# cc-ai/climategan

Hardware: AMD Instinct MI355X
Metric: 640x640 images/sec (G+D step): per-domain sample slots per second of the joint Masker+Painter training step (update_G + update_D), global batch 32 per domain (higher is better)
Workload: dtype bf16

## Files before the change

climategan_amd/_lib.py:

```python
import ctypes as C
import os
from pathlib import Path

_HERE = Path(__file__).resolve().parent
LIB_PATH = Path(os.environ["CGAN_LIB"]).resolve() if os.environ.get("CGAN_LIB") else _HERE / "libcgan_hip.so"

CGAN_F16, CGAN_BF16, CGAN_F32 = 0, 1, 2
ACT_NONE, ACT_RELU, ACT_LRELU, ACT_TANH, ACT_SIGMOID = 0, 1, 2, 3, 4
PAD_ZERO, PAD_REFLECT = 0, 1
ABI_VERSION = 1


class ConvDesc(C.Structure):
    _fields_ = [
        ("dtype", C.c_int32), ("n", C.c_int32), ("h_in", C.c_int32), ("w_in", C.c_int32),
        ("c_in", C.c_int32), ("c_out", C.c_int32),
        ("kh", C.c_int32), ("kw", C.c_int32), ("stride", C.c_int32), ("pad", C.c_int32), ("dilation", C.c_int32),
        ("pad_mode", C.c_int32), ("h_out", C.c_int32), ("w_out", C.c_int32), ("in_upsample", C.c_int32),
        ("act", C.c_int32), ("act_slope", C.c_float), ("has_bias", C.c_int32), ("has_residual", C.c_int32),
        ("residual_upsample", C.c_int32),
    ]


class NormStatsDesc(C.Structure):
# ... 2 lines not shown

class SpadeDesc(C.Structure):
    _fields_ = [
        ("dtype", C.c_int32), ("n", C.c_int32), ("h", C.c_int32), ("w", C.c_int32), ("c", C.c_int32),
        ("x_upsample", C.c_int32), ("cond_h", C.c_int32), ("cond_w", C.c_int32), ("cond_c", C.c_int32),
        ("hidden", C.c_int32), ("ksize", C.c_int32), ("act", C.c_int32), ("act_slope", C.c_float),
    ]


class SnItem(C.Structure):
    _fields_ = [("w_bar", C.c_void_p), ("u", C.c_void_p), ("v", C.c_void_p), ("sigma", C.c_void_p),
                ("workspace", C.c_void_p), ("rows", C.c_int32), ("cols", C.c_int32)]


class PackItem(C.Structure):
    _fields_ = [("w_oihw", C.c_void_p), ("bias", C.c_void_p), ("sigma", C.c_void_p), ("packed", C.c_void_p),
                ("bias_out", C.c_void_p), ("c_out", C.c_int32), ("c_in", C.c_int32), ("kh", C.c_int32),
                ("kw", C.c_int32), ("transposed", C.c_int32)]


class AdamItem(C.Structure):
    _fields_ = [("p", C.c_void_p), ("g", C.c_void_p), ("m", C.c_void_p), ("v", C.c_void_p), ("copy", C.c_void_p),
                ("numel", C.c_int64)]


class AmpOptimItem(C.Structure):
    _fields_ = [("p", C.c_void_p), ("g", C.c_void_p), ("m", C.c_void_p), ("v", C.c_void_p), ("step", C.c_void_p),
                ("numel", C.c_int64)]


class DataTfMap(C.Structure):
    _fields_ = [("row_off", C.c_int32), ("col_off", C.c_int32), ("flip", C.c_int32)]


class DataTfStage(C.Structure):
    _fields_ = [("in_h", C.c_int32), ("in_w", C.c_int32), ("out_h", C.c_int32), ("out_w", C.c_int32)]


class DataTfItem(C.Structure):
    _fields_ = [("src", C.c_void_p), ("dst", C.c_void_p), ("src_h", C.c_int32), ("src_w", C.c_int32),
                ("channels", C.c_int32), ("stride_c", C.c_int32), ("stride_h", C.c_int32), ("stride_w", C.c_int32),
                ("out_h", C.c_int32), ("out_w", C.c_int32), ("n_stages", C.c_int32), ("u8_min", C.c_float),
                ("u8_range", C.c_float), ("stage", DataTfStage * 2), ("map", DataTfMap * 3),
                ("stats", C.c_void_p), ("far_plane", C.c_float), ("dec_flags", C.c_int32)]


class DataTfPalette(C.Structure):
    _fields_ = [("n", C.c_int32), ("default_class", C.c_int32), ("colour", C.c_uint32 * 16), ("cls", C.c_int32 * 16)]


class DataMinmaxItem(C.Structure):
    _fields_ = [("src", C.c_void_p), ("out", C.c_void_p), ("pixels", C.c_int64), ("channels", C.c_int32),
                ("far_plane", C.c_float)]


_P = C.c_void_p
_SIGNATURES = {
    "cgan_version": (C.c_int, []),
    "cgan_last_error": (C.c_char_p, []),
    "cgan_conv2d_packed_weight_bytes": (C.c_size_t, [C.POINTER(ConvDesc)]),
    "cgan_conv2d_pack_weight": (C.c_int, [_P, _P, _P, _P, _P, C.POINTER(ConvDesc), _P]),
    "cgan_conv2d_nhwc_fwd": (C.c_int, [_P, _P, _P, _P, _P, C.POINTER(ConvDesc), _P]),
    "cgan_conv2d_pack_weight_batched": (C.c_int, [_P, C.c_int32, C.c_int32, C.c_int32, _P]),
    "cgan_conv2d_dgrad_packed_weight_bytes": (C.c_size_t, [C.POINTER(ConvDesc)]),
    "cgan_conv2d_pack_weight_dgrad": (C.c_int, [_P, _P, _P, C.POINTER(ConvDesc), _P]),
    "cgan_conv2d_nhwc_bwd_data": (C.c_int, [_P, _P, _P, C.POINTER(ConvDesc), _P]),
    "cgan_conv2d_nhwc_fwd_pair": (C.c_int, [_P, _P, _P, _P, _P, C.POINTER(ConvDesc), _P]),
    "cgan_pair_expand_weight": (C.c_int, [_P, _P, _P, C.c_int32, C.c_int32, C.c_int32, C.c_int32, C.c_int32, _P]),
    "cgan_pair_instnorm_stats": (C.c_int, [_P, _P, _P, C.c_int32, C.c_int32, C.c_int32, C.c_int64, C.c_float, _P]),
    "cgan_pair_spade_apply": (C.c_int, [_P, _P, _P, _P, _P, _P, C.c_int32, C.c_int32, C.c_int32, C.c_int32, C.c_int32, C.c_int32,
                                        C.c_int32, C.c_float, _P]),
    "cgan_pair_make_m_cond_workspace_bytes": (C.c_size_t, [C.c_int32]),
    "cgan_pair_make_m_cond": (C.c_int, [_P, _P, _P, _P, C.c_int32, C.c_int32, C.c_int32, C.c_int32, C.c_int32, C.c_int32, C.c_int32,
                                        _P, C.c_size_t, _P]),
    "cgan_pair_from_nchw": (C.c_int, [_P, _P, C.c_int32, C.c_int32, C.c_int32, C.c_int32, C.c_int32, _P]),
    "cgan_pair_to_nchw": (C.c_int, [_P, _P, C.c_int32, C.c_int32, C.c_int32, C.c_int32, C.c_int32, C.c_int32, _P]),
    "cgan_pair_to_nhwc": (C.c_int, [_P, _P, C.c_int32, C.c_int64, C.c_int32, _P]),
    "cgan_pair_maxpool3x3s2": (C.c_int, [_P, _P, C.c_int32, C.c_int32, C.c_int32, C.c_int32, C.c_int32, _P]),
    "cgan_pair_resize_bilinear": (C.c_int, [_P, _P, C.c_int32, C.c_int32, C.c_int32, C.c_int32, C.c_int32, C.c_int32,
                                            C.c_int32, C.c_int32, _P]),
    "cgan_pair_resize_nearest": (C.c_int, [_P, _P, C.c_int32, C.c_int32, C.c_int32, C.c_int32, C.c_int32, C.c_int32, C.c_int32,
                                           _P]),
    "cgan_pair_resize_bicubic": (C.c_int, [_P, _P, C.c_int32, C.c_int32, C.c_int32, C.c_int32, C.c_int32, C.c_int32, C.c_int32, _P]),
    "cgan_pair_mul": (C.c_int, [_P, _P, _P, C.c_int32, C.c_int64, C.c_int32, _P]),
    "cgan_pair_copy_channels": (C.c_int, [_P, _P, C.c_int32, C.c_int64, C.c_int32, C.c_int32, C.c_int32, _P]),
    "cgan_conv2d_nhwc_bwd_data_add": (C.c_int, [_P, _P, _P, _P, C.POINTER(ConvDesc), _P]),
    "cgan_conv2d_nhwc_bwd_data_relu": (C.c_int, [_P, _P, _P, _P, C.POINTER(ConvDesc), _P]),
    "cgan_conv2d_nhwc_bwd_data_add_relu": (C.c_int, [_P, _P, _P, _P, _P, C.POINTER(ConvDesc), _P]),
    "cgan_conv2d_kernel_kind": (C.c_int, [C.POINTER(ConvDesc), C.c_int32]),
    "cgan_conv2d_kernel_kind_on": (C.c_int, [C.POINTER(ConvDesc), C.c_int32, _P]),
    "cgan_conv2d_bind_workspace": (C.c_int, [_P, _P, C.c_size_t]),
    "cgan_rccl_load": (C.c_int, [C.c_char_p]),
    "cgan_rccl_loaded": (C.c_int, []),
    "cgan_comm_unique_id": (C.c_int, [_P]),
    "cgan_comm_init_rank": (C.c_int, [C.POINTER(C.c_void_p), C.c_int32, _P, C.c_int32]),
    "cgan_comm_destroy": (C.c_int, [_P]),
    "cgan_allreduce_bucket": (C.c_int, [_P, C.c_int64, C.c_int32, _P, _P]),
    "cgan_seg_counts": (C.c_int, [_P, C.c_int32, C.c_int32, C.c_int32, C.c_int64, C.c_int32, _P, _P, _P]),
    "cgan_mask_label_encode": (C.c_int, [_P] + [C.c_int32] * 10 + [_P, _P]),
    "cgan_masker_eval_workspace_bytes": (C.c_size_t, [C.c_int32] * 3),
    "cgan_masker_eval": (C.c_int, [_P, C.c_int32, _P, C.c_int32, C.c_int32, C.c_int32, C.c_int32, C.c_double, C.c_double,
                                   _P, _P, _P, _P, _P, _P, C.c_size_t, _P]),
    "cgan_resize_crop_geometry":(C.c_int, [C.c_int32, C.c_int32, C.c_int32, C.POINTER(C.c_int32), C.POINTER(C.c_int32),
                                            C.POINTER(C.c_int32), C.POINTER(C.c_int32)]),
    "cgan_resize_u8": (C.c_int, [_P, C.c_int32, C.c_int32, C.c_int32, C.c_int32, C.c_int32, _P, C.c_int32, _P, C.c_int32, _P,
                                 _P, C.c_size_t, _P]),
# ... 7 lines not shown
    "cgan_norm_act_apply": (C.c_int, [_P, _P, _P, _P, C.POINTER(NormStatsDesc), C.c_int32, C.c_float, _P]),
    "cgan_make_m_cond_bwd_nhwc": (C.c_int, [_P, _P, _P, _P, _P, C.c_int32, C.c_int32, C.c_int32, C.c_int32, C.c_int32,
                                            C.c_int32, _P]),
    "cgan_resize_nearest_bwd_nhwc": (C.c_int, [_P, _P, C.c_int32, C.c_int32, C.c_int32, C.c_int32, C.c_int32, C.c_int32,
                                               C.c_int32, C.c_int32, C.c_int32, _P]),
    "cgan_norm_add_act_apply": (C.c_int, [_P, _P, _P, _P, _P, C.POINTER(NormStatsDesc), C.c_int32, C.c_float, _P]),
    "cgan_spade_packed_weight_bytes": (C.c_size_t, [C.POINTER(SpadeDesc)]),
    "cgan_spade_pack_weights": (C.c_int, [_P, _P, _P, _P, _P, _P, _P, C.POINTER(SpadeDesc), _P]),
    "cgan_spade_fused_fwd": (C.c_int, [_P, _P, _P, _P, _P, _P, C.POINTER(SpadeDesc), _P]),
    "cgan_spade_fused_fwd_train": (C.c_int, [_P, _P, _P, _P, _P, _P, _P, C.POINTER(SpadeDesc), _P]),
    "cgan_spectral_norm_workspace_bytes": (C.c_size_t, [C.c_int32, C.c_int32]),
    "cgan_spectral_norm_power_iter": (C.c_int, [_P, _P, _P, _P, C.c_int32, C.c_int32, _P, C.c_size_t, _P]),
    "cgan_spectral_norm_power_iter_batched": (C.c_int, [_P, C.c_int32, C.c_int32, C.c_int32, _P]),
    "cgan_extra_adam_multi_tensor": (C.c_int, [_P, C.c_int32, C.c_int64, C.c_int32, C.c_int32, C.c_int32, C.c_double,
                                               C.c_double, C.c_double, C.c_double, C.c_double, _P]),
    "cgan_grads_nonfinite_check_multi_tensor": (C.c_int, [_P, C.c_int32, C.c_int64, C.c_double, C.c_int32, _P, _P]),
    "cgan_adam_multi_tensor": (C.c_int, [_P, C.c_int32, C.c_int64] + [C.c_double] * 6 + [_P, _P]),
    "cgan_rmsprop_multi_tensor": (C.c_int, [_P, C.c_int32, C.c_int64] + [C.c_double] * 5 + [_P, _P]),
    "cgan_amp_optim_finish": (C.c_int, [_P, C.c_int32, _P, _P]),
    "cgan_nchw_to_nhwc": (C.c_int, [_P, _P, _P, C.c_int32, C.c_int32, C.c_int32, C.c_int32, C.c_int32, C.c_int32, _P]),
    "cgan_nhwc_to_nchw": (C.c_int, [_P, _P, _P, _P, C.c_int32, C.c_int32, C.c_int32, C.c_int32, C.c_int32, C.c_int32, _P]),
    "cgan_resize_nearest_nhwc": (C.c_int, [_P, _P, C.c_int32, C.c_int32, C.c_int32, C.c_int32, C.c_int32, C.c_int32,
                                           C.c_int32, C.c_int32, C.c_int32, _P]),
    "cgan_avgpool3x3s2_nhwc": (C.c_int, [_P, _P, C.c_int32, C.c_int32, C.c_int32, C.c_int32, C.c_int32, _P]),
    "cgan_maxpool3x3s2_nhwc": (C.c_int, [_P, _P, C.c_int32, C.c_int32, C.c_int32, C.c_int32, C.c_int32, _P]),
    "cgan_resize_bilinear_nhwc": (C.c_int, [_P, _P, C.c_int32, C.c_int32, C.c_int32, C.c_int32, C.c_int32, C.c_int32,
                                            C.c_int32, C.c_int32, _P]),
    "cgan_resize_bicubic_nhwc": (C.c_int, [_P, _P, C.c_int32, C.c_int32, C.c_int32, C.c_int32, C.c_int32, C.c_int32,
                                           C.c_int32, _P]),
    "cgan_sumpool2x2_nhwc": (C.c_int, [_P, _P, C.c_int32, C.c_int32, C.c_int32, C.c_int32, C.c_int32, _P]),
    "cgan_reflect_pad_bwd_nhwc": (C.c_int, [_P, _P, C.c_int32, C.c_int32, C.c_int32, C.c_int32, C.c_int32, C.c_int32, _P]),
    "cgan_copy_channels_nhwc": (C.c_int, [_P, _P, C.c_int64, C.c_int32, C.c_int32, C.c_int32, C.c_int32, _P]),
    "cgan_eltwise_nhwc": (C.c_int, [_P, _P, _P, C.c_int32, C.c_int32, C.c_int64, _P]),
    "cgan_fold_bn": (C.c_int, [_P, _P, _P, _P, _P, _P, C.c_float, _P, _P, C.c_int32, C.c_int64, _P]),
    "cgan_act_bwd": (C.c_int, [_P, _P, _P, C.c_int32, C.c_int32, C.c_float, C.c_int64, _P]),
    "cgan_instnorm_act_bwd_workspace_bytes": (C.c_size_t, [C.POINTER(NormStatsDesc)]),
    "cgan_instnorm_act_bwd": (C.c_int, [_P, _P, _P, _P, C.POINTER(NormStatsDesc), C.c_int32, C.c_float, _P, C.c_size_t,
                                        _P]),
    "cgan_spade_bwd_prepare": (C.c_int, [_P, _P, _P, _P, _P, _P, _P, _P, _P, C.POINTER(SpadeDesc), _P]),
    "cgan_spade_hidden_bwd_workspace_bytes": (C.c_size_t, [C.POINTER(SpadeDesc)]),
    "cgan_spade_hidden_bwd": (C.c_int, [_P, _P, _P, _P, _P, _P, _P, _P, C.c_size_t, C.POINTER(SpadeDesc), _P]),
    "cgan_batchnorm_train_stats": (C.c_int, [_P, _P, _P, C.c_float, _P, _P, _P, _P, _P, _P, _P, C.POINTER(NormStatsDesc), _P,
                                             C.c_size_t, _P]),
    "cgan_batchnorm_train_stats_from_partials": (C.c_int, [_P, C.c_int32, _P, _P, C.c_float, _P, _P, _P, _P, _P, _P, _P,
                                                           C.POINTER(NormStatsDesc), _P]),
    "cgan_conv2d_stats_chunk_pixels": (C.c_int32, [C.POINTER(ConvDesc)]),
    "cgan_conv2d_nhwc_fwd_stats": (C.c_int, [_P, _P, _P, _P, _P, C.c_size_t, C.POINTER(ConvDesc), _P]),
    "cgan_bn_train_prepare": (C.c_int, [_P, _P, _P, _P, C.c_float, C.c_float, C.c_int64, _P, _P, _P, _P, _P, C.c_int32, _P]),
    "cgan_batchnorm_act_bwd_workspace_bytes": (C.c_size_t, [C.c_int32]),
    "cgan_batchnorm_act_bwd": (C.c_int, [_P, _P, _P, _P, _P, _P, _P, _P, _P, _P, _P, _P, C.c_int32, C.c_int64, C.c_int32,
                                         C.c_int32, C.c_float, _P, C.c_size_t, _P]),
    "cgan_batchnorm_act_bwd_grouped": (C.c_int, [_P, _P, _P, _P, _P, _P, _P, _P, _P, _P, _P, _P, C.c_int32, C.c_int64,
                                                 C.c_int32, C.c_int32, C.c_int32, C.c_float, _P, C.c_size_t, _P]),
    "cgan_bce_logits_nhwc": (C.c_int, [_P, C.c_int32, C.c_int64, C.c_int32, C.c_float, C.c_float, _P, _P, _P]),
    "cgan_hinge_nhwc": (C.c_int, [_P, C.c_int32, C.c_int64, C.c_int32, C.c_int32, C.c_int32, C.c_float, _P, _P, _P]),
    "cgan_l1_nhwc": (C.c_int, [_P, _P, C.c_int32, C.c_int64, C.c_float, _P, _P, _P]),
    "cgan_mse_const_nhwc": (C.c_int, [_P, C.c_int32, C.c_int64, C.c_int32, C.c_float, C.c_float, _P, _P, _P]),
    "cgan_painter_aux_losses": (C.c_int, [_P, _P, _P, C.c_int32, C.c_int32, C.c_int32, C.c_int32, C.c_float, C.c_float,
                                          C.c_float, C.c_float, _P, _P, _P]),
    "cgan_resize_bicubic_bwd_nhwc": (C.c_int, [_P, _P, C.c_int32, C.c_int32, C.c_int32, C.c_int32, C.c_int32, C.c_int32,
                                               C.c_int32, _P]),
    "cgan_spectral_norm_bwd": (C.c_int, [_P, _P, _P, _P, _P, C.c_int32, C.c_int32, _P, _P]),
    "cgan_painter_heads_fwd": (C.c_int, [_P, _P, _P, _P, _P, C.c_int32, C.c_int32, C.c_int32, C.c_int32, _P]),
    "cgan_painter_heads_bwd": (C.c_int, [_P, _P, _P, _P, C.c_int32, C.c_int32, C.c_int32, C.c_int32, _P]),
    "cgan_diffaug_fwd": (C.c_int, [_P, _P, _P, _P, C.c_int32, C.c_int32, C.c_int32, C.c_int32, C.c_int32, C.c_int32,
                                   C.c_int32, _P, _P]),
    "cgan_diffaug_bwd": (C.c_int, [_P, _P, _P, _P, C.c_int32, C.c_int32, C.c_int32, C.c_int32, C.c_int32, C.c_int32,
                                   C.c_int32, _P, _P]),
    "cgan_painter_heads_diffaug_fwd": (C.c_int, [_P, _P, _P, _P, _P, _P, _P, C.c_int32, C.c_int32, C.c_int32, C.c_int32,
                                                 C.c_int32, C.c_int32, C.c_int32, _P, _P]),
    "cgan_painter_heads_diffaug_bwd": (C.c_int, [_P, _P, _P, _P, _P, _P, C.c_int32, C.c_int32, C.c_int32, C.c_int32,
                                                 C.c_int32, C.c_int32, C.c_int32, _P, _P]),
    "cgan_data_transform": (C.c_int, [_P, _P, C.c_int32, C.c_int32, C.c_int32, C.c_int32, _P, _P, _P, C.c_int32, _P, _P]),
    "cgan_data_source_minmax": (C.c_int, [_P, _P, C.c_int32, C.c_int32, _P, _P]),
    "cgan_data_jitter": (C.c_int, [_P, _P, _P, C.c_int32, C.c_int32, C.c_int32, C.c_int32, _P, _P, _P, _P]),
    "cgan_avgpool3x3s2_bwd_nhwc": (C.c_int, [_P, _P, C.c_int32, C.c_int32, C.c_int32, C.c_int32, C.c_int32, _P]),
    "cgan_maxpool2x2_nhwc": (C.c_int, [_P, _P, C.c_int32, C.c_int32, C.c_int32, C.c_int32, C.c_int32, _P]),
    "cgan_maxpool2x2_bwd_nhwc": (C.c_int, [_P, _P, _P, C.c_int32, C.c_int32, C.c_int32, C.c_int32, C.c_int32, _P]),
    "cgan_maxpool2x2_relu_bwd_nhwc": (C.c_int, [_P, _P, _P, C.c_int32, C.c_int32, C.c_int32, C.c_int32, C.c_int32, _P]),
    "cgan_softmax_nhwc": (C.c_int, [_P, _P, C.c_int32, C.c_int64, C.c_int32, _P]),
    "cgan_softmax_bwd_nhwc": (C.c_int, [_P, _P, _P, C.c_int32, C.c_int64, C.c_int32, _P]),
    "cgan_sigmoid_pair_nhwc": (C.c_int, [_P, _P, C.c_int32, C.c_int64, _P]),
    "cgan_sigmoid_pair_bwd_nhwc": (C.c_int, [_P, _P, _P, C.c_int32, C.c_int64, _P]),
    "cgan_softmax_ce_nhwc": (C.c_int, [_P, _P, C.c_int32, C.c_int64, C.c_int32, C.c_float, _P, _P, _P]),
    "cgan_tv_nhwc": (C.c_int, [_P, C.c_int32, C.c_int32, C.c_int32, C.c_int32, C.c_int32, C.c_float, C.c_float, _P, _P, _P]),
    "cgan_advent_entropy_pair_nhwc": (C.c_int, [_P, _P, _P, C.c_int32, C.c_int64, C.c_int32, C.c_int32, _P]),
    "cgan_entropy_pair_from_nchw": (C.c_int, [_P, _P, _P, C.c_int32, C.c_int32, C.c_int32, C.c_int32, C.c_int32, _P]),
    "cgan_entropy_pair_from_nchw_bwd": (C.c_int, [_P, _P, _P, _P, C.c_int32, C.c_int32, C.c_int32, C.c_int32, C.c_int32, _P]),
    "cgan_advent_entropy_pair_bwd_nhwc": (C.c_int, [_P, _P, _P, _P, C.c_int32, C.c_int64, C.c_int32, C.c_int32, _P]),
    "cgan_entropy_map_nhwc": (C.c_int, [_P, _P, _P, C.c_int32, C.c_int64, C.c_int32, _P]),
    "cgan_entropy_map_bwd_nhwc": (C.c_int, [_P, _P, _P, _P, C.c_int32, C.c_int64, C.c_int32, _P]),
    "cgan_minent_nhwc": (C.c_int, [_P, C.c_int32, C.c_int64, C.c_int32, C.c_int32, C.c_float, C.c_float, _P, _P, _P, _P]),
    "cgan_bce_logits_map_nhwc": (C.c_int, [_P, _P, C.c_int32, C.c_int64, C.c_float, _P, _P, _P]),
    "cgan_ground_intersection_nhwc": (C.c_int, [_P, _P, C.c_int32, C.c_int64, C.c_float, _P, _P]),
    "cgan_affine_sum_nhwc": (C.c_int, [_P, C.c_int32, C.c_int64, C.c_int32, C.c_float, C.c_float, _P, _P, _P]),
    "cgan_resize_bilinear_bwd_workspace_bytes": (C.c_size_t, [C.c_int32] * 4),
    "cgan_resize_bilinear_bwd_nhwc": (C.c_int, [_P, _P] + [C.c_int32] * 8 + [_P, C.c_size_t, _P]),
    "cgan_maxpool3x3s2_bwd_nhwc": (C.c_int, [_P, _P, _P, C.c_int32, C.c_int32, C.c_int32, C.c_int32, C.c_int32, _P]),
    "cgan_add_act_nhwc": (C.c_int, [_P, _P, _P, C.c_int32, C.c_int32, C.c_float, C.c_int64, _P]),
    "cgan_slice_channels_nhwc": (C.c_int, [_P, _P, C.c_int64, C.c_int32, C.c_int32, C.c_int32, _P]),
    "cgan_sigm_loss_workspace_bytes": (C.c_size_t, [C.c_int32, C.c_int32, C.c_int32]),
    "cgan_sigm_loss_nhwc": (C.c_int, [_P, _P, C.c_int32, C.c_int32, C.c_int32, C.c_int32, C.c_float, C.c_int32, C.c_float,
                                      _P, _P, _P, C.c_size_t, _P]),
    "cgan_normalize_u8_workspace_bytes": (C.c_size_t, [C.c_int32]),
    "cgan_normalize_u8_nhwc": (C.c_int, [_P, C.c_int32, _P, C.c_int32, C.c_int32, C.c_int32, C.c_int32, _P, C.c_size_t,
                                         _P]),
# ... 115 lines not shown
```

climategan_amd/autograd.py:

```python
import ctypes as C

import os

import torch

from . import ops


GRAD_SCALE = 1.0


def set_grad_scale(s: float):
    global GRAD_SCALE
    GRAD_SCALE = float(s)


BN_GROUPS = 1


class bn_groups:

    def __init__(self, groups: int):
        self.groups = int(groups)

# ... 89 lines not shown

    @staticmethod
    def backward(ctx, dy_t):
        c, h, w, cs = ctx.cfg
        return ops.resize_nearest_bwd(ops.NHWC(dy_t.contiguous(), c), (h, w), cs).t, None, None, None


class ConvFn(torch.autograd.Function):

    @staticmethod
    def forward(ctx, x_t, weight, bias, res_t, packed, cfg, sn):
        x = ops.NHWC(x_t, cfg["c_in"])
        res = ops.NHWC(res_t, weight.shape[0]) if res_t is not None else None
        if cfg.get("mask_input") and (cfg.get("in_upsample", False) or cfg.get("pair_in", False)):
            raise NotImplementedError("ConvFn: mask_input with a folded upsample / a pair map")
        if cfg.get("want_stats") and res is None and cfg["act"] == ops.ACT_NONE and not cfg.get("in_upsample", False):
            y, cfg["stats_out"] = ops.conv2d_with_stats(x, packed, stride=cfg["stride"], pad=cfg["pad"],
                                                        dilation=cfg["dilation"], pad_mode=cfg.get("pad_mode", ops.PAD_ZERO),
                                                        groups=BN_GROUPS)
        else:
            y = ops.conv2d(x, packed, stride=cfg["stride"], pad=cfg["pad"], dilation=cfg["dilation"], act=cfg["act"],
                           slope=cfg["slope"], residual=res, in_upsample=cfg.get("in_upsample", False),
                           residual_upsample=cfg.get("residual_upsample", False),
                           pad_mode=cfg.get("pad_mode", ops.PAD_ZERO))
        ctx.cfg = cfg
        ctx.has_bias = bias is not None
        ctx.has_res = res_t is not None
        ctx.premasked = False
        ctx.sn = None if sn is None else (tuple(sn) if cfg.get("sn_owned") else tuple(t.clone() for t in sn))
        ctx.dgrad = None
        if ctx.needs_input_grad[0] and not cfg.get("pair_in", False):
            ctx.dgrad = ops.dgrad_register(weight, ctx.sn[0] if ctx.sn is not None else None, x_t.dtype, cfg["stride"])
        ctx.save_for_backward(x_t, weight, y.t if cfg["act"] != ops.ACT_NONE else None)
        return y.t

    @staticmethod
    def backward(ctx, dy_t):
        cfg = ctx.cfg
        x_t, weight, y_t = ctx.saved_tensors
        c_out = weight.shape[0]
        ups = cfg.get("in_upsample", False)
        dy = ops.NHWC(dy_t.contiguous(), c_out)
        if y_t is not None and not ctx.premasked:
            dy = ops.act_bwd(ops.NHWC(y_t, c_out), dy, cfg["act"], cfg["slope"])
        sigma = ctx.sn[0] if ctx.sn is not None else None
        dx_t = dres_t = None
        pair = cfg.get("pair_in", False)
        w_eff = torch.cat([weight.detach(), weight.detach()], 1) if pair else weight
        if ctx.needs_input_grad[0]:
            h_in, w_in = (x_t.shape[1] * 2, x_t.shape[2] * 2) if ups else (x_t.shape[1], x_t.shape[2])
            relu_out = ops.NHWC(x_t, cfg["c_in"]) if cfg.get("mask_input") else None
            dx = ops.conv2d_bwd_data(dy, w_eff, (x_t.shape[0], h_in, w_in), stride=cfg["stride"], pad=cfg["pad"],
                                     dilation=cfg["dilation"], sigma=sigma, pad_mode=cfg.get("pad_mode", ops.PAD_ZERO),
                                     prepacked=ctx.dgrad, relu_out=relu_out)
            dx_t = (ops.sumpool2x2(dx) if ups else dx).t
        if ctx.has_res and ctx.needs_input_grad[3]:
            dres_t = (ops.sumpool2x2(dy) if cfg.get("residual_upsample", False) else dy).t
        dw = db = None
        if ctx.needs_input_grad[1] or (ctx.has_bias and ctx.needs_input_grad[2]):
            def wgrad():
                dw, db = ops.conv2d_bwd_weight(ops.NHWC(x_t, cfg["c_in"]), dy, tuple(w_eff.shape), stride=cfg["stride"],
                                               pad=cfg["pad"], dilation=cfg["dilation"], want_bias=ctx.has_bias,
                                               in_upsample=ups, pad_mode=cfg.get("pad_mode", ops.PAD_ZERO))
                if pair:
                    dw = dw[:, :weight.shape[1]] + dw[:, weight.shape[1]:]
                if ctx.sn is not None:
                    dw = ops.spectral_norm_bwd(dw, weight.detach(), ctx.sn[1], ctx.sn[2], ctx.sn[0])
                return dw, db
            dw, db = wgrad()
        return dx_t, dw, db, dres_t, None, None, None


class ConvPassFn(torch.autograd.Function):

    @staticmethod
    def forward(ctx, x_t, weight, bias, packed, cfg):
        x = ops.NHWC(x_t, cfg["c_in"])
        if cfg.get("want_stats") and cfg.get("act", ops.ACT_NONE) != ops.ACT_NONE:
            raise NotImplementedError("ConvPassFn: the statistics epilogue belongs to a conv without an activation")
        if cfg.get("want_stats"):
            y, cfg["stats_out"] = ops.conv2d_with_stats(x, packed, stride=cfg["stride"], pad=cfg["pad"],
                                                        dilation=cfg["dilation"], pad_mode=cfg.get("pad_mode", ops.PAD_ZERO),
                                                        groups=BN_GROUPS)
        else:
            y = ops.conv2d(x, packed, stride=cfg["stride"], pad=cfg["pad"], dilation=cfg["dilation"],
                           act=cfg.get("act", ops.ACT_NONE), slope=cfg.get("slope", 0.0),
                           pad_mode=cfg.get("pad_mode", ops.PAD_ZERO))
        ctx.cfg = cfg
        ctx.has_bias = bias is not None
        ctx.premasked = False
        ctx.dgrad = ops.dgrad_register(weight, None, x_t.dtype, cfg["stride"]) if ctx.needs_input_grad[0] else None
        ctx.save_for_backward(x_t, weight, y.t if cfg.get("act", ops.ACT_NONE) != ops.ACT_NONE else None)
        return y.t, x_t

    @staticmethod
    def backward(ctx, dy_t, dpass_t):
        cfg = ctx.cfg
        x_t, weight, y_t = ctx.saved_tensors
        c_out = weight.shape[0]
        dy = ops.NHWC(dy_t.contiguous(), c_out)
        if y_t is not None and not ctx.premasked:
            dy = ops.act_bwd(ops.NHWC(y_t, c_out), dy, cfg["act"], cfg.get("slope", 0.0))
        dx_t = None
        if ctx.needs_input_grad[0]:
            add = ops.NHWC(dpass_t.contiguous(), cfg["c_in"]) if dpass_t is not None else None
            relu_out = ops.NHWC(x_t, cfg["c_in"]) if cfg.get("mask_input") else None
            dx_t = ops.conv2d_bwd_data(dy, weight, (x_t.shape[0], x_t.shape[1], x_t.shape[2]), stride=cfg["stride"],
                                       pad=cfg["pad"], dilation=cfg["dilation"],
                                       pad_mode=cfg.get("pad_mode", ops.PAD_ZERO), add=add, prepacked=ctx.dgrad,
                                       relu_out=relu_out).t
        dw = db = None
        if ctx.needs_input_grad[1] or (ctx.has_bias and ctx.needs_input_grad[2]):
            dw, db = ops.conv2d_bwd_weight(
                ops.NHWC(x_t, cfg["c_in"]), dy, tuple(weight.shape), stride=cfg["stride"], pad=cfg["pad"],
                dilation=cfg["dilation"], want_bias=ctx.has_bias, pad_mode=cfg.get("pad_mode", ops.PAD_ZERO))
        return dx_t, dw, db, None, None


class InstNormActFn(torch.autograd.Function):

    @staticmethod
    def forward(ctx, x_t, c, eps, act, slope):
        x = ops.NHWC(x_t, c)
        mean, rstd = ops.instnorm_stats(x, eps=eps)
        out = ops.norm_act_apply(x, mean, rstd, act=act, slope=slope)
        ctx.c, ctx.act, ctx.slope = c, act, slope
        ctx.save_for_backward(out.t, rstd)
        return out.t

    @staticmethod
    def backward(ctx, dy_t):
        out_t, rstd = ctx.saved_tensors
        dx = ops.instnorm_act_bwd(ops.NHWC(out_t, ctx.c), ops.NHWC(dy_t.contiguous(), ctx.c), rstd, act=ctx.act,
                                  slope=ctx.slope)
        return dx.t, None, None, None, None


_SPADE_REMAT_GAMMA = os.environ.get("CGAN_SPADE_REMAT_GAMMA") == "1"


_SPADE_FUSED_BWD = os.environ.get("CGAN_SPADE_FUSED_BWD", "1") != "0"


class SpadeFn(torch.autograd.Function):

    @staticmethod
    def forward(ctx, x_t, cond_t, mean, rstd, w_sh, b_sh, w_g, b_g, w_b, b_b, packed, cfg):
        x = ops.NHWC(x_t, cfg["c"])
        cond = ops.NHWC(cond_t, cfg["cond_c"])
        gamma_t = None
        if _SPADE_REMAT_GAMMA or not any(ctx.needs_input_grad):
            y = ops.spade_fused(x, mean, rstd, cond, packed, act=cfg["act"], slope=cfg["slope"],
                                x_upsample=cfg["x_upsample"])
        else:
            y, gamma = ops.spade_fused(x, mean, rstd, cond, packed, act=cfg["act"], slope=cfg["slope"],
                                       x_upsample=cfg["x_upsample"], want_gamma=True)
            gamma_t = gamma.t
        ctx.cfg = cfg
        ctx.save_for_backward(x_t, cond_t, mean, rstd, y.t, w_sh, b_sh, w_g, b_g, w_b, b_b, gamma_t)
        return y.t

    @staticmethod
    def backward(ctx, dy_t):
# ... 121 lines not shown
        ctx.c, ctx.hw = c, (x_t.shape[1], x_t.shape[2])
        return ops.avgpool3x3s2(ops.NHWC(x_t, c)).t

    @staticmethod
    def backward(ctx, dy_t):
        return ops.avgpool3x3s2_bwd(ops.NHWC(dy_t.contiguous(), ctx.c), ctx.hw).t, None


class MaxPool2x2Fn(torch.autograd.Function):

    @staticmethod
    def forward(ctx, x_t, c, mask_input=False):
        ctx.c = c
        ctx.mask_input = bool(mask_input)
        ctx.save_for_backward(x_t)
        return ops.maxpool2x2(ops.NHWC(x_t, c)).t

    @staticmethod
    def backward(ctx, dy_t):
        (x_t,) = ctx.saved_tensors
        return ops.maxpool2x2_bwd(ops.NHWC(x_t, ctx.c), ops.NHWC(dy_t.contiguous(), ctx.c), relu_input=ctx.mask_input).t, None, None


_BN_BWD_READS_OUT = os.environ.get("CGAN_BN_BWD_OUT") == "1"


class BatchNormActFn(torch.autograd.Function):

    @staticmethod
    def forward(ctx, x_t, gamma, beta, running_mean, running_var, c, eps, momentum, act, slope, nbt=None, res_t=None,
                conv_stats=None):
        n, h, w, cs = x_t.shape
        G = BN_GROUPS
        if n % G:
            raise ValueError("BatchNormActFn: batch %d does not divide into %d groups" % (n, G))
        npix = n * h * w // G
        x_t = x_t.contiguous()
        flat = ops.NHWC(x_t.view(G, npix, 1, cs), c)
        if conv_stats is not None and npix % conv_stats.chunk_pixels == 0:
            mean, rstd, mean_f, rstd_f = ops.batchnorm_train_stats_from_partials(
                conv_stats, G, npix, c, gamma, beta, running_mean, running_var, nbt, eps, momentum)
        else:
            mean, rstd, mean_f, rstd_f = ops.batchnorm_train_stats(flat, gamma, beta, running_mean, running_var, nbt, eps,
                                                                   momentum)
        res = None
        if res_t is not None:
            if res_t.shape != x_t.shape:
                raise ValueError("BatchNormActFn: residual %s does not match %s" % (tuple(res_t.shape), tuple(x_t.shape)))
            res = ops.NHWC(res_t.contiguous().view(G, npix, 1, cs), c)
        out = ops.norm_act_apply(flat, mean_f, rstd_f, act=act, slope=slope, residual=res).t.view(n, h, w, cs)
        ctx.cfg = (c, act, slope, G)
        ctx.has_res = res_t is not None
        ctx.premasked = False
        keep_out = res_t is not None or _BN_BWD_READS_OUT
        ctx.save_for_backward(x_t, out if keep_out else None, mean, rstd, gamma,
                              None if keep_out else mean_f, None if keep_out else rstd_f)
        return out

    @staticmethod
    def backward(ctx, dy_t):
        from . import _lib
        lib = _lib.load()
        x_t, out, mean, rstd, gamma, mean_f, rstd_f = ctx.saved_tensors
        c, act, slope, G = ctx.cfg
        if ctx.premasked:
            act = ops.ACT_NONE
        n, h, w, cs = x_t.shape
        nbytes = G * lib.cgan_batchnorm_act_bwd_workspace_bytes(c)
        ws = torch.empty(nbytes, dtype=torch.uint8, device=x_t.device)
        dx = torch.empty_like(x_t)
        want_res = ctx.has_res and ctx.needs_input_grad[11]
        dy_t = dy_t.contiguous()
        if want_res and act == ops.ACT_NONE:
            dres = dy_t
        else:
            dres = torch.empty_like(x_t) if want_res else None
        dg = db = None
        if gamma is not None:
            dg, db = torch.empty((2, c), dtype=torch.float32, device=x_t.device).unbind(0)
        _lib.check(lib.cgan_batchnorm_act_bwd_grouped(
            ops._ptr(x_t), ops._ptr(out), ops._ptr(dy_t), ops._ptr(mean), ops._ptr(rstd), ops._ptr(gamma),
            ops._ptr(mean_f), ops._ptr(rstd_f), ops._ptr(dx), ops._ptr(dg), ops._ptr(db), ops._ptr(dres) if dres is not None and dres is not dy_t else None,
            ops._DT[x_t.dtype], n * h * w, c, G, act, slope, ops._ptr(ws), nbytes, ops._stream()),
            "cgan_batchnorm_act_bwd_grouped")
        return dx, dg, db, None, None, None, None, None, None, None, None, dres, None


def claim_relu_mask(out_t: torch.Tensor) -> bool:
    fn = out_t.grad_fn
    if fn is None:
        return False
    if isinstance(fn, BatchNormActFn._backward_cls):
        if not fn.has_res or fn.cfg[1] != ops.ACT_RELU:
            return False
    elif isinstance(fn, (ConvFn._backward_cls, ConvPassFn._backward_cls)):
        if fn.cfg.get("act", ops.ACT_NONE) != ops.ACT_RELU:
            return False
    else:
        return False
    fn.premasked = True
    return True


def _scaled(dx, c, g):
    return None if dx is None else ops.scale_by_scalar(ops.NHWC(dx, c), g.reshape(1).float().contiguous()).t


class PainterAuxFn(torch.autograd.Function):

    @staticmethod
    def forward(ctx, fake_t, x, m, lam_tv, lam_ctx, lam_rec):
        from . import _lib
        n, h, w = fake_t.shape[0], fake_t.shape[1], fake_t.shape[2]
        x = x.contiguous().float()
        m = m.contiguous().float()
        cnt = float(n * 3 * h * w)
        wh = GRAD_SCALE * lam_tv * 2.0 / (3 * (h - 1) * w) / n
        ww = GRAD_SCALE * lam_tv * 2.0 / (3 * h * (w - 1)) / n
        acc = torch.zeros(3, dtype=torch.float32, device=fake_t.device)
        dfake = torch.empty_like(fake_t) if ctx.needs_input_grad[0] else None
        _lib.check(_lib.load().cgan_painter_aux_losses(ops._ptr(fake_t), ops._ptr(x), ops._ptr(m), ops._DT[fake_t.dtype], n, h, w,
                                                       wh, ww, GRAD_SCALE * lam_ctx / cnt, GRAD_SCALE * lam_rec / cnt,
                                                       ops._ptr(acc), ops._ptr(dfake), ops._stream()), "cgan_painter_aux_losses")
        ctx.save_for_backward(dfake)
        if GRAD_SCALE != 1.0:
            acc = acc / GRAD_SCALE
        ctx.mark_non_differentiable(acc)
        return acc.sum(), acc

    @staticmethod
    def backward(ctx, g, _g_parts):
        (dfake,) = ctx.saved_tensors
        return _scaled(dfake, 3, g), None, None, None, None, None


class ResizeBicubicFn(torch.autograd.Function):

    @staticmethod
    def forward(ctx, x_t, c, size):
        ctx.cfg = (c, x_t.shape[1], x_t.shape[2], int(size[0]), int(size[1]))
        return ops.resize_bicubic(ops.NHWC(x_t, c), size).t

    @staticmethod
    def backward(ctx, dy):
        from . import _lib
        c, h_in, w_in, h_out, w_out = ctx.cfg
        dy = dy.contiguous()
        dx = torch.empty((dy.shape[0], h_in, w_in, dy.shape[3]), dtype=dy.dtype, device=dy.device)
        _lib.check(_lib.load().cgan_resize_bicubic_bwd_nhwc(ops._ptr(dy), ops._ptr(dx), ops._DT[dy.dtype], dy.shape[0], c, h_in,
                                                            w_in, h_out, w_out, ops._stream()), "cgan_resize_bicubic_bwd_nhwc")
        return dx, None, None


def _call(name, *args):
# ... 347 lines not shown
```

climategan_amd/csrc/conv_gemm.h:

```cpp
#pragma once
#include "cgan_common.h"

struct ConvGemmArgs {
  const uint16_t* x;
  const u32x4* w;
  const float* bias;
  const uint16_t* res;
  const uint16_t* res2;
  uint16_t* y;
  int n, h_in, w_in, cin_s;
  int cout, cout_s, ctiles, ksteps;
  int kh, kw, stride, pad, dil, pad_mode;
  int h_out, w_out, npix;
  int act, has_res, res_ups;
  float slope;
  float* stats;
};

struct ConvGemmCls {
  int koff;
  int kh, kw;
  int offy, offx;
};
struct ConvGemmExtArgs {
  ConvGemmArgs a;
  int cls_s;
  int ksplit;
  int ks_per;
  float* ws;
  int pair;
  ConvGemmCls cls[4];
};
bool conv_gemm_ext_shape_ok(const ConvGemmArgs& a);
int conv_gemm_splitk_plan(const ConvGemmArgs& a);
size_t conv_gemm_splitk_workspace_bytes(const ConvGemmArgs& a, int ksplit);
int conv_gemm_splitk_launch(const ConvGemmArgs& a, int ksplit, float* ws, int dtype, hipStream_t s);
int conv_gemm_cls_launch(const ConvGemmArgs& a, int cls_s, const ConvGemmCls* cls, int dtype, hipStream_t s);
int conv_gemm_pair_launch(const ConvGemmArgs& a, int dtype, hipStream_t s);

bool conv_gemm_applicable(const CganConvDesc* d);
int conv_gemm_launch(const ConvGemmArgs& a, int dtype, hipStream_t s);
bool conv_gemm_res2_ok(const ConvGemmArgs& a, int dtype);
int conv_gemm_stats_chunk_pixels(const ConvGemmArgs& a, int dtype);
bool conv_gemm_big_ok(const ConvGemmArgs& a);
bool conv1x1_allc_ok(const ConvGemmArgs& a);
int conv1x1_allc_launch(const ConvGemmArgs& a, int dtype, hipStream_t s);
int conv_gemm_big_launch(const ConvGemmArgs& a, int dtype, hipStream_t s);
bool conv_gemm_big_pair_ok(const ConvGemmArgs& a, int dtype);
int conv_gemm_big_pair_launch(const ConvGemmArgs& a, int dtype, hipStream_t s);
bool conv1x1_xres_ok(const ConvGemmArgs& a);
int conv1x1_xres_launch(const ConvGemmArgs& a, int dtype, hipStream_t s);

#ifdef __HIPCC__
typedef float f32x2 __attribute__((ext_vector_type(2)));

__device__ __forceinline__ float row16_sum(float v) {
  v += __builtin_bit_cast(float, __builtin_amdgcn_update_dpp(0, __builtin_bit_cast(int, v), 0x128, 0xf, 0xf, false));
  v += __builtin_bit_cast(float, __builtin_amdgcn_update_dpp(0, __builtin_bit_cast(int, v), 0x124, 0xf, 0xf, false));
  v += __builtin_bit_cast(float, __builtin_amdgcn_update_dpp(0, __builtin_bit_cast(int, v), 0x122, 0xf, 0xf, false));
  v += __builtin_bit_cast(float, __builtin_amdgcn_update_dpp(0, __builtin_bit_cast(int, v), 0x121, 0xf, 0xf, false));
  return v;
}

template <typename T, int WC, int WP>
__device__ __forceinline__ void conv_gemm_stats_epilogue(f32x4 (&acc)[WC][WP], const ConvGemmArgs& p, int cout_base,
                                                         int chunk, int j, int g) {
  if (p.bias) {
#pragma unroll
    for (int c = 0; c < WC; ++c) {
      const int chb = cout_base + c * 16 + 4 * g;
      const f32x4 b = chb < p.cout_s ? *reinterpret_cast<const f32x4*>(p.bias + chb) : (f32x4){0.f, 0.f, 0.f, 0.f};
#pragma unroll
      for (int t = 0; t < WP; ++t) acc[c][t] += b;
    }
  }
  constexpr float inv_cnt = 1.f / (float)(WP * 16);
#pragma unroll
  for (int c = 0; c < WC; ++c) {
    f32x2 vr[WP][2];
#pragma unroll
    for (int t = 0; t < WP; ++t) {
#pragma unroll
      for (int hh = 0; hh < 2; ++hh) {
        float r0, r1;
        unpack2<T>(pack2<T>(acc[c][t][2 * hh], acc[c][t][2 * hh + 1]), r0, r1);
        vr[t][hh] = (f32x2){r0, r1};
      }
    }
    f32x2 s0[2] = {vr[0][0], vr[0][1]};
#pragma unroll
    for (int t = 1; t < WP; ++t) {
      s0[0] += vr[t][0];
      s0[1] += vr[t][1];
    }
    float sm[4], sq[4];
#pragma unroll
    for (int r = 0; r < 4; ++r) sm[r] = row16_sum(s0[r >> 1][r & 1]) * inv_cnt;
    const f32x2 m2[2] = {(f32x2){sm[0], sm[1]}, (f32x2){sm[2], sm[3]}};
    f32x2 s1[2];
#pragma unroll
    for (int hh = 0; hh < 2; ++hh) {
      const f32x2 dv = vr[0][hh] - m2[hh];
      s1[hh] = dv * dv;
    }
#pragma unroll
    for (int t = 1; t < WP; ++t)
#pragma unroll
      for (int hh = 0; hh < 2; ++hh) {
        const f32x2 dv = vr[t][hh] - m2[hh];
        s1[hh] += dv * dv;
      }
#pragma unroll
    for (int r = 0; r < 4; ++r) sq[r] = row16_sum(s1[r >> 1][r & 1]);
    const int ch = cout_base + c * 16 + 4 * g;
    if (j == 0 && ch < p.cout_s) {
      float o[8];
#pragma unroll
      for (int r = 0; r < 4; ++r) {
        o[2 * r] = sm[r];
        o[2 * r + 1] = sq[r];
      }
      float* dst = p.stats + ((size_t)chunk * p.cout_s + ch) * 2;
      *reinterpret_cast<f32x4*>(dst) = (f32x4){o[0], o[1], o[2], o[3]};
      *reinterpret_cast<f32x4*>(dst + 4) = (f32x4){o[4], o[5], o[6], o[7]};
    }
  }
}

template <typename T, int WC, int WP, int PP, bool RES2 = false>
__device__ __forceinline__ void conv_gemm_staged_store(const f32x4 (&acc)[WC][WP], const ConvGemmArgs& p,
                                                       unsigned char* stg, int pix0, int cout_base, const float* bias_ep,
                                                       int lane, int j, int g) {
  constexpr int ROWB = WC * 64 + 16;
  constexpr int CH = WC * 2;
  constexpr int NIT = PP * 16 * CH / 64;
  constexpr int NPASS = WP / PP;
  constexpr int PSTEP = 64 / CH;
  static_assert(64 % CH == 0 && WP % PP == 0, "a lane keeps its channel chunk over the iterations");
  const int qc = lane % CH, pl0 = lane / CH;
  const int ch = cout_base + qc * 8;
  const bool ch_ok = ch < p.cout_s;
  const bool plain = !bias_ep && !p.has_res && p.act == CGAN_ACT_NONE && p.cout == p.cout_s;
  f32x4 bb0 = (f32x4){0.f, 0.f, 0.f, 0.f}, bb1 = bb0;
  if (bias_ep && ch_ok) {
    bb0 = *reinterpret_cast<const f32x4*>(bias_ep + ch);
    bb1 = *reinterpret_cast<const f32x4*>(bias_ep + ch + 4);
  }
  u32x4 rv[NPASS][NIT];
  u32x4 rm[RES2 ? (NPASS > 1 ? 2 : 1) : 1][RES2 ? NIT : 1];
  auto load_rm = [&](int pass, u32x4 (&dst)[RES2 ? NIT : 1]) {
#pragma unroll
    for (int it = 0; it < (RES2 ? NIT : 0); ++it) {
      const int pix = pix0 + pass * PP * 16 + it * PSTEP + pl0;
      dst[it] = (u32x4){0u, 0u, 0u, 0u};
      if (pix < p.npix && ch_ok) dst[it] = CGAN_LD_STREAM(reinterpret_cast<const u32x4*>(p.res2 + (size_t)pix * p.cout_s + ch));
    }
  };
  if (p.has_res) {
#pragma unroll
    for (int pass = 0; pass < NPASS; ++pass)
#pragma unroll
      for (int it = 0; it < NIT; ++it) {
        const int pix = pix0 + pass * PP * 16 + it * PSTEP + pl0;
        rv[pass][it] = (u32x4){0u, 0u, 0u, 0u};
        if (pix < p.npix && ch_ok) {
          size_t rbase;
          if (p.res_ups) {
            const int ox = pix % p.w_out;
            const int r = pix / p.w_out;
            const int oy = r % p.h_out;
            const int nn = r / p.h_out;
            rbase = (((size_t)nn * (p.h_out >> 1) + (oy >> 1)) * (p.w_out >> 1) + (ox >> 1)) * p.cout_s;
          } else {
            rbase = (size_t)pix * p.cout_s;
          }
          rv[pass][it] = CGAN_LD_STREAM(reinterpret_cast<const u32x4*>(p.res + rbase + ch));
        }
      }
    if (RES2 && p.has_res == 3) load_rm(0, rm[0]);
    __builtin_amdgcn_sched_barrier(0);
  }
#pragma unroll
  for (int pass = 0; pass < NPASS; ++pass) {
#pragma unroll
    for (int tt = 0; tt < PP; ++tt)
#pragma unroll
      for (int c = 0; c < WC; ++c)
        *reinterpret_cast<f32x4*>(stg + (tt * 16 + j) * ROWB + c * 64 + g * 16) = acc[c][pass * PP + tt];
    asm volatile("s_waitcnt lgkmcnt(0)" ::: "memory");
    if (RES2 && NPASS > 1 && p.has_res == 3 && pass + 1 < NPASS) {
      __builtin_amdgcn_sched_barrier(0);
      load_rm(pass + 1, rm[(pass + 1) & 1]);
      __builtin_amdgcn_sched_barrier(0);
    }
    if (pass == 0 || (RES2 && p.has_res == 3 && pass >= 2)) __builtin_amdgcn_s_waitcnt(0x0F70);
#pragma unroll
    for (int it = 0; it < NIT; ++it) {
      const int pl = it * PSTEP + pl0;
      const int pix = pix0 + pass * PP * 16 + pl;
      const f32x4 v0 = *reinterpret_cast<const f32x4*>(stg + pl * ROWB + qc * 32);
      const f32x4 v1 = *reinterpret_cast<const f32x4*>(stg + pl * ROWB + qc * 32 + 16);
      float v[8] = {v0[0], v0[1], v0[2], v0[3], v1[0], v1[1], v1[2], v1[3]};
      if (!plain) {
        if (bias_ep) {
#pragma unroll
          for (int r = 0; r < 4; ++r) {
            v[r] += bb0[r];
            v[4 + r] += bb1[r];
          }
        }
        if (RES2 && p.has_res == 3) {
#pragma unroll
          for (int e = 0; e < 4; ++e) {
            float r0, r1, m0, m1;
            unpack2<T>(rv[pass][it][e], r0, r1);
            unpack2<T>(rm[RES2 && NPASS > 1 ? (pass & 1) : 0][RES2 ? it : 0][e], m0, m1);
            v[2 * e] = cgan_res_apply3(v[2 * e], r0, m0);
            v[2 * e + 1] = cgan_res_apply3(v[2 * e + 1], r1, m1);
          }
        } else if (p.has_res) {
#pragma unroll
          for (int e = 0; e < 4; ++e) {
            float r0, r1;
            unpack2<T>(rv[pass][it][e], r0, r1);
            v[2 * e] = cgan_res_apply(v[2 * e], r0, p.has_res);
            v[2 * e + 1] = cgan_res_apply(v[2 * e + 1], r1, p.has_res);
          }
        }
        act_apply_n(v, p.act, p.slope);
        if (p.cout < p.cout_s) {
#pragma unroll
          for (int r = 0; r < 8; ++r)
            if (ch + r >= p.cout) v[r] = 0.f;
        }
      }
      u32x4 o;
#pragma unroll
      for (int e = 0; e < 4; ++e) o[e] = pack2<T>(v[2 * e], v[2 * e + 1]);
      if (pix < p.npix && ch_ok) CGAN_ST_STREAM(o, reinterpret_cast<u32x4*>(p.y + (size_t)pix * p.cout_s + ch));
    }
    asm volatile("s_waitcnt lgkmcnt(0)" ::: "memory");
  }
}
#endif
```

climategan_amd/csrc/conv_gemm.hip:

```cpp
#include "conv_gemm.h"
#include <type_traits>

namespace {

__device__ __attribute__((aligned(16))) unsigned int g_gemm_zeros[4];

constexpr int NSTAGE = 3;
CGAN_KNOB(int, g_gemm_ws, 0);

__device__ __forceinline__ int reflect_i(int i, int n) {
  if (i < 0) i = -i;
  if (i >= n) i = 2 * n - 2 - i;
  return i;
}

template <typename T, int WAVES_C, int WC, int WP, bool REFLECT, int NS = NSTAGE, bool RES2 = false>
__global__ __launch_bounds__(256, 2) void conv_gemm_kernel(ConvGemmArgs p, int npb, int ncb) {
  constexpr int WAVES_P = 4 / WAVES_C;
  constexpr int CT_BLK = WAVES_C * WC;
  constexpr int PT_BLK = WAVES_P * WP;
  constexpr int STAGE_BYTES = (CT_BLK + PT_BLK) * 1024;
  constexpr int W_PER_WAVE = CT_BLK / 4;
  constexpr int P_PER_WAVE = PT_BLK / 4;
  constexpr int DMA_PER_WAVE = W_PER_WAVE + P_PER_WAVE;
  static_assert(CT_BLK % 4 == 0 && PT_BLK % 4 == 0, "tiles must split evenly over the 4 waves");
  extern __shared__ __attribute__((aligned(1024))) unsigned char smem[];

  const int lane = threadIdx.x & 63;
  const int wave = __builtin_amdgcn_readfirstlane(threadIdx.x >> 6);
  const int j = lane & 15;
  const int g = lane >> 4;
  const int wc = wave % WAVES_C, wp = wave / WAVES_C;

  const int xcd = blockIdx.x & 7, slot = blockIdx.x >> 3;
  const int cblk = slot % ncb;
  const int pblk = xcd * ((npb + 7) >> 3) + slot / ncb;
  if (pblk >= npb) return;

  int pbase[P_PER_WAVE], py0[P_PER_WAVE], px0[P_PER_WAVE];
#pragma unroll
  for (int m = 0; m < P_PER_WAVE; ++m) {
    int pix = (pblk * PT_BLK + wave + 4 * m) * 16 + j;
    bool v = pix < p.npix;
    int pc = v ? pix : 0;
    int ox = pc % p.w_out;
    int r = pc / p.w_out;
    int oy = r % p.h_out;
    int nn = r / p.h_out;
    pbase[m] = nn * p.h_in * p.w_in * p.cin_s + g * 8;
    py0[m] = v ? oy * p.stride - p.pad : -(1 << 28);
    px0[m] = ox * p.stride - p.pad;
  }
  const int ccn = p.cin_s >> 5;
  const long zero_off = reinterpret_cast<const unsigned char*>(g_gemm_zeros) - reinterpret_cast<const unsigned char*>(p.x);

  int i_ky = 0, i_kx = 0, i_cc = 0, i_buf = 0;
  auto issue_piece = [&](int piece) {
    unsigned char* buf = smem + i_buf * STAGE_BYTES;
    if (piece < W_PER_WAVE) {
      const int i = wave + 4 * piece;
      const int ct = min(cblk * CT_BLK + i, p.ctiles - 1);
      const u32x4* src = p.w + ((size_t)ct * p.ksteps + (i_ky * p.kw + i_kx) * ccn + i_cc) * 64 + lane;
      __builtin_amdgcn_global_load_lds((const __attribute__((address_space(1))) void*)src,
                                       (__attribute__((address_space(3))) void*)(buf + i * 1024), 16, 0, 0);
    } else {
      const int m = piece - W_PER_WAVE;
      const int i = wave + 4 * m;
      int iy = py0[m] + i_ky * p.dil, ix = px0[m] + i_kx * p.dil;
      bool ok;
      if (REFLECT) {
// ... 25 lines not shown
    for (int q = 0; q < DMA_PER_WAVE; ++q) issue_piece(q);
    issue_advance();
  };

  f32x4 acc[WC][WP];
#pragma unroll
  for (int c = 0; c < WC; ++c)
#pragma unroll
    for (int t = 0; t < WP; ++t) acc[c][t] = (f32x4){0.f, 0.f, 0.f, 0.f};

  issue();
  if (NS > 2) issue();
  int r_buf = 0;
  for (int ks = 0; ks < p.ksteps; ++ks) {
    asm volatile("s_waitcnt vmcnt(%0) lgkmcnt(0)" ::"n"((NS - 2) * DMA_PER_WAVE) : "memory");
    __builtin_amdgcn_s_barrier();
    const unsigned char* buf = smem + r_buf * STAGE_BYTES;
    u32x4 a[WC], b[WP];
#pragma unroll
    for (int t = 0; t < WP; ++t)
      b[t] = *reinterpret_cast<const u32x4*>(buf + (CT_BLK + wp * WP + t) * 1024 + lane * 16);
#pragma unroll
    for (int c = 0; c < WC; ++c) a[c] = *reinterpret_cast<const u32x4*>(buf + (wc * WC + c) * 1024 + lane * 16);
    constexpr int NM = WC * WP;
    constexpr int GAP = NM / (DMA_PER_WAVE + 1);
    __builtin_amdgcn_sched_barrier(0);
#pragma unroll
    for (int i = 0; i < NM; ++i) {
      const int c = i / WP, t = i % WP;
      acc[c][t] = mfma16(as_vec8<T>(a[c]), as_vec8<T>(b[t]), acc[c][t]);
      if ((i + 1) % GAP == 0 && (i + 1) / GAP <= DMA_PER_WAVE) {
        issue_piece((i + 1) / GAP - 1);
        __builtin_amdgcn_sched_barrier(0);
      }
    }
    issue_advance();
    r_buf = (r_buf + 1 == NS) ? 0 : r_buf + 1;
  }

  constexpr int ROWB = WC * 64 + 16;
  constexpr int PP = (4 * 4 * 16 * ROWB <= NS * STAGE_BYTES && WP % 4 == 0) ? 4
                     : (4 * 2 * 16 * ROWB <= NS * STAGE_BYTES ? 2 : 1);
  static_assert(4 * PP * 16 * ROWB <= NS * STAGE_BYTES, "epilogue staging does not fit");
  static_assert(WP % PP == 0, "WP must be a multiple of PP");
  asm volatile("s_waitcnt vmcnt(0) lgkmcnt(0)" ::: "memory");
  __builtin_amdgcn_s_barrier();
  unsigned char* stg = smem + wave * (PP * 16 * ROWB);
  const int cout_base = (cblk * CT_BLK + wc * WC) * 16;
  const float* bias_ep = p.bias;
  if (p.stats && (pblk * PT_BLK + wp * WP) * 16 < p.npix) {
    conv_gemm_stats_epilogue<T, WC, WP>(acc, p, cout_base, pblk * WAVES_P + wp, j, g);
    if (p.bias) bias_ep = nullptr;
  }
  conv_gemm_staged_store<T, WC, WP, PP, RES2>(acc, p, stg, (pblk * PT_BLK + wp * WP) * 16, cout_base, bias_ep, lane, j, g);
}

template <typename T, int WC, int WP>
__global__ __launch_bounds__(512, 2) void conv_gemm_k64_kernel(ConvGemmArgs p, int npb, int ncb, int tiles_total) {
  constexpr int CT_BLK = 2 * WC, PT_BLK = 2 * WP;
  constexpr int W_BYTES = CT_BLK * 2048, STAGE_BYTES = (CT_BLK + PT_BLK) * 2048;
  constexpr int NS = 3;
  constexpr int W_PER = CT_BLK / 2, P_PER = PT_BLK / 2, PIECES = W_PER + P_PER;
  static_assert(PIECES <= 63, "vmcnt range");
  extern __shared__ __attribute__((aligned(1024))) unsigned char smem[];

  const int lane = threadIdx.x & 63;
  const int wave = __builtin_amdgcn_readfirstlane(threadIdx.x >> 6);
  const int xcd = blockIdx.x & 7, slot = blockIdx.x >> 3, nslot = gridDim.x >> 3;
  const int per = (tiles_total + 7) >> 3;
  const int t0 = xcd * per;
  const int t1 = min(t0 + per, tiles_total);
  const int my_n = (t1 - t0 > slot) ? (t1 - t0 - slot + nslot - 1) / nslot : 0;
  if (my_n <= 0) return;
  const int first = t0 + slot;
  const int cc2n = p.cin_s >> 6;
  const int n_st = p.kh * p.kw * cc2n;
  const int n_it = my_n * n_st;

  if (wave >= 4) {
    const int pw = wave - 4;
    const int half = pw & 1;
    const int ccn = p.cin_s >> 5;
    const long zero_off = reinterpret_cast<const unsigned char*>(g_gemm_zeros) - reinterpret_cast<const unsigned char*>(p.x);
    const int q = lane >> 3;
    const int kchunk = (lane & 7) ^ (4 * half + ((q >> 1) & 3));
    int poff[P_PER];
    unsigned vmask[P_PER];
    const u32x4* wtile[W_PER];
    auto set_tile = [&](int ti) {
      const int gt = first + ti * nslot;
      const int pblk = gt / ncb;
      const int cblk = gt - pblk * ncb;
#pragma unroll
      for (int m = 0; m < W_PER; ++m)
        wtile[m] = p.w + (size_t)min(cblk * CT_BLK + (pw >> 1) + 2 * m, p.ctiles - 1) * p.ksteps * 64 + half * 64 + lane;
#pragma unroll
      for (int m = 0; m < P_PER; ++m) {
        const int pix = (pblk * PT_BLK + (pw >> 1) + 2 * m) * 16 + 8 * half + q;
        const bool v = pix < p.npix;
        const int pc = v ? pix : 0;
        const int ox = pc % p.w_out;
        const int r = pc / p.w_out;
        const int oy = r % p.h_out;
        const int nn = r / p.h_out;
        const int py0 = oy * p.stride - p.pad, px0 = ox * p.stride - p.pad;
        poff[m] = ((nn * p.h_in * p.w_in + py0 * p.w_in + px0) * p.cin_s + kchunk * 8) * 2;
        unsigned mk = 0;
// ... 156 lines not shown
#pragma unroll
        for (int r = 0; r < 4; ++r) {
          v[r] = act_apply(v[r], p.act, p.slope);
          if (ch + r >= p.cout) v[r] = 0.f;
        }
        u32x2 o;
        o.x = pack2<T>(v[0], v[1]);
        o.y = pack2<T>(v[2], v[3]);
        CGAN_ST_STREAM(o, reinterpret_cast<u32x2*>(p.y + (size_t)pix * p.cout_s + ch));
      }
    }
  };

  for (int ti = 0; ti < my_n; ++ti) {
    first_read(ti > 0);
    for (int st = 0; st + 1 < n_st; ++st) {
      step(a0, b0, a1, b1, 1);
      step(a1, b1, a0, b0, 0);
    }
    step(a0, b0, a1, b1, 1);
    step(a1, b1, a0, b0, -1);
    epilogue(ti);
  }
}

template <typename T, int WC, int WP>
int launch_k64(const ConvGemmArgs& a, hipStream_t s) {
  constexpr int CT_BLK = 2 * WC, PT_BLK = 2 * WP;
  constexpr size_t smem = (size_t)3 * (CT_BLK + PT_BLK) * 2048;
  static bool attr_set = false;
  if (!attr_set) {
    hipError_t e = hipFuncSetAttribute(reinterpret_cast<const void*>(&conv_gemm_k64_kernel<T, WC, WP>),
                                       hipFuncAttributeMaxDynamicSharedMemorySize, 160 * 1024);
    if (e != hipSuccess) {
      cgan_set_error("conv_gemm_k64: hipFuncSetAttribute failed: %s", hipGetErrorString(e));
      return CGAN_ERR_HIP;
    }
    attr_set = true;
  }
  const int npb = ceil_div(ceil_div(a.npix, 16), PT_BLK);
  const int ncb = ceil_div(a.ctiles, CT_BLK);
  const int tiles = npb * ncb;
  const int per = ceil_div(tiles, 8);
  const int nslot = per < 32 ? per : 32;
  hipLaunchKernelGGL((conv_gemm_k64_kernel<T, WC, WP>), dim3(8 * nslot), dim3(512), smem, s, a, npb, ncb, tiles);
  return CGAN_OK;
}
bool k64_ok(const ConvGemmArgs& a) {
  return (a.cin_s & 63) == 0 && a.pad_mode != CGAN_PAD_REFLECT && a.kh * a.kw <= 32 &&
         (long)a.n * a.h_in * a.w_in * a.cin_s < (1L << 30) - (1L << 20);
}


template <typename T, int WAVES_C, int WC, int WP, bool REFLECT, int NS = NSTAGE, bool RES2 = false>
int launch_cfg2(const ConvGemmArgs& a, hipStream_t s) {
  constexpr int WAVES_P = 4 / WAVES_C;
  constexpr int CT_BLK = WAVES_C * WC, PT_BLK = WAVES_P * WP;
  constexpr size_t smem = (size_t)NS * (CT_BLK + PT_BLK) * 1024;
  static bool attr_set = false;
  if (!attr_set) {
    hipError_t e = hipFuncSetAttribute(reinterpret_cast<const void*>(&conv_gemm_kernel<T, WAVES_C, WC, WP, REFLECT, NS, RES2>),
                                       hipFuncAttributeMaxDynamicSharedMemorySize, 160 * 1024);
    if (e != hipSuccess) {
      cgan_set_error("conv_gemm: hipFuncSetAttribute failed: %s", hipGetErrorString(e));
      return CGAN_ERR_HIP;
    }
    attr_set = true;
  }
  const int npb = ceil_div(ceil_div(a.npix, 16), PT_BLK);
  const int ncb = ceil_div(a.ctiles, CT_BLK);
  const int grid = ceil_div(npb, 8) * 8 * ncb;
  hipLaunchKernelGGL((conv_gemm_kernel<T, WAVES_C, WC, WP, REFLECT, NS, RES2>), dim3(grid), dim3(256), smem, s, a, npb, ncb);
  return CGAN_OK;
}

template <typename T, int WAVES_C, int WC, int WP, int NS = NSTAGE>
int launch_cfg(const ConvGemmArgs& a, hipStream_t s) {
  return a.pad_mode == CGAN_PAD_REFLECT ? launch_cfg2<T, WAVES_C, WC, WP, true, NS>(a, s)
                                        : launch_cfg2<T, WAVES_C, WC, WP, false, NS>(a, s);
}

CGAN_KNOB(int, g_gemm_cfg, 0);

enum { KIND_PLAIN = 0, KIND_K64_256x128, KIND_K64_128x256, KIND_BIG, KIND_DIRECT, KIND_XRES };
struct Choice {
  int kind;
  int cfg;
};

Choice choose(const ConvGemmArgs& a, bool bf16) {
  const int ptiles = ceil_div(a.npix, 16);
  const bool no_big = g_gemm_ws == 9;
  const bool no_xres = g_gemm_ws == 9 || g_gemm_ws == 12;
  const int ws = (no_big || no_xres || g_gemm_ws == 13 || g_gemm_ws == 14) ? 0 : g_gemm_ws;
  switch (ws) {
    case 5: if (k64_ok(a)) return {KIND_K64_256x128, 0}; break;
    case 6: if (k64_ok(a)) return {KIND_K64_128x256, 0}; break;
    case 8: if (conv_gemm_big_ok(a)) return {KIND_BIG, 0}; break;
    case 10: if (conv1x1_allc_ok(a)) return {KIND_DIRECT, 0}; break;
    case 11: if (conv1x1_xres_ok(a)) return {KIND_XRES, 0}; break;
    default: break;
  }
  const bool automatic = ws == 0 && g_gemm_cfg == 0;
  (void)bf16;
  if (automatic && !no_big && conv1x1_allc_ok(a) && a.ctiles <= 4 && a.npix >= 16384) return {KIND_DIRECT, 0};
  if (automatic && !no_xres && conv1x1_xres_ok(a) && a.ctiles >= 16 && a.npix >= 16384) return {KIND_XRES, 0};
  const bool long_1x1 = a.kh * a.kw == 1 && g_gemm_ws != 13 &&
                        (g_gemm_ws == 14 ? (a.cin_s >= 2048 || (a.cin_s >= 512 && a.ctiles >= 128))
                                         : (a.cin_s >= 1024 || (a.cin_s >= 512 && a.ctiles >= 128)));
  if (automatic && !no_big && conv_gemm_big_ok(a) && a.npix >= 16384 &&
      ((a.cin_s * a.kh * a.kw >= 4096 && a.cin_s >= 512 && !(a.kh * a.kw >= 9 && a.cin_s >= 2048)) || long_1x1))
    return {KIND_BIG, 0};
  if (automatic && k64_ok(a) && a.kh * a.kw >= 9 && a.cin_s >= 512 && a.npix >= 16384) return {KIND_K64_256x128, 0};
  switch (g_gemm_cfg) {
    case 1: return {KIND_PLAIN, 1};
    case 2: if (a.ctiles <= 16) return {KIND_PLAIN, 2}; break;
    case 3: return {KIND_PLAIN, 3};
    case 4: return {KIND_PLAIN, 4};
    case 5: return {KIND_PLAIN, 5};
    default: break;
  }
  if (a.ctiles <= 4) return {KIND_PLAIN, 1};
  if (a.kh * a.kw == 1 && a.ksteps <= 16) return {KIND_PLAIN, 5};
  if (a.ctiles > 8 && a.ctiles <= 16 && ceil_div(ptiles, 8) >= 384) return {KIND_PLAIN, 2};
  if ((long)ceil_div(ptiles, 16) * ceil_div(a.ctiles, 8) >= 384) return {KIND_PLAIN, 3};
  return {KIND_PLAIN, 4};
}

template <typename T>
int launch(const ConvGemmArgs& a, hipStream_t s) {
  const Choice ch = choose(a, std::is_same<T, BF16>::value);
  switch (ch.kind) {
    case KIND_K64_256x128: return launch_k64<T, 8, 4>(a, s);
    case KIND_K64_128x256: return launch_k64<T, 4, 8>(a, s);
    case KIND_BIG: return conv_gemm_big_launch(a, T::id, s);
    case KIND_DIRECT: return conv1x1_allc_launch(a, T::id, s);
    case KIND_XRES: return conv1x1_xres_launch(a, T::id, s);
    default: break;
  }
  switch (ch.cfg) {
    case 1: return launch_cfg<T, 1, 4, 4>(a, s);
    case 2: return launch_cfg<T, 2, 8, 4>(a, s);
    case 3: return launch_cfg<T, 2, 4, 8>(a, s);
    case 5:
      if (a.has_res == 3) return launch_cfg2<T, 2, 4, 4, false, 2, true>(a, s);
      return launch_cfg<T, 2, 4, 4, 2>(a, s);
    default: return launch_cfg<T, 2, 4, 4>(a, s);
  }
}

}

bool conv_gemm_applicable(const CganConvDesc* d) {
  const int cin_s = cgan_cs(d->c_in), cout_s = cgan_cs(d->c_out);
  const long npix = (long)d->n * d->h_out * d->w_out;
  const long in_elems = (long)d->n * d->h_in * d->w_in * cin_s;
  return (cin_s % 32) == 0 && cout_s >= 64 && !d->in_upsample && npix >= 2048 && in_elems < (1L << 31) - (1L << 20) &&
         (long)ceil_div((int)ceil_div((int)npix, 16), 8) * ceil_div(ceil_div(cout_s, 16), 8) >= 128;
}

CGAN_DEV_ONLY(extern "C" void cgan_debug_set_gemm_cfg(int v) { g_gemm_cfg = v; })
CGAN_DEV_ONLY(extern "C" void cgan_debug_set_gemm_ws(int v) { g_gemm_ws = v; })

int conv_gemm_launch(const ConvGemmArgs& a, int dtype, hipStream_t s) {
  return dtype == CGAN_F16 ? launch<F16>(a, s) : launch<BF16>(a, s);
}

bool conv_gemm_res2_ok(const ConvGemmArgs& a, int dtype) {
  const Choice ch = choose(a, dtype == CGAN_BF16);
  return (ch.kind == KIND_PLAIN && ch.cfg == 5 && a.pad_mode != CGAN_PAD_REFLECT) || ch.kind == KIND_BIG;
}

int conv_gemm_stats_chunk_pixels(const ConvGemmArgs& a, int dtype) {
  const Choice ch = choose(a, dtype == CGAN_BF16);
  if (ch.kind == KIND_XRES) return a.npix % 128 == 0 ? 128 : 0;
  if (ch.kind == KIND_BIG) return a.npix % 64 == 0 ? 64 : 0;
  if (ch.kind != KIND_PLAIN) return 0;
  const int ppb = ch.cfg == 3 ? 128 : 64;
  return a.npix % ppb == 0 ? ppb : 0;
}
```

climategan_amd/csrc/conv_gemm_big.hip:

```cpp
#include "conv_gemm.h"
#include <type_traits>

namespace {

__device__ __attribute__((aligned(16))) unsigned int g_big_zeros[4];

template <typename T, int NW, bool PAIR = false, bool RES2 = false>
__global__ __launch_bounds__(NW * 64, NW / 4) void conv_gemm_big_kernel(ConvGemmArgs p, int npb, int ncb) {
  constexpr int WC = NW == 16 ? 4 : 8;
  constexpr int WP = NW == 4 ? 8 : 4;
  constexpr bool DOUBLE = NW == 4;
  constexpr int CT_BLK = 16, PT_BLK = 16;
  constexpr int STAGE = 32 * 1024;
  constexpr int NSW = 2, NSX = 3;
  constexpr int X_BASE = NSW * STAGE;
  constexpr int NPC = 32 / NW;
  constexpr int NM = WC * WP, NR = WC + WP;
  static_assert(NSW * STAGE + NSX * STAGE == 160 * 1024, "the rings take all of the CU's LDS");
  extern __shared__ __attribute__((aligned(1024))) unsigned char smem[];

  const int lane = threadIdx.x & 63;
  const int wave = __builtin_amdgcn_readfirstlane(threadIdx.x >> 6);
  const int xcd = blockIdx.x & 7, slot = blockIdx.x >> 3;
  const int cblk = slot % ncb;
  const int pblk = xcd * ((npb + 7) >> 3) + slot / ncb;
  if (pblk >= npb) return;

  const int half = wave & 1;
  const int ccn = p.cin_s >> 5;
  const int cc2n = p.cin_s >> 6;
  const int n_st = p.kh * p.kw * cc2n;
  const long zero_off = reinterpret_cast<const unsigned char*>(g_big_zeros) - reinterpret_cast<const unsigned char*>(p.x);
  const u32x4* wsrc[NPC];
  int poff[NPC];
  unsigned vmask[NPC];
  const int csb = PAIR ? p.cin_s / Split<T>::NB : p.cin_s;
  const int xs = PAIR ? Split<T>::NS * csb : p.cin_s;
  const float inv_csb = 1.0f / (float)csb;
  const int kchunk = (lane & 7) ^ (4 * half + (((lane >> 3) >> 1) & 3));
  {
    const int q = lane >> 3;
#pragma unroll
    for (int m = 0; m < NPC; ++m) {
      const int t = (wave >> 1) + (NW / 2) * m;
      wsrc[m] = p.w + (size_t)min(cblk * CT_BLK + t, p.ctiles - 1) * p.ksteps * 64 + half * 64 + lane;
      const int pix = (pblk * PT_BLK + t) * 16 + 8 * half + q;
      const bool v = pix < p.npix;
      const int pc = v ? pix : 0;
      const int ox = pc % p.w_out;
      const int r = pc / p.w_out;
      const int oy = r % p.h_out;
      const int nn = r / p.h_out;
      const int py0 = oy * p.stride - p.pad, px0 = ox * p.stride - p.pad;
      poff[m] = ((nn * p.h_in * p.w_in + py0 * p.w_in + px0) * xs + (PAIR ? 0 : kchunk * 8)) * 2;
      unsigned mk = 0;
      for (int ky = 0; ky < p.kh; ++ky)
        for (int kx = 0; kx < p.kw; ++kx) {
          const bool ok = v && (unsigned)(py0 + ky * p.dil) < (unsigned)p.h_in && (unsigned)(px0 + kx * p.dil) < (unsigned)p.w_in;
          mk |= (ok ? 1u : 0u) << (ky * p.kw + kx);
        }
      vmask[m] = mk;
// ... 106 lines not shown
  };
  auto next_slots = [&]() {
    rw = (rw + 1 == NSW) ? 0 : rw + 1;
    rx = (rx + 1 == NSX) ? 0 : rx + 1;
  };

  issue_w_stage();
  issue_x_stage();
  if (n_st > 1) {
    issue_x_stage();
    issue_w_stage();
    asm volatile("s_waitcnt vmcnt(%0)" ::"n"(2 * NPC) : "memory");
  } else {
    asm volatile("s_waitcnt vmcnt(0)" ::: "memory");
  }
  __builtin_amdgcn_s_barrier();
  fetch_half(0, 0, 0, a0, b0);

  for (int s = 0; s < n_st; ++s) {
    const bool more = s + 2 < n_st;
    if (DOUBLE) {
      half_step(a0, b0, a1, b1, true, rw, rx, 1, P1{}, more);
    } else {
      half_step(a0, b0, a0, b0, false, 0, 0, 0, P1{}, more);
      fetch_half(rw, rx, 1, a0, b0);
    }
    if (more) asm volatile("s_waitcnt vmcnt(%0) lgkmcnt(0)" ::"n"(NPC) : "memory");
    else asm volatile("s_waitcnt vmcnt(0) lgkmcnt(0)" ::: "memory");
    __builtin_amdgcn_s_barrier();
    next_slots();
    if (DOUBLE) {
      half_step(a1, b1, a0, b0, true, rw, rx, 0, P2{}, more);
    } else {
      half_step(a0, b0, a0, b0, false, 0, 0, 0, P2{}, more);
      fetch_half(rw, rx, 0, a0, b0);
    }
  }

  constexpr int ROWB = WC * 64 + 16;
  constexpr int PP = NW == 4 ? 4 : 2;
  constexpr int CH = WC * 2;
  static_assert(NW * PP * 16 * ROWB <= 160 * 1024, "epilogue staging does not fit");
  static_assert(WP % PP == 0, "WP must be a multiple of PP");
  asm volatile("s_waitcnt vmcnt(0) lgkmcnt(0)" ::: "memory");
  __builtin_amdgcn_s_barrier();
  unsigned char* stg = smem + wave * (PP * 16 * ROWB);
  const int cout_base = (cblk * CT_BLK + wc * WC) * 16;
  const float* bias_ep = p.bias;
  if (p.stats && (pblk * PT_BLK + wp * WP) * 16 < p.npix) {
    conv_gemm_stats_epilogue<T, WC, WP>(acc, p, cout_base, pblk * (PT_BLK / WP) + wp, j16, g);
    if (p.bias) bias_ep = nullptr;
  }
  if constexpr (!PAIR) {
    conv_gemm_staged_store<T, WC, WP, PP, RES2>(acc, p, stg, (pblk * PT_BLK + wp * WP) * 16, cout_base, bias_ep, lane, j16, g);
    return;
  }
  constexpr int NIT = PP * 16 * CH / 64;
  constexpr int NSB = Split<T>::NS, NCC = Split<T>::NC;
  const int qc = lane % CH, pl0 = lane / CH;
  const int ch = cout_base + qc * 8;
  const bool ch_ok = ch < p.cout_s;
  f32x4 bb0 = (f32x4){0.f, 0.f, 0.f, 0.f}, bb1 = bb0;
  if (bias_ep && ch_ok) {
    bb0 = *reinterpret_cast<const f32x4*>(bias_ep + ch);
    bb1 = *reinterpret_cast<const f32x4*>(bias_ep + ch + 4);
  }
  auto epilogue_pass = [&](auto pass_tag) {
    constexpr int pass = decltype(pass_tag)::value;
#pragma unroll
    for (int tt = 0; tt < PP; ++tt)
#pragma unroll
      for (int c = 0; c < WC; ++c)
        *reinterpret_cast<f32x4*>(stg + (tt * 16 + j16) * ROWB + c * 64 + g * 16) = acc[c][pass * PP + tt];
    asm volatile("s_waitcnt lgkmcnt(0)" ::: "memory");
    const int pix_base = (pblk * PT_BLK + wp * WP + pass * PP) * 16;
    u32x4 rs[NIT][NCC];
    if (p.has_res) {
      __builtin_amdgcn_sched_barrier(0);
#pragma unroll
      for (int it = 0; it < NIT; ++it) {
        const int pix = pix_base + it * (64 / CH) + pl0;
        size_t rpix = (size_t)(pix < p.npix ? pix : 0);
        if (p.res_ups && pix < p.npix) {
          const int ox = pix % p.w_out;
          const int r = pix / p.w_out;
          const int oy = r % p.h_out;
          const int nn = r / p.h_out;
          rpix = ((size_t)nn * (p.h_out >> 1) + (oy >> 1)) * (p.w_out >> 1) + (ox >> 1);
        }
        const uint16_t* rp = p.res + rpix * p.cout_s * NSB + ch;
#pragma unroll
        for (int k = 0; k < NCC; ++k) {
          rs[it][k] = (u32x4){0u, 0u, 0u, 0u};
          if (pix < p.npix && ch_ok) rs[it][k] = *reinterpret_cast<const u32x4*>(rp + k * p.cout_s);
        }
      }
      __builtin_amdgcn_sched_barrier(0);
    }
    __builtin_amdgcn_s_waitcnt(0x0F70);
#pragma unroll
    for (int it = 0; it < NIT; ++it) {
      const int pl = it * (64 / CH) + pl0;
      const int pix = pix_base + pl;
      const f32x4 v0 = *reinterpret_cast<const f32x4*>(stg + pl * ROWB + qc * 32);
      const f32x4 v1 = *reinterpret_cast<const f32x4*>(stg + pl * ROWB + qc * 32 + 16);
      float v[8] = {v0[0], v0[1], v0[2], v0[3], v1[0], v1[1], v1[2], v1[3]};
      if (bias_ep) {
#pragma unroll
        for (int r = 0; r < 4; ++r) {
          v[r] += bb0[r];
          v[4 + r] += bb1[r];
        }
      }
      if (p.has_res) {
        float rsum[8] = {0.f, 0.f, 0.f, 0.f, 0.f, 0.f, 0.f, 0.f};
#pragma unroll
        for (int k = NCC - 1; k >= 0; --k) {
#pragma unroll
          for (int e = 0; e < 4; ++e) {
            float r0, r1;
            unpack2<T>(rs[it][k][e], r0, r1);
            rsum[2 * e] += r0;
            rsum[2 * e + 1] += r1;
          }
        }
#pragma unroll
        for (int r = 0; r < 8; ++r) v[r] += rsum[r];
      }
      act_apply_n(v, p.act, p.slope);
      if (p.cout < p.cout_s) {
#pragma unroll
        for (int r = 0; r < 8; ++r)
          if (ch + r >= p.cout) v[r] = 0.f;
      }
      uint16_t* yp = p.y + (size_t)pix * p.cout_s * NSB + ch;
#pragma unroll
      for (int k = 0; k < NCC; ++k) {
        u32x4 comp;
#pragma unroll
        for (int e = 0; e < 4; ++e) {
          comp[e] = pack2<T>(v[2 * e], v[2 * e + 1]);
          float q0, q1;
          unpack2<T>(comp[e], q0, q1);
          v[2 * e] -= q0;
          v[2 * e + 1] -= q1;
        }
        if (pix < p.npix && ch_ok) *reinterpret_cast<u32x4*>(yp + k * p.cout_s) = comp;
      }
    }
    asm volatile("s_waitcnt lgkmcnt(0)" ::: "memory");
  };
  static_assert(WP / PP == 2, "two staging passes");
  epilogue_pass(std::integral_constant<int, 0>{});
  epilogue_pass(std::integral_constant<int, 1>{});
}

template <typename T, int NW, bool PAIR = false, bool RES2 = false>
int launch_big(const ConvGemmArgs& a, hipStream_t s) {
  constexpr size_t smem = 160 * 1024;
  static bool attr_set = false;
  if (!attr_set) {
    hipError_t e = hipFuncSetAttribute(reinterpret_cast<const void*>(&conv_gemm_big_kernel<T, NW, PAIR, RES2>),
                                       hipFuncAttributeMaxDynamicSharedMemorySize, 160 * 1024);
    if (e != hipSuccess) {
      cgan_set_error("conv_gemm_big: hipFuncSetAttribute failed: %s", hipGetErrorString(e));
      return CGAN_ERR_HIP;
    }
    attr_set = true;
  }
  const int npb = ceil_div(ceil_div(a.npix, 16), 16);
  const int ncb = ceil_div(a.ctiles, 16);
  const int grid = ceil_div(npb, 8) * 8 * ncb;
  hipLaunchKernelGGL((conv_gemm_big_kernel<T, NW, PAIR, RES2>), dim3(grid), dim3(NW * 64), smem, s, a, npb, ncb);
  return CGAN_OK;
}

}

bool conv_gemm_big_ok(const ConvGemmArgs& a) {
  return (a.cin_s & 63) == 0 && a.pad_mode != CGAN_PAD_REFLECT && a.kh * a.kw <= 32 && a.ctiles >= 12 &&
         (long)a.n * a.h_in * a.w_in * a.cin_s < (1L << 30) - (1L << 20);
}

CGAN_KNOB(int, g_big_waves, 8);
CGAN_DEV_ONLY(extern "C" void cgan_debug_set_big_waves(int v) { g_big_waves = v; })

int conv_gemm_big_launch(const ConvGemmArgs& a, int dtype, hipStream_t s) {
  if (g_big_waves == 16 && a.has_res != 3)
    return dtype == CGAN_F16 ? launch_big<F16, 16>(a, s) : launch_big<BF16, 16>(a, s);
  if (a.has_res == 3)
    return dtype == CGAN_F16 ? launch_big<F16, 8, false, true>(a, s) : launch_big<BF16, 8, false, true>(a, s);
  return dtype == CGAN_F16 ? launch_big<F16, 8>(a, s) : launch_big<BF16, 8>(a, s);
}

bool conv_gemm_big_pair_ok(const ConvGemmArgs& a, int dtype) {
  const int nb = cgan_split_blocks(dtype), ns = cgan_split_store_blocks(dtype);
  return (a.cin_s & 63) == 0 && (a.cin_s % nb) == 0 && a.pad_mode != CGAN_PAD_REFLECT && a.kh * a.kw <= 32 && a.ctiles >= 12 &&
         a.npix >= 16384 && a.stats == nullptr &&
         (long)a.n * a.h_in * a.w_in * (a.cin_s / nb) * ns < (1L << 30) - (1L << 20) &&
         (long)a.npix * a.cout_s * ns < (1L << 31);
}
int conv_gemm_big_pair_launch(const ConvGemmArgs& a, int dtype, hipStream_t s) {
  return dtype == CGAN_F16 ? launch_big<F16, 8, true>(a, s) : launch_big<BF16, 8, true>(a, s);
}
```

climategan_amd/csrc/conv_mfma.hip:

```cpp
#include "cgan_common.h"
#include "conv3x3_lds.h"
#include "conv_gemm.h"

namespace {

struct ConvParams {
  const uint16_t* x;
  const u32x4* w;
  const float* bias;
  const uint16_t* res;
  const uint16_t* res2;
  uint16_t* y;
  int n, h_in, w_in, hx, wx, cin_s, cin_p, cg;
  int cout, cout_s, ctiles;
  int kh, kw, stride, pad, dil, pad_mode;
  int h_out, w_out, npix;
  int kgroups, ksteps;
  int in_ups, act, has_res, res_ups;
  int in_zs;
  int cls_s;
  int cls_pad;
  float slope;
  float* stats;
  int pair;
// ... 596 lines not shown
extern "C" int cgan_conv2d_pack_weight(const float* w_oihw, const float* bias, const float* sigma, void* packed,
                                       float* bias_out, const CganConvDesc* d, void* stream) {
  ConvParams p;
  int rc = fill_params(p, d);
  if (rc != CGAN_OK) return rc;
  CGAN_REQUIRE(w_oihw && packed, "conv2d_pack_weight: null pointer");
  const int total = p.ctiles * p.ksteps * 64;
  const int blocks = ceil_div(total, 256) < 2048 ? ceil_div(total, 256) : 2048;
  hipStream_t s = (hipStream_t)stream;
  if (d->dtype == CGAN_F16)
    hipLaunchKernelGGL(pack_conv_weight_kernel<F16>, dim3(blocks), dim3(256), 0, s, w_oihw, bias, sigma,
                       (uint16_t*)packed, bias_out, d->c_out, d->c_in, p.cin_p, d->kh, d->kw, p.ctiles, p.ksteps, 0);
  else
    hipLaunchKernelGGL(pack_conv_weight_kernel<BF16>, dim3(blocks), dim3(256), 0, s, w_oihw, bias, sigma,
                       (uint16_t*)packed, bias_out, d->c_out, d->c_in, p.cin_p, d->kh, d->kw, p.ctiles, p.ksteps, 0);
  CGAN_CHECK_LAUNCH("conv2d_pack_weight");
  return CGAN_OK;
}

extern "C" int cgan_conv2d_pack_weight_batched(const CganPackItem* items_device, int32_t count, int32_t dtype,
                                               int32_t max_fragments, void* stream) {
  CGAN_REQUIRE(items_device && count > 0 && max_fragments > 0, "conv2d_pack_weight_batched: bad arguments");
  CGAN_REQUIRE(dtype == CGAN_F16 || dtype == CGAN_BF16, "conv2d_pack_weight_batched: bad dtype %d", dtype);
  const int blocks = ceil_div(max_fragments, 256) < 512 ? ceil_div(max_fragments, 256) : 512;
  hipStream_t s = (hipStream_t)stream;
  if (dtype == CGAN_F16)
    hipLaunchKernelGGL(pack_conv_weight_batched_kernel<F16>, dim3(blocks, count), dim3(256), 0, s, items_device);
  else
    hipLaunchKernelGGL(pack_conv_weight_batched_kernel<BF16>, dim3(blocks, count), dim3(256), 0, s, items_device);
  CGAN_CHECK_LAUNCH("conv2d_pack_weight_batched");
  return CGAN_OK;
}

#include <mutex>
namespace {
struct WsSlot { int device; void* stream; void* ws; size_t bytes; };
constexpr int WS_SLOTS = 64;
WsSlot g_ws[WS_SLOTS];
int g_ws_n = 0;
int g_ws_next = 0;
std::mutex g_ws_mu;
int ws_device() {
  int dev = 0;
  if (hipGetDevice(&dev) != hipSuccess) dev = 0;
  return dev;
}
WsSlot ws_lookup(void* stream) {
  const int dev = ws_device();
  std::lock_guard<std::mutex> lk(g_ws_mu);
  for (int i = 0; i < g_ws_n; ++i)
    if (g_ws[i].stream == stream && g_ws[i].device == dev) return g_ws[i];
  return WsSlot{dev, stream, nullptr, 0};
}
size_t ws_max_bytes() {
  const int dev = ws_device();
  std::lock_guard<std::mutex> lk(g_ws_mu);
  size_t m = 0;
  for (int i = 0; i < g_ws_n; ++i)
    if (g_ws[i].device == dev && g_ws[i].bytes > m) m = g_ws[i].bytes;
  return m;
}
}

extern "C" int cgan_conv2d_bind_workspace(void* stream, void* workspace, size_t bytes) {
  CGAN_REQUIRE((workspace != nullptr) == (bytes > 0), "conv2d_bind_workspace: workspace and bytes must both be set or both be zero");
  CGAN_REQUIRE((reinterpret_cast<size_t>(workspace) & 15) == 0, "conv2d_bind_workspace: workspace must be 16-byte aligned");
  const int dev = ws_device();
  std::lock_guard<std::mutex> lk(g_ws_mu);
  for (int i = 0; i < g_ws_n; ++i)
    if (g_ws[i].stream == stream && g_ws[i].device == dev) {
      if (workspace == nullptr) {
        g_ws[i] = g_ws[g_ws_n - 1];
        --g_ws_n;
        if (g_ws_next >= g_ws_n) g_ws_next = 0;
      } else {
        g_ws[i].ws = workspace; g_ws[i].bytes = bytes;
      }
      return CGAN_OK;
    }
  if (workspace == nullptr) return CGAN_OK;
  if (g_ws_n < WS_SLOTS) {
    g_ws[g_ws_n++] = WsSlot{dev, stream, workspace, bytes};
  } else {
    g_ws[g_ws_next] = WsSlot{dev, stream, workspace, bytes};
    g_ws_next = (g_ws_next + 1) % WS_SLOTS;
  }
  return CGAN_OK;
}

static int dgrad_desc(const CganConvDesc* f, CganConvDesc* t) {
  CGAN_REQUIRE(f != nullptr, "conv2d bwd_data: null descriptor");
  CGAN_REQUIRE(f->pad_mode == CGAN_PAD_ZERO, "conv2d bwd_data: only zero padding has a backward path");
  CGAN_REQUIRE(f->stride >= 1 && f->dilation >= 1 && f->kh > 0 && f->kw > 0, "conv2d bwd_data: bad kernel params");
  *t = *f;
  t->c_in = f->c_out; t->c_out = f->c_in;
  t->h_in = (f->h_out - 1) * f->stride + 1;
  t->w_in = (f->w_out - 1) * f->stride + 1;
  t->stride = 1;
  t->pad = f->dilation * (f->kh - 1) - f->pad;
  CGAN_REQUIRE(f->kh == f->kw, "conv2d bwd_data: square kernels only");
  t->h_out = t->h_in + 2 * t->pad - f->dilation * (f->kh - 1);
  t->w_out = t->w_in + 2 * t->pad - f->dilation * (f->kw - 1);
  CGAN_REQUIRE(t->h_out <= f->h_in && t->w_out <= f->w_in && t->h_out > 0 && t->w_out > 0,
               "conv2d bwd_data: inconsistent forward descriptor");
  t->in_upsample = 0; t->act = CGAN_ACT_NONE; t->has_bias = 0; t->has_residual = 0; t->residual_upsample = 0;
  return CGAN_OK;
// ... 1 lines not shown

static bool dgrad_subpixel(const CganConvDesc* f) {
  return g_conv_force == 0 && f->kh == 4 && f->kw == 4 && f->stride == 2 && f->pad == 1 && f->dilation == 1 &&
         f->pad_mode == CGAN_PAD_ZERO && f->c_in <= 4 && !f->in_upsample && (cgan_cs(f->c_out) % 32) == 0 &&
         (f->h_in % 2) == 0 && (f->w_in % 2) == 0 && (long)f->h_out * f->w_out >= 1024;
}

template <typename T>
__global__ void pack_dgrad_subpixel_kernel(const float* __restrict__ w, const float* __restrict__ sigma,
                                           uint16_t* __restrict__ packed, int c_out, int c_in, int cin_p) {
  const int nq = cin_p / 32, total = 9 * nq * 64;
  const float sig = sigma ? sigma[0] : 1.f;
  for (int idx = blockIdx.x * blockDim.x + threadIdx.x; idx < total; idx += gridDim.x * blockDim.x) {
    const int lane = idx & 63, ks = idx >> 6;
    const int tap = ks / nq, q = ks - tap * nq;
    const int ty = tap / 3, tx = tap - ty * 3;
    const int row = lane & 15, a = row >> 3, b = (row >> 2) & 1, c = row & 3;
    const int ky = a + 3 - 2 * ty, kx = b + 3 - 2 * tx;
    const int k0 = q * 32 + (lane >> 4) * 8;
    uint16_t o[8];
#pragma unroll
    for (int e = 0; e < 8; ++e) {
      const int co = k0 + e;
      float v = 0.f;
      if (co < c_out && c < c_in && ky >= 0 && ky < 4 && kx >= 0 && kx < 4)
        v = __fdiv_rn(w[(((size_t)co * c_in + c) * 4 + ky) * 4 + kx], sig);
      o[e] = bits_of<T>(v);
    }
    u32x4 pk;
    pk[0] = o[0] | ((uint32_t)o[1] << 16);
    pk[1] = o[2] | ((uint32_t)o[3] << 16);
    pk[2] = o[4] | ((uint32_t)o[5] << 16);
    pk[3] = o[6] | ((uint32_t)o[7] << 16);
    reinterpret_cast<u32x4*>(packed)[idx] = pk;
  }
}

namespace {
enum ConvRoute {
  ROUTE_GEMM,
  ROUTE_SPLITK,
  ROUTE_LDS3X3,
  ROUTE_SMALLCIN,
  ROUTE_SUBPIXEL,
  ROUTE_CLS_GEMM,
  ROUTE_PAIR_BIG,
  ROUTE_PAIR_GEMM,
  ROUTE_GENERAL,
};
enum { FWD_PLAIN, FWD_STATS, FWD_PAIR };
enum { RES_NONE = 0, RES_ADD = 1, RES_RELU = 2, RES_ADD_RELU = 3 };

struct ConvPlan {
  ConvRoute route;
  ConvParams p;
  CganConvDesc d;
  int ksplit;
  float* ws;
};

ConvGemmArgs gemm_args(const ConvParams& p) {
  ConvGemmArgs a;
  a.x = p.x; a.w = p.w; a.bias = p.bias; a.res = p.res; a.res2 = p.res2; a.y = p.y;
  a.n = p.n; a.h_in = p.h_in; a.w_in = p.w_in; a.cin_s = p.cin_s;
  a.cout = p.cout; a.cout_s = p.cout_s; a.ctiles = p.ctiles; a.ksteps = p.ksteps;
  a.kh = p.kh; a.kw = p.kw; a.stride = p.stride; a.pad = p.pad; a.dil = p.dil; a.pad_mode = p.pad_mode;
  a.h_out = p.h_out; a.w_out = p.w_out; a.npix = p.npix;
  a.act = p.act; a.has_res = p.has_res; a.res_ups = p.res_ups; a.slope = p.slope;
  a.stats = p.stats;
  return a;
}

Conv3x3LdsArgs lds_args(const ConvPlan& pl) {
  const ConvParams& p = pl.p;
  Conv3x3LdsArgs a;
  a.x = p.x; a.w = p.w; a.bias = p.bias; a.res = p.res; a.y = p.y;
  a.n = p.n; a.h = p.h_out; a.w_ = p.w_out; a.hi = p.h_in; a.wi = p.w_in; a.pad = p.pad;
  a.reflect = p.pad_mode == CGAN_PAD_REFLECT;
  a.hx = p.hx; a.wx = p.wx; a.cin = pl.d.c_in; a.cin_s = p.cin_s; a.cin_p = p.cin_p;
  a.cout = p.cout; a.cout_s = p.cout_s; a.ctiles = p.ctiles; a.ksteps = p.ksteps;
  a.in_ups = p.in_ups; a.act = p.act; a.has_res = p.has_res; a.res_ups = p.res_ups; a.slope = p.slope;
  a.shuffle = 0; a.shuffle_w = 0; a.k = 0; a.stride = 0;
  if (pl.route == ROUTE_SMALLCIN) {
    a.k = p.kh; a.stride = p.stride; a.res_ups = 0;
  } else if (pl.route == ROUTE_SUBPIXEL) {
    a.h = a.hi = p.hx; a.w_ = a.wi = p.wx; a.pad = 1; a.slope = 0.f;
    a.cout = 16; a.cout_s = 16; a.ctiles = 1; a.ksteps = 9 * (a.cin_p / 32);
    a.shuffle = p.h_out; a.shuffle_w = p.w_out;
  }
  return a;
}

void cls_table(const ConvParams& p, ConvGemmCls (&cls)[4]) {
  int koff = 0;
  for (int c = 0; c < p.cls_s * p.cls_s; ++c) {
    const int ca = c / p.cls_s, cb = c % p.cls_s;
    int ry, rx, nty, ntx;
    cls_axis(p.cls_s, p.kh, p.cls_pad, ca, ry, nty);
    cls_axis(p.cls_s, p.kw, p.cls_pad, cb, rx, ntx);
    cls[c] = ConvGemmCls{koff, nty, ntx, (ca - p.cls_pad + ry) / p.cls_s, (cb - p.cls_pad + rx) / p.cls_s};
    if (nty * ntx == 0) cls[c].kh = cls[c].kw = 0;
    koff += cls_ksteps(p.cls_s, p.kh, p.kw, p.cls_pad, p.cg, c);
  }
}

ConvRoute route_stride1(ConvPlan& pl, bool stats, const WsSlot& ws) {
  const ConvParams& p = pl.p;
  const CganConvDesc* d = &pl.d;
  const bool lds = conv3x3_lds_applicable(d);
  const bool prefer_3x3 = lds && p.cin_s < 256 && g_conv_force != 3;
  if ((g_conv_force == 0 || g_conv_force == 3) && !prefer_3x3 && conv_gemm_applicable(d)) return ROUTE_GEMM;
  ConvRoute r = ROUTE_GENERAL;
  if (g_conv_force != 1 && lds) r = ROUTE_LDS3X3;
  else if (g_conv_force == 0 && conv_smallcin_applicable(d)) r = ROUTE_SMALLCIN;
  if ((r == ROUTE_GENERAL || (r == ROUTE_LDS3X3 && p.cin_s >= 256)) && g_conv_force == 0 && !stats && !p.in_ups &&
      p.cin_p == p.cin_s) {
    const ConvGemmArgs a = gemm_args(p);
    const int ks = conv_gemm_splitk_plan(a);
    if (ks > 1 && conv_gemm_splitk_workspace_bytes(a, ks) <= ws.bytes) {
      pl.ksplit = ks;
      pl.ws = (float*)ws.ws;
      return ROUTE_SPLITK;
    }
  }
  return r;
}

int plan_fwd(ConvPlan& pl, const CganConvDesc* d, int mode, const WsSlot& ws) {
  ConvParams& p = pl.p;
  int rc = fill_params(p, d);
  if (rc != CGAN_OK) return rc;
  pl.d = *d; pl.ksplit = 1; pl.ws = nullptr;
  if (mode != FWD_PAIR) {
    pl.route = route_stride1(pl, mode == FWD_STATS, ws);
    return CGAN_OK;
  }
  const int nb = cgan_split_blocks(d->dtype), ns = cgan_split_store_blocks(d->dtype);
  CGAN_REQUIRE((d->c_in % (8 * nb)) == 0, "conv2d_nhwc_fwd_pair: c_in must be the %d * round_up(C, 8) storage channels of a split map", nb);
  CGAN_REQUIRE((double)p.npix * p.cout_s * ns * 2.0 < 4294967295.0, "conv2d_nhwc_fwd_pair: output map of 4 GiB or more");
  p.pair = 1;
  p.csb = p.cin_s / nb;
  p.xs = ns * p.csb;
  pl.route = ROUTE_GENERAL;
  if (g_conv_force == 0 && !p.in_ups && p.cin_p == p.cin_s && p.npix >= 1024 && p.ksteps >= 4) {
    const ConvGemmArgs a = gemm_args(p);
    if (g_pair_big && conv_gemm_big_pair_ok(a, d->dtype)) pl.route = ROUTE_PAIR_BIG;
    else if (conv_gemm_ext_shape_ok(a) && (double)p.npix * p.cout_s * ns < 2147483647.0) pl.route = ROUTE_PAIR_GEMM;
  }
  return CGAN_OK;
}

int plan_dgrad(ConvPlan& pl, const CganConvDesc* f, int res_mode, const WsSlot& ws) {
  ConvParams& p = pl.p;
  CganConvDesc& t = pl.d;
  int rc = dgrad_desc(f, &t);
  if (rc != CGAN_OK) return rc;
  const int pad_t = t.pad;
  if (pad_t < 0) {
    t.pad = 0;
    t.h_out = t.h_in; t.w_out = t.w_in;
  }
  rc = fill_params(p, &t);
  if (rc != CGAN_OK) return rc;
  pl.ksplit = 1; pl.ws = nullptr;
  t.pad = p.pad = pad_t;
  t.h_out = p.h_out = f->h_in; t.w_out = p.w_out = f->w_in;
  p.npix = f->n * f->h_in * f->w_in;
  p.hx = f->h_out; p.wx = f->w_out;
  p.in_zs = f->stride;
  if (f->stride > 1 && f->dilation == 1 && pad_t >= 0 && g_dgrad_zero_insert == 0) {
    p.cls_s = f->stride; p.cls_pad = pad_t; p.in_zs = 1;
    p.h_in = p.hx; p.w_in = p.wx;
  }
  const bool plain = f->stride == 1 && pad_t >= 0 && t.h_in + 2 * pad_t - t.dilation * (t.kh - 1) == t.h_out &&
                     t.w_in + 2 * pad_t - t.dilation * (t.kw - 1) == t.w_out;
  if (res_mode != RES_NONE) {
    CGAN_REQUIRE(plain, "conv2d_nhwc_bwd_data_add / _relu: only for stride-1 'same' convolutions");
    p.has_res = res_mode == RES_ADD_RELU ? RES_ADD : res_mode;
    p.res_ups = 0;
    t.has_residual = 1;
  }
  if (plain) {
    pl.route = route_stride1(pl, false, ws);
    if (res_mode == RES_ADD_RELU && pl.route == ROUTE_GEMM && conv_gemm_res2_ok(gemm_args(p), t.dtype)) p.has_res = 3;
  } else if (dgrad_subpixel(f)) {
    pl.route = ROUTE_SUBPIXEL;
  } else if (p.cls_s && p.cls_s <= 2 && g_conv_force == 0 && p.cin_p == p.cin_s && conv_gemm_ext_shape_ok(gemm_args(p)) &&
             p.cout_s >= 64) {
    pl.route = ROUTE_CLS_GEMM;
  } else {
    pl.route = ROUTE_GENERAL;
  }
  return CGAN_OK;
}

int route_family(ConvRoute r) {
  switch (r) {
    case ROUTE_GENERAL: return CGAN_CONV_KERNEL_GENERAL;
    case ROUTE_LDS3X3: case ROUTE_SMALLCIN: case ROUTE_SUBPIXEL: return CGAN_CONV_KERNEL_LDS3X3;
    default: return CGAN_CONV_KERNEL_GEMM;
  }
}

int stats_chunk_pixels(const ConvPlan& pl) {
  const CganConvDesc& d = pl.d;
  if (pl.route != ROUTE_GEMM || d.has_residual || d.act != CGAN_ACT_NONE || d.in_upsample) return 0;
  static const float bias_present = 0.f;
  ConvGemmArgs a = gemm_args(pl.p);
  a.bias = d.has_bias ? &bias_present : nullptr;
  return conv_gemm_stats_chunk_pixels(a, d.dtype);
}

int launch_plan(const ConvPlan& pl, hipStream_t s, const char* what) {
  const ConvParams& p = pl.p;
  const int dt = pl.d.dtype;
  int rc = CGAN_OK;
  switch (pl.route) {
    case ROUTE_GEMM: rc = conv_gemm_launch(gemm_args(p), dt, s); break;
    case ROUTE_SPLITK: rc = conv_gemm_splitk_launch(gemm_args(p), pl.ksplit, pl.ws, dt, s); break;
    case ROUTE_LDS3X3: case ROUTE_SUBPIXEL: rc = conv3x3_lds_launch(lds_args(pl), dt, s); break;
    case ROUTE_SMALLCIN: rc = conv_smallcin_launch(lds_args(pl), dt, s); break;
    case ROUTE_CLS_GEMM: {
      ConvGemmCls cls[4];
      cls_table(p, cls);
      rc = conv_gemm_cls_launch(gemm_args(p), p.cls_s, cls, dt, s);
      break;
    }
    case ROUTE_PAIR_BIG: rc = conv_gemm_big_pair_launch(gemm_args(p), dt, s); break;
    case ROUTE_PAIR_GEMM: rc = conv_gemm_pair_launch(gemm_args(p), dt, s); break;
    case ROUTE_GENERAL:
      if (dt == CGAN_F16) launch<F16>(p, s);
      else launch<BF16>(p, s);
      break;
  }
  if (rc != CGAN_OK) return rc;
  CGAN_CHECK_LAUNCH(what);
  return CGAN_OK;
}

void bind(ConvParams& p, const void* x, const void* w, const float* bias, const void* res, void* y) {
  p.x = (const uint16_t*)x; p.w = (const u32x4*)w; p.bias = bias; p.res = (const uint16_t*)res; p.y = (uint16_t*)y;
}
}

extern "C" int cgan_conv2d_nhwc_fwd(const void* x, const void* packed_w, const float* bias_padded, const void* residual,
                                    void* y, const CganConvDesc* d, void* stream) {
  CGAN_REQUIRE(x && packed_w && y, "conv2d_nhwc_fwd: null pointer");
  ConvPlan pl;
  int rc = plan_fwd(pl, d, FWD_PLAIN, ws_lookup(stream));
  if (rc != CGAN_OK) return rc;
  CGAN_REQUIRE(!d->has_bias || bias_padded, "conv2d_nhwc_fwd: has_bias but bias is null");
  CGAN_REQUIRE(!d->has_residual || residual, "conv2d_nhwc_fwd: has_residual but residual is null");
  bind(pl.p, x, packed_w, d->has_bias ? bias_padded : nullptr, residual, y);
  return launch_plan(pl, (hipStream_t)stream, "conv2d_nhwc_fwd");
}

extern "C" int cgan_conv2d_nhwc_fwd_pair(const void* x3, const void* packed_w3, const float* bias_padded,
                                         const void* residual3, void* y3, const CganConvDesc* d, void* stream) {
  CGAN_REQUIRE(x3 && packed_w3 && y3, "conv2d_nhwc_fwd_pair: null pointer");
  ConvPlan pl;
  int rc = plan_fwd(pl, d, FWD_PAIR, WsSlot{});
  if (rc != CGAN_OK) return rc;
  CGAN_REQUIRE(!d->has_bias || bias_padded, "conv2d_nhwc_fwd_pair: has_bias but bias is null");
  CGAN_REQUIRE(!d->has_residual || residual3, "conv2d_nhwc_fwd_pair: has_residual but residual is null");
  bind(pl.p, x3, packed_w3, d->has_bias ? bias_padded : nullptr, residual3, y3);
  return launch_plan(pl, (hipStream_t)stream, "conv2d_nhwc_fwd_pair");
}

extern "C" int32_t cgan_conv2d_stats_chunk_pixels(const CganConvDesc* d) {
  ConvPlan pl;
  if (plan_fwd(pl, d, FWD_STATS, WsSlot{}) != CGAN_OK) return 0;
// ... 47 lines not shown
  const ConvParams& p = pl.p;
  const CganConvDesc& t = pl.d;
  hipStream_t s = (hipStream_t)stream;
  if (pl.route == ROUTE_SUBPIXEL) {
    const int cin_p = lds_args(pl).cin_p;
    const int tot = 9 * (cin_p / 32) * 64;
    if (fwd->dtype == CGAN_F16)
      hipLaunchKernelGGL(pack_dgrad_subpixel_kernel<F16>, dim3(ceil_div(tot, 256)), dim3(256), 0, s, w_oihw, sigma,
                         (uint16_t*)packed, fwd->c_out, fwd->c_in, cin_p);
    else
      hipLaunchKernelGGL(pack_dgrad_subpixel_kernel<BF16>, dim3(ceil_div(tot, 256)), dim3(256), 0, s, w_oihw, sigma,
                         (uint16_t*)packed, fwd->c_out, fwd->c_in, cin_p);
  } else if (p.cls_s) {
    int max_ks = 1;
    for (int c = 0; c < p.cls_s * p.cls_s; ++c) {
      const int k = cls_ksteps(p.cls_s, p.kh, p.kw, p.cls_pad, p.cg, c);
      max_ks = k > max_ks ? k : max_ks;
    }
    const int tot = p.ctiles * max_ks * 64;
    const dim3 grid(ceil_div(tot, 256) < 1024 ? ceil_div(tot, 256) : 1024, p.cls_s * p.cls_s);
    if (fwd->dtype == CGAN_F16)
      hipLaunchKernelGGL(pack_dgrad_classes_kernel<F16>, grid, dim3(256), 0, s, w_oihw, sigma, (uint16_t*)packed, t.c_out,
                         t.c_in, p.cin_p, t.kh, t.kw, p.ctiles, p.cls_s, p.cls_pad);
    else
      hipLaunchKernelGGL(pack_dgrad_classes_kernel<BF16>, grid, dim3(256), 0, s, w_oihw, sigma, (uint16_t*)packed, t.c_out,
                         t.c_in, p.cin_p, t.kh, t.kw, p.ctiles, p.cls_s, p.cls_pad);
  } else {
    const int total = p.ctiles * p.ksteps * 64;
    const int blocks = ceil_div(total, 256) < 2048 ? ceil_div(total, 256) : 2048;
    if (fwd->dtype == CGAN_F16)
      hipLaunchKernelGGL(pack_conv_weight_kernel<F16>, dim3(blocks), dim3(256), 0, s, w_oihw, (const float*)nullptr, sigma,
                         (uint16_t*)packed, (float*)nullptr, t.c_out, t.c_in, p.cin_p, t.kh, t.kw, p.ctiles, p.ksteps, 1);
    else
      hipLaunchKernelGGL(pack_conv_weight_kernel<BF16>, dim3(blocks), dim3(256), 0, s, w_oihw, (const float*)nullptr, sigma,
                         (uint16_t*)packed, (float*)nullptr, t.c_out, t.c_in, p.cin_p, t.kh, t.kw, p.ctiles, p.ksteps, 1);
  }
  CGAN_CHECK_LAUNCH("conv2d_pack_weight_dgrad");
  return CGAN_OK;
}

static int kernel_kind_impl(const CganConvDesc* d, int32_t bwd_data, const WsSlot& ws) {
  ConvPlan pl;
  const int rc = bwd_data ? plan_dgrad(pl, d, RES_NONE, ws) : plan_fwd(pl, d, FWD_PLAIN, ws);
  return rc != CGAN_OK ? rc : route_family(pl.route);
}

extern "C" int cgan_conv2d_kernel_kind_on(const CganConvDesc* d, int32_t bwd_data, void* stream) {
  return kernel_kind_impl(d, bwd_data, ws_lookup(stream));
}
extern "C" int cgan_conv2d_kernel_kind(const CganConvDesc* d, int32_t bwd_data) {
  return kernel_kind_impl(d, bwd_data, WsSlot{0, nullptr, nullptr, ws_max_bytes()});
}

static int bwd_data_impl(const void* dy, const void* packed_w_dgrad, const void* res, const void* relu_out, void* dx,
                         const CganConvDesc* fwd, void* stream, int res_mode) {
  CGAN_REQUIRE(dy && packed_w_dgrad && dx, "conv2d_nhwc_bwd_data: null pointer");
  ConvPlan pl;
  int rc = plan_dgrad(pl, fwd, res_mode, ws_lookup(stream));
  if (rc != CGAN_OK) return rc;
  bind(pl.p, dy, packed_w_dgrad, nullptr, res, dx);
  if (pl.p.has_res == 3) pl.p.res2 = (const uint16_t*)relu_out;
  rc = launch_plan(pl, (hipStream_t)stream, "conv2d_nhwc_bwd_data");
  if (rc != CGAN_OK || res_mode != RES_ADD_RELU || pl.p.has_res == 3) return rc;
  return cgan_act_bwd(relu_out, dx, dx, fwd->dtype, CGAN_ACT_RELU, 0.f,
                      (int64_t)fwd->n * fwd->h_in * fwd->w_in * cgan_cs(fwd->c_in), stream);
}

extern "C" int cgan_conv2d_nhwc_bwd_data(const void* dy, const void* packed_w_dgrad, void* dx, const CganConvDesc* fwd,
                                         void* stream) {
  return bwd_data_impl(dy, packed_w_dgrad, nullptr, nullptr, dx, fwd, stream, RES_NONE);
}

extern "C" int cgan_conv2d_nhwc_bwd_data_relu(const void* dy, const void* packed_w_dgrad, const void* relu_out, void* dx,
                                              const CganConvDesc* fwd, void* stream) {
  CGAN_REQUIRE(relu_out != nullptr, "conv2d_nhwc_bwd_data_relu: null pointer");
  return bwd_data_impl(dy, packed_w_dgrad, relu_out, nullptr, dx, fwd, stream, RES_RELU);
}

extern "C" int cgan_conv2d_nhwc_bwd_data_add_relu(const void* dy, const void* packed_w_dgrad, const void* dx_add,
                                                  const void* relu_out, void* dx, const CganConvDesc* fwd, void* stream) {
  CGAN_REQUIRE(dx_add != nullptr && relu_out != nullptr, "conv2d_nhwc_bwd_data_add_relu: null pointer");
  return bwd_data_impl(dy, packed_w_dgrad, dx_add, relu_out, dx, fwd, stream, RES_ADD_RELU);
}

extern "C" int cgan_conv2d_nhwc_bwd_data_add(const void* dy, const void* packed_w_dgrad, const void* dx_add, void* dx,
                                             const CganConvDesc* fwd, void* stream) {
  CGAN_REQUIRE(dx_add != nullptr, "conv2d_nhwc_bwd_data_add: null pointer");
  return bwd_data_impl(dy, packed_w_dgrad, dx_add, nullptr, dx, fwd, stream, RES_ADD);
}
```

climategan_amd/csrc/train_ops.hip:

```cpp
#include "cgan_common.h"

namespace {

__host__ __device__ inline int grid_for_n(long total) {
  long g = (total + 255) / 256;
  return (int)(g < 1 ? 1 : (g > 8192 ? 8192 : g));
}

__device__ __forceinline__ float act_grad_from_out(float out, int act, float slope) {
  switch (act) {
    case CGAN_ACT_RELU: return out > 0.f ? 1.f : 0.f;
    case CGAN_ACT_LRELU: return out > 0.f ? 1.f : slope;
    case CGAN_ACT_TANH: return 1.f - out * out;
    case CGAN_ACT_SIGMOID: return out * (1.f - out);
    default: return 1.f;
  }
}

template <typename T>
__global__ void act_bwd_kernel(const uint16_t* __restrict__ out, const uint16_t* dy, uint16_t* dx, int act, float slope,
                               long groups) {
  for (long i = (long)blockIdx.x * blockDim.x + threadIdx.x; i < groups; i += (long)gridDim.x * blockDim.x) {
    const u32x4 o = CGAN_LD_STREAM(reinterpret_cast<const u32x4*>(out) + i);
    const u32x4 g = CGAN_LD_STREAM(reinterpret_cast<const u32x4*>(dy) + i);
// ... 373 lines not shown
    float a = 0.f, b = 0.f;
    for (int k0 = kl; k0 < chunks; k0 += 256) {
      float2 v[8];
#pragma unroll
      for (int j = 0; j < 8; ++j) {
        const int k = k0 + 32 * j;
        v[j] = k < chunks ? *reinterpret_cast<const float2*>(rows + (size_t)k * cs * 2) : make_float2(0.f, 0.f);
      }
#pragma unroll
      for (int j = 0; j < 8; ++j) {
        a += v[j].x;
        b += v[j].y;
      }
    }
#pragma unroll
    for (int off = 32; off >= 8; off >>= 1) {
      a += __shfl_down(a, off, 64);
      b += __shfl_down(b, off, 64);
    }
    if (lane < 8) {
      red[grp][wave][chl][0] = a;
      red[grp][wave][chl][1] = b;
    }
  }
  __syncthreads();
  if (threadIdx.x >= 8) return;
  float dg_sum = 0.f, db_sum = 0.f;
  for (int grp = 0; grp < groups; ++grp) {
    float s1 = 0.f, s2 = 0.f;
#pragma unroll
    for (int w = 0; w < 4; ++w) {
      s1 += red[grp][w][chl][0];
      s2 += red[grp][w][chl][1];
    }
    float A = 0.f, B = 0.f, C = 0.f;
    if (ch < c) {
      dg_sum += s2;
      db_sum += s1;
      const float rs = rstd[ch], mu = mean[ch];
      A = rs * (gamma ? gamma[ch] : 1.f);
      const float m1 = s1 * inv_count, m2 = s2 * inv_count;
      B = -A * rs * m2;
      C = A * (mu * rs * m2 - m1);
    }
    coef[ch] = A;
    coef[cs + ch] = B;
    coef[2 * cs + ch] = C;
    mean += cs; rstd += cs; coef += 3 * (size_t)cs;
  }
  if (ch < c) {
    if (dgamma) dgamma[ch] = dg_sum;
    if (dbeta) dbeta[ch] = db_sum;
  }
}

template <typename T, int MASK>
__global__ __launch_bounds__(256) void bn_bwd_apply_kernel(const uint16_t* __restrict__ x, const uint16_t* __restrict__ out,
                                                           const uint16_t* __restrict__ dy, const float* __restrict__ coef,
                                                           const float* __restrict__ fmean, const float* __restrict__ frstd,
                                                           uint16_t* __restrict__ dx, uint16_t* __restrict__ dz_out,
                                                           long npix, int cs, float gneg) {
  const int cg_total = cs / 8;
  const int tpp = cg_total < 256 ? cg_total : 256;
  const int rows = 256 / tpp;
  const int cgl = threadIdx.x % tpp, prow = threadIdx.x / tpp;
  if (prow >= rows) return;
  {
    const size_t gofs = (size_t)blockIdx.y * npix * cs;
    x += gofs; dy += gofs; dx += gofs;
    if (MASK == 1) out += gofs;
    if (dz_out) dz_out += gofs;
    coef += (size_t)blockIdx.y * 3 * cs;
    if (MASK == 2) { fmean += (size_t)blockIdx.y * cs; frstd += (size_t)blockIdx.y * cs; }
  }
  for (int cg = cgl; cg < cg_total; cg += tpp) {
    float A[8], B[8], Cc[8], fm[8], fr[8];
#pragma unroll
    for (int e = 0; e < 8; ++e) {
      A[e] = coef[cg * 8 + e];
      B[e] = coef[cs + cg * 8 + e];
      Cc[e] = coef[2 * cs + cg * 8 + e];
      fm[e] = MASK == 2 ? fmean[cg * 8 + e] : 0.f;
      fr[e] = MASK == 2 ? frstd[cg * 8 + e] : 0.f;
    }
#pragma unroll 2
    for (long p = (long)blockIdx.x * rows + prow; p < npix; p += (long)gridDim.x * rows) {
      const size_t off = (size_t)p * cs + cg * 8;
      const u32x4 vx = CGAN_LD_STREAM(reinterpret_cast<const u32x4*>(x + off));
      u32x4 vo = {0, 0, 0, 0};
      if (MASK == 1) vo = CGAN_LD_STREAM(reinterpret_cast<const u32x4*>(out + off));
      const u32x4 vg = CGAN_LD_STREAM(reinterpret_cast<const u32x4*>(dy + off));
      u32x4 r, z;
#pragma unroll
      for (int e = 0; e < 4; ++e) {
        float xv[2], ov[2], gv[2], res[2], dzv[2];
        unpack2<T>(vx[e], xv[0], xv[1]);
        unpack2<T>(vo[e], ov[0], ov[1]);
        unpack2<T>(vg[e], gv[0], gv[1]);
#pragma unroll
        for (int hh = 0; hh < 2; ++hh) {
          const int k = 2 * e + hh;
          dzv[hh] = gv[hh] * bn_bwd_act_grad<MASK>(ov[hh], xv[hh], fm[k], fr[k], gneg);
          res[hh] = A[k] * dzv[hh] + B[k] * xv[hh] + Cc[k];
        }
        r[e] = pack2<T>(res[0], res[1]);
        z[e] = pack2<T>(dzv[0], dzv[1]);
// ... 177 lines not shown
  CGAN_REQUIRE(out || act == CGAN_ACT_NONE || (fold_mean && fold_rstd),
               "batchnorm_act_bwd: without out the activation mask needs fold_mean / fold_rstd");
  CGAN_REQUIRE(dtype == CGAN_F16 || dtype == CGAN_BF16, "batchnorm_act_bwd: bad dtype %d", dtype);
  CGAN_REQUIRE(groups >= 1 && groups <= 16 && npix_total > 0 && c > 0 && npix_total % groups == 0,
               "batchnorm_act_bwd: bad shape (the pixel count must divide into the groups)");
  CGAN_REQUIRE(act == CGAN_ACT_NONE || act == CGAN_ACT_RELU || act == CGAN_ACT_LRELU,
               "batchnorm_act_bwd: Unsupported activation: %d", act);
  CGAN_REQUIRE(workspace_bytes >= (size_t)groups * cgan_batchnorm_act_bwd_workspace_bytes(c),
               "batchnorm_act_bwd: workspace too small");
  const long npix = npix_total / groups;
  const int cs = cgan_cs(c);
  hipStream_t s = (hipStream_t)stream;
  float* coef = (float*)workspace;
  float* partial = coef + (size_t)groups * 3 * cs;
  const int cg_total = cs / 8;
  const int cgb = cg_total < 256 ? cg_total : 256;
  const int PL = 256 / cgb;
  const int cgblocks = ceil_div(cg_total, cgb);
  long chunks = BN_BWD_MAX_CHUNKS / cgblocks;
  if (chunks < 1) chunks = 1;
  long ppb = (npix + chunks - 1) / chunks;
  if (ppb < 8 * PL) ppb = 8 * PL;
  chunks = (npix + ppb - 1) / ppb;
  const size_t smem = (size_t)PL * cgb * 8 * 2 * sizeof(float);
  const int mask = act == CGAN_ACT_NONE ? 0 : (out ? 1 : 2);
  const float gneg = act == CGAN_ACT_RELU ? 0.f : act_slope;
  uint16_t* dz_early = (mask == 1 && dz_out && act == CGAN_ACT_RELU) ? (uint16_t*)dz_out : nullptr;
#define BN_BWD_REDUCE(M)                                                                                              \
  DISPATCH_T2(dtype, bn_bwd_reduce_kernel, M, dim3((unsigned)chunks, cgblocks, groups), dim3(256), smem, s,           \
              (const uint16_t*)x, (const uint16_t*)out, (const uint16_t*)dy, batch_mean, batch_rstd, fold_mean,       \
              fold_rstd, partial, dz_early, (long)npix, cs, (int)ppb, gneg)
  if (mask == 0) { BN_BWD_REDUCE(0); } else if (mask == 1) { BN_BWD_REDUCE(1); } else { BN_BWD_REDUCE(2); }
#undef BN_BWD_REDUCE
  hipLaunchKernelGGL(bn_bwd_finalize_kernel, dim3(cs / 8), dim3(256), 0, s, (const float*)partial, (int)chunks,
                     batch_mean, batch_rstd, gamma, 1.f / (float)npix, coef, dgamma, dbeta, (int)c, cs, (int)groups);
  const int tpp = cg_total < 256 ? cg_total : 256;
  const int rows = 256 / tpp;
  long blocks = (npix + (long)rows * 4 - 1) / ((long)rows * 4);
  blocks = blocks < 1 ? 1 : (blocks > 4096 / groups ? 4096 / groups : blocks);
#define BN_BWD_APPLY(M)                                                                                               \
  DISPATCH_T2(dtype, bn_bwd_apply_kernel, M, dim3((unsigned)blocks, groups), dim3(256), 0, s, (const uint16_t*)x,     \
              (const uint16_t*)out, (const uint16_t*)dy, (const float*)coef, fold_mean, fold_rstd, (uint16_t*)dx,     \
              (uint16_t*)dz_out, (long)npix, cs, gneg)
  if (dz_early) {
    DISPATCH_T2(dtype, bn_bwd_apply_kernel, 0, dim3((unsigned)blocks, groups), dim3(256), 0, s, (const uint16_t*)x,
                (const uint16_t*)nullptr, (const uint16_t*)dz_early, (const float*)coef, fold_mean, fold_rstd,
                (uint16_t*)dx, (uint16_t*)nullptr, (long)npix, cs, gneg);
  } else if (mask == 0) { BN_BWD_APPLY(0); } else if (mask == 1) { BN_BWD_APPLY(1); } else { BN_BWD_APPLY(2); }
#undef BN_BWD_APPLY
  CGAN_CHECK_LAUNCH("batchnorm_act_bwd");
  return CGAN_OK;
}

extern "C" int cgan_spectral_norm_bwd(float* grad_w, const float* w_bar, const float* u, const float* v,
                                      const float* sigma, int32_t rows, int32_t cols, float* workspace,
                                      void* stream) {
  CGAN_REQUIRE(grad_w && w_bar && u && v && sigma && workspace, "spectral_norm_bwd: null pointer");
  CGAN_REQUIRE(rows > 0 && cols > 0, "spectral_norm_bwd: bad shape");
  hipStream_t s = (hipStream_t)stream;
  const long numel = (long)rows * cols;
  int g = grid_for_n(numel);
  if (g > SN_BWD_ROWS) g = SN_BWD_ROWS;
  hipLaunchKernelGGL(sn_bwd_dot_kernel, dim3(g), dim3(256), 0, s, (const float*)grad_w, w_bar, workspace, numel);
  hipLaunchKernelGGL(sn_bwd_apply_kernel, dim3(grid_for_n(numel)), dim3(256), 0, s, grad_w, u, v, sigma,
                     (const float*)workspace, g, cols, numel);
  CGAN_CHECK_LAUNCH("spectral_norm_bwd");
  return CGAN_OK;
}
```

climategan_amd/deeplab/resnet101_v3.py:

```python
import torch.nn as nn

from .. import functional as Fn
from .. import ops
from ..norms import DEFAULT_COMPUTE_DTYPE, _PackCache, conv_bn_forward, needs_grad


FUSE_RESIDUAL_GRADIENT = True


class Bottleneck(nn.Module):
    expansion = 4

    def __init__(self, inplanes, planes, stride=1, dilation=1, downsample=None, BatchNorm=None):
        super().__init__()
        self.conv1 = nn.Conv2d(inplanes, planes, kernel_size=1, bias=False)
        self.bn1 = BatchNorm(planes)
        self.conv2 = nn.Conv2d(planes, planes, kernel_size=3, stride=stride, dilation=dilation, padding=dilation,
                               bias=False)
        self.bn2 = BatchNorm(planes)
        self.conv3 = nn.Conv2d(planes, planes * 4, kernel_size=1, bias=False)
        self.bn3 = BatchNorm(planes * 4)
        self.relu = nn.ReLU(inplace=True)
        self.downsample = downsample
        self.stride = stride
        self.dilation = dilation
        self._c = [_PackCache() for _ in range(4)]

    def forward_nhwc(self, x, sole_consumer=False):
        residual = x
        if FUSE_RESIDUAL_GRADIENT and self.bn1.training and needs_grad(self, x.t):
            out, residual = conv_bn_forward(self.conv1, self.bn1, self._c[0], x, act=ops.ACT_RELU, passthrough=True,
                                            sole_consumer=sole_consumer)
            x = residual
        else:
            out = conv_bn_forward(self.conv1, self.bn1, self._c[0], x, act=ops.ACT_RELU)
        out = conv_bn_forward(self.conv2, self.bn2, self._c[1], out, act=ops.ACT_RELU)
        if self.downsample is not None:
            residual = conv_bn_forward(self.downsample[0], self.downsample[1], self._c[3], x)
        return conv_bn_forward(self.conv3, self.bn3, self._c[2], out, act=ops.ACT_RELU, residual=residual)


class ResNet(nn.Module):

    def __init__(self, block, layers, output_stride, BatchNorm, verbose=0, no_init=False):
        self.inplanes = 64
        self.verbose = verbose
        super().__init__()
        blocks = [1, 2, 4]
        if output_stride == 16:
            strides, dilations = [1, 2, 2, 1], [1, 1, 1, 2]
        elif output_stride == 8:
            strides, dilations = [1, 2, 1, 1], [1, 1, 2, 4]
        else:
            raise NotImplementedError
        self.conv1 = nn.Conv2d(3, 64, kernel_size=7, stride=2, padding=3, bias=False)
        self.bn1 = BatchNorm(64)
        self.relu = nn.ReLU(inplace=True)
        self.maxpool = nn.MaxPool2d(kernel_size=3, stride=2, padding=1)
        self.layer1 = self._make_layer(block, 64, layers[0], strides[0], dilations[0], BatchNorm)
        self.layer2 = self._make_layer(block, 128, layers[1], strides[1], dilations[1], BatchNorm)
        self.layer3 = self._make_layer(block, 256, layers[2], strides[2], dilations[2], BatchNorm)
        self.layer4 = self._make_MG_unit(block, 512, blocks, strides[3], dilations[3], BatchNorm)
        self.compute_dtype = DEFAULT_COMPUTE_DTYPE
        self.pair_precision = False
        self._stem = _PackCache()

    def _downsample(self, block, planes, stride, BatchNorm):
        if stride != 1 or self.inplanes != planes * block.expansion:
            return nn.Sequential(nn.Conv2d(self.inplanes, planes * block.expansion, kernel_size=1, stride=stride, bias=False),
                                 BatchNorm(planes * block.expansion))
        return None

    def _make_layer(self, block, planes, blocks, stride=1, dilation=1, BatchNorm=None):
        layers = [block(self.inplanes, planes, stride, dilation, self._downsample(block, planes, stride, BatchNorm), BatchNorm)]
        self.inplanes = planes * block.expansion
        for _ in range(1, blocks):
            layers.append(block(self.inplanes, planes, dilation=dilation, BatchNorm=BatchNorm))
        return nn.Sequential(*layers)

    def _make_MG_unit(self, block, planes, blocks, stride=1, dilation=1, BatchNorm=None):
        layers = [block(self.inplanes, planes, stride, dilation=blocks[0] * dilation,
                        downsample=self._downsample(block, planes, stride, BatchNorm), BatchNorm=BatchNorm)]
        self.inplanes = planes * block.expansion
        for i in range(1, len(blocks)):
            layers.append(block(self.inplanes, planes, stride=1, dilation=blocks[i] * dilation, BatchNorm=BatchNorm))
        return nn.Sequential(*layers)

    def forward_nhwc(self, x: ops.NHWC):
        x = conv_bn_forward(self.conv1, self.bn1, self._stem, x, act=ops.ACT_RELU)
        x = Fn.maxpool3x3s2(x)
        sole = False
        for b in self.layer1:
# ... 23 lines not shown
```

climategan_amd/norms.py:

```python
import torch
import torch.nn as nn

from . import ops

DEFAULT_COMPUTE_DTYPE = torch.float16


def _grad_guard(module: nn.Module):
    if torch.is_grad_enabled() and any(p.requires_grad for p in module.parameters()):
        raise NotImplementedError(
            "climategan_amd: only the forward (inference) path is implemented in HIP so far; call under "
            "torch.no_grad() (the reference's infer_all does, trainer.py:217) or set requires_grad=False")


def needs_grad(module: nn.Module, *tensors) -> bool:
    if not torch.is_grad_enabled():
        return False
    return any(t is not None and t.requires_grad for t in tensors) or any(p.requires_grad for p in module.parameters())


def _conv_train(x: ops.NHWC, weight, bias, packed, sn, stride, pad, dilation, kw) -> ops.NHWC:
    from .autograd import ConvFn

    pad_mode = kw.get("pad_mode", ops.PAD_ZERO)
    if pad_mode == ops.PAD_REFLECT and kw.get("in_upsample"):
        raise NotImplementedError("climategan_amd: reflect padding on a folded upsample has no backward kernel")
    res = kw.get("residual")
    cfg = dict(c_in=x.c, stride=stride, pad=pad, dilation=dilation, act=kw.get("act", ops.ACT_NONE),
               slope=kw.get("slope", 0.2), in_upsample=bool(kw.get("in_upsample", False)),
               residual_upsample=bool(kw.get("residual_upsample", False)), pad_mode=pad_mode,
               sn_owned=bool(kw.get("sn_owned", False)), pair_in=bool(kw.get("pair_in", False)),
               want_stats=bool(kw.get("want_stats", False)))
    y_t = ConvFn.apply(x.t, weight, bias, res.t if res is not None else None, packed, cfg, sn)
    if kw.get("want_stats"):
        return ops.NHWC(y_t, weight.shape[0]), cfg.get("stats_out")
    return ops.NHWC(y_t, weight.shape[0])


class _PackCache:

    _plain = {}

    def __init__(self):
        self.key = None
        self.value = None
        self._plain_src = None

    @staticmethod
    def _key_of(params, dtype):
        return tuple((p.data_ptr(), p._version, p.dtype, str(p.device)) if torch.is_tensor(p) else p
                     for p in params if p is not None) + (dtype,)

    def get(self, params, dtype, build):
        key = self._key_of(params, dtype)
        if key != self.key:
            self.value = build()
            self.key = key
        return self.value

    def get_plain(self, weight, bias, dtype):
        import weakref

        key = self._key_of((weight, bias, "plain"), dtype)
        if key == self.key:
            return self.value
        self._plain_src = (weakref.ref(weight), weakref.ref(bias) if bias is not None else None, dtype)
        _PackCache._plain[id(self)] = weakref.ref(self)
        _PackCache.repack_stale(dtype, weight.device)
        return self.value

    @staticmethod
    def repack_stale(dtype, device) -> int:
        self = _PackCache
        stale = []
        for cid, ref in list(_PackCache._plain.items()):
            c = ref()
            src = c._plain_src if c is not None else None
            w = src[0]() if src is not None else None
            if c is None or w is None:
                del _PackCache._plain[cid]
                continue
            b = src[1]() if src[1] is not None else None
            if src[2] != dtype or w.device != device:
                continue
            k = self._key_of((w, b, "plain"), dtype)
# ... 92 lines not shown
        pw = self.packed(x.t.dtype)
        pad = conv_kwargs.pop("pad", m.padding[0])
        if self.trainable and needs_grad(self, x.t):
            snap, self._sn_snapshot = self._sn_snapshot, None
            if self._pre_used and snap is not None:
                sn = snap
                conv_kwargs = dict(conv_kwargs, sn_owned=True)
            else:
                sn = (self._sigma, getattr(m, self.name + "_u").data, getattr(m, self.name + "_v").data)
            return _conv_train(x, getattr(m, self.name + "_bar"), m.bias, pw, sn, m.stride[0], pad, m.dilation[0],
                               conv_kwargs)
        return ops.conv2d(x, pw, stride=m.stride[0], pad=pad, dilation=m.dilation[0], **conv_kwargs)


class PlainConv(nn.Module):

    def __init__(self, conv: nn.Conv2d):
        super().__init__()
        self.conv = conv
        self._cache = _PackCache()

    def packed(self, dtype):
        c = self.conv
        return self._cache.get((c.weight, c.bias), dtype,
                               lambda: ops.pack_conv_weight(c.weight.data, c.bias.data if c.bias is not None else None,
                                                            dtype))


def conv_forward(conv: nn.Module, cache: _PackCache, x: ops.NHWC, **kw) -> ops.NHWC:
    if isinstance(conv, SpectralNorm):
        return conv(x, **kw)
    trainable = kw.pop("trainable", False)
    if not trainable:
        _grad_guard(conv)
    if trainable and needs_grad(conv, x.t):
        pw = cache.get_plain(conv.weight, conv.bias, x.t.dtype)
        return _conv_train(x, conv.weight, conv.bias, pw, None, conv.stride[0], conv.padding[0], conv.dilation[0], kw)
    pair = isinstance(x, ops.PairMap)
    pw = cache.get((conv.weight, conv.bias) + (("pair",) if pair else ()), x.t.dtype,
                   lambda: ops.pack_conv_weight(conv.weight.data, conv.bias.data if conv.bias is not None else None,
                                                x.t.dtype, pair=pair))
    if trainable and needs_grad(conv, x.t):
        return _conv_train(x, conv.weight, conv.bias, pw, None, conv.stride[0], conv.padding[0], conv.dilation[0], kw)
    return ops.conv2d(x, pw, stride=conv.stride[0], pad=conv.padding[0], dilation=conv.dilation[0], **kw)


FUSE_BN_RESIDUAL = True
import os as _os
FUSE_BN_STATS = _os.environ.get("CGAN_FUSE_BN_STATS", "1") != "0"
FUSE_RELU_MASK = _os.environ.get("CGAN_FUSE_RELU_MASK", "1") != "0"


def conv_bn_forward(conv: nn.Conv2d, bn, cache: _PackCache, x: ops.NHWC, pad_mode=ops.PAD_ZERO, pad=None, **kw) -> ops.NHWC:
    train_bn = bn is not None and bn.training
    grad = needs_grad(conv, x.t) or (bn is not None and needs_grad(bn))
    p = conv.padding[0] if pad is None else pad
    if not train_bn and not grad:
        pair = isinstance(x, ops.PairMap)

        def build():
            if bn is None:
                return ops.pack_conv_weight(conv.weight.data, conv.bias.data if conv.bias is not None else None, x.t.dtype,
                                            pair=pair)
            w, b = ops.fold_bn(conv.weight.data, conv.bias.data if conv.bias is not None else None,
                               bn.weight.data if bn.affine else None, bn.bias.data if bn.affine else None,
                               bn.running_mean, bn.running_var, bn.eps)
            return ops.pack_conv_weight(w, b, x.t.dtype, pair=pair)

        params = [conv.weight, conv.bias]
        if bn is not None:
            params += [bn.weight, bn.bias, bn.running_mean, bn.running_var]
        if pair:
            params = params + ["pair"]
        pw = cache.get(params, x.t.dtype, build)
        return ops.conv2d(x, pw, stride=conv.stride[0], pad=p, dilation=conv.dilation[0], pad_mode=pad_mode, **kw)

    if bn is not None and not bn.training:
        raise NotImplementedError("climategan_amd: an eval-mode BatchNorm under autograd has no HIP backward (the "
                                  "reference trains with BatchNorm in training mode)")
    from .autograd import BatchNormActFn

    act, slope, residual = kw.pop("act", ops.ACT_NONE), kw.pop("slope", 0.2), kw.pop("residual", None)
    sole_consumer = kw.pop("sole_consumer", False)
    if kw.get("in_upsample") or kw.get("residual_upsample"):
        raise NotImplementedError("conv_bn_forward: folded upsamples are not used on the training path")
    pw = cache.get_plain(conv.weight, conv.bias, x.t.dtype)
    passthrough = None
    if kw.pop("passthrough", False):
        from .autograd import ConvPassFn

        assert bn is not None and residual is None
        pcfg = dict(c_in=x.c, stride=conv.stride[0], pad=p, dilation=conv.dilation[0], pad_mode=pad_mode, want_stats=FUSE_BN_STATS)
        if sole_consumer and FUSE_RELU_MASK:
            from .autograd import claim_relu_mask
            pcfg["mask_input"] = claim_relu_mask(x.t)
        y_t, pass_t = ConvPassFn.apply(x.t, conv.weight, conv.bias, pw, pcfg)
        y, passthrough = ops.NHWC(y_t, conv.weight.shape[0]), ops.NHWC(pass_t, x.c)
        conv_stats = pcfg.get("stats_out")
    if bn is None:
        return _conv_train(x, conv.weight, conv.bias, pw, None, conv.stride[0], p, conv.dilation[0],
                           dict(act=act, slope=slope, residual=residual, pad_mode=pad_mode))
    if passthrough is None:
        conv_stats = None
        if FUSE_BN_STATS:
            y, conv_stats = _conv_train(x, conv.weight, conv.bias, pw, None, conv.stride[0], p, conv.dilation[0],
                                        dict(pad_mode=pad_mode, want_stats=True))
        else:
            y = _conv_train(x, conv.weight, conv.bias, pw, None, conv.stride[0], p, conv.dilation[0], dict(pad_mode=pad_mode))
    if residual is not None and not FUSE_BN_RESIDUAL:
        from . import functional as Fn
        out_t = BatchNormActFn.apply(y.t, bn.weight if bn.affine else None, bn.bias if bn.affine else None,
                                     bn.running_mean, bn.running_var, y.c, bn.eps,
                                     bn.momentum if bn.momentum is not None else 0.1, ops.ACT_NONE, slope,
                                     bn.num_batches_tracked if bn.track_running_stats else None)
        return Fn.add_act(ops.NHWC(out_t, y.c), residual, act, slope)
    if residual is not None and (residual.c != y.c or residual.t.shape != y.t.shape):
        raise ValueError("conv_bn_forward: residual %s does not match the conv output %s"
                         % (tuple(residual.t.shape), tuple(y.t.shape)))
    out_t = BatchNormActFn.apply(y.t, bn.weight if bn.affine else None, bn.bias if bn.affine else None, bn.running_mean,
                                 bn.running_var, y.c, bn.eps, bn.momentum if bn.momentum is not None else 0.1, act,
                                 slope, bn.num_batches_tracked if bn.track_running_stats else None,
                                 residual.t if residual is not None else None, conv_stats)
    return ops.NHWC(out_t, y.c) if passthrough is None else (ops.NHWC(out_t, y.c), passthrough)


class SPADE(nn.Module):

    def __init__(self, param_free_norm_type, kernel_size, norm_nc, cond_nc):
        super().__init__()
        if param_free_norm_type == "instance":
            self.param_free_norm = nn.InstanceNorm2d(norm_nc, affine=False)
        elif param_free_norm_type == "batch":
            self.param_free_norm = nn.BatchNorm2d(norm_nc, affine=False)
        else:
            raise ValueError("%s is not a recognized param-free norm type in SPADE" % param_free_norm_type)
        self.param_free_norm_type = param_free_norm_type
        nhidden = 128
        pw = kernel_size // 2
        self.mlp_shared = nn.Sequential(nn.Conv2d(cond_nc, nhidden, kernel_size=kernel_size, padding=pw), nn.ReLU())
        self.mlp_gamma = nn.Conv2d(nhidden, norm_nc, kernel_size=kernel_size, padding=pw)
        self.mlp_beta = nn.Conv2d(nhidden, norm_nc, kernel_size=kernel_size, padding=pw)
        self.kernel_size = kernel_size
        self._cache = _PackCache()

    def packed(self, dtype) -> ops.PackedSpade:
        ps = (self.mlp_shared[0].weight, self.mlp_shared[0].bias, self.mlp_gamma.weight, self.mlp_gamma.bias,
              self.mlp_beta.weight, self.mlp_beta.bias)
        return self._cache.get(ps, dtype, lambda: ops.pack_spade_weights(*[p.data for p in ps], dtype))

    def forward_nhwc(self, x: ops.NHWC, cond: ops.NHWC, stats=None, act=ops.ACT_NONE, x_upsample=False) -> ops.NHWC:
        if self.kernel_size != 3:
            raise NotImplementedError("SPADE: only kernel_size 3 is supported")
        if isinstance(x, ops.PairMap):
            return self._forward_pair(x, cond, stats, act, x_upsample)
        batch_stats = False
        if self.param_free_norm_type == "batch":
            bn = self.param_free_norm
            if bn.training:
                from . import autograd as _ag
                if _ag.BN_GROUPS != 1:
                    raise NotImplementedError("SPADE with a batch param-free norm inside autograd.bn_groups(%d): run the "
# ... 90 lines not shown
```

climategan_amd/ops.py:

```python
import collections
import ctypes as C
import functools
import inspect
import os
from dataclasses import dataclass
from typing import Optional, Tuple

import torch

from . import _lib
from ._lib import (ACT_LRELU, ACT_NONE, ACT_RELU, ACT_SIGMOID, ACT_TANH, CGAN_BF16, CGAN_F16, PAD_REFLECT,
                   PAD_ZERO, ConvDesc, NormStatsDesc, PackItem, SnItem, SpadeDesc)

_DT = {torch.float16: CGAN_F16, torch.bfloat16: CGAN_BF16}


def touch(*tensors) -> None:
    ts = [t for t in tensors if t is not None]
    if ts:
        torch.autograd.graph.increment_version(ts)


MAX_MAP_BYTES = 2 ** 31
ABI_MAX_BYTES = 2 ** 31
# ... 981 lines not shown

@dataclass
class ConvStats:
    partial: torch.Tensor
    chunk_pixels: int


def conv2d_with_stats(x: NHWC, pw: PackedConv, stride=1, pad=0, dilation=1, pad_mode=PAD_ZERO, groups: int = 1):
    _need_cuda(x.t)
    _need_cs8("conv2d", x)
    if x.c != pw.c_in:
        raise RuntimeError("conv2d: input has %d channels, weight expects %d" % (x.c, pw.c_in))
    if x.t.dtype != pw.dtype:
        raise RuntimeError("conv2d: activation dtype %s != packed weight dtype %s" % (x.t.dtype, pw.dtype))
    d = _conv_desc(x.dtype_id, x.n, x.h, x.w, pw.c_in, pw.c_out, pw.kh, pw.kw, stride, pad, dilation, pad_mode,
                   has_bias=pw.has_bias)
    lib = _lib.load()
    ppb = lib.cgan_conv2d_stats_chunk_pixels(C.byref(d))
    npix = x.n * d.h_out * d.w_out
    if ppb <= 0 or x.n % groups or (npix // groups) % ppb:
        return conv2d(x, pw, stride=stride, pad=pad, dilation=dilation, pad_mode=pad_mode), None
    y = _empty((x.n, d.h_out, d.w_out, cs8(pw.c_out)), dtype=x.t.dtype, device=x.t.device)
    partial = _empty((npix // ppb, cs8(pw.c_out), 2), dtype=torch.float32, device=x.t.device)
    _lib.check(lib.cgan_conv2d_nhwc_fwd_stats(_ptr(x.t), _ptr(pw.w), _ptr(pw.bias), _ptr(y), _ptr(partial),
                                              partial.numel() * 4, C.byref(d), _stream()), "cgan_conv2d_nhwc_fwd_stats")
    return NHWC(y, pw.c_out), ConvStats(partial, ppb)


def batchnorm_train_stats_from_partials(st: ConvStats, groups: int, pix_per_group: int, c: int, gamma, beta, running_mean,
                                        running_var, num_batches_tracked, eps, momentum):
    lib = _lib.load()
    cs = st.partial.shape[1]
    d = NormStatsDesc(CGAN_BF16, groups, pix_per_group, c, float(eps))
    stats = _empty((4, groups, cs), dtype=torch.float32, device=st.partial.device)
    _lib.check(lib.cgan_batchnorm_train_stats_from_partials(
        _ptr(st.partial), int(st.chunk_pixels), _ptr(gamma), _ptr(beta), float(momentum), _ptr(running_mean),
        _ptr(running_var), _ptr(num_batches_tracked), _ptr(stats[0]), _ptr(stats[1]), _ptr(stats[2]), _ptr(stats[3]),
        C.byref(d), _stream()), "cgan_batchnorm_train_stats_from_partials")
    touch(running_mean, running_var, num_batches_tracked)
    return stats[0], stats[1], stats[2], stats[3]


@_batch_chunked("dxp")
def reflect_pad_bwd(dxp: NHWC, pad: int) -> NHWC:
    _need_cuda(dxp.t)
    h, w = dxp.h - 2 * pad, dxp.w - 2 * pad
    dx = _empty((dxp.n, h, w, dxp.cs), dtype=dxp.t.dtype, device=dxp.t.device)
    lib = _lib.load()
    _lib.check(lib.cgan_reflect_pad_bwd_nhwc(_ptr(dxp.t), _ptr(dx), dxp.dtype_id, dxp.n, dxp.c, h, w, int(pad), _stream()),
               "cgan_reflect_pad_bwd_nhwc")
    return NHWC(dx, dxp.c)


def conv2d_bwd_data(dy: NHWC, w: torch.Tensor, x_shape, stride=1, pad=0, dilation=1,
                    sigma: Optional[torch.Tensor] = None, pad_mode=PAD_ZERO, add: Optional[NHWC] = None,
                    prepacked: Optional[DgradPack] = None, relu_out: Optional[NHWC] = None) -> NHWC:
    same = stride == 1 and pad_mode == PAD_ZERO and 2 * pad == dilation * (w.shape[2] - 1) and w.shape[2] == w.shape[3]
    if relu_out is not None:
        if not same:
            dx = conv2d_bwd_data(dy, w, x_shape, stride, pad, dilation, sigma, pad_mode, add=add, prepacked=prepacked)
            return act_bwd(relu_out, dx, ACT_RELU)
    per_sample = max(dy.t.nbytes // max(dy.n, 1), (x_shape[1] + 2 * pad) * (x_shape[2] + 2 * pad) * cs8(w.shape[1]) * 2)
    if x_shape[0] * per_sample >= MAX_MAP_BYTES:
        k = (MAX_MAP_BYTES - 1) // per_sample
        if k < 1:
            raise RuntimeError("conv2d_bwd_data: ONE sample's map exceeds the 2 GiB a C-ABI call covers")
        return _run_chunks(x_shape[0], k, lambda lo, cnt: conv2d_bwd_data(
            NHWC(dy.t[lo:lo + cnt], dy.c), w, (cnt, x_shape[1], x_shape[2]), stride, pad, dilation, sigma, pad_mode,
            NHWC(add.t[lo:lo + cnt], add.c) if add is not None else None, prepacked,
            NHWC(relu_out.t[lo:lo + cnt], relu_out.c) if relu_out is not None else None))
    if add is not None and not same:
        dx = conv2d_bwd_data(dy, w, x_shape, stride, pad, dilation, sigma, pad_mode, prepacked=prepacked)
        return NHWC(dx.t + add.t, dx.c)
    if pad_mode == PAD_REFLECT and pad > 0:
        n, h_in, w_in = x_shape
        dxp = conv2d_bwd_data(dy, w, (n, h_in + 2 * pad, w_in + 2 * pad), stride=stride, pad=0, dilation=dilation,
                              sigma=sigma, prepacked=prepacked)
        return reflect_pad_bwd(dxp, pad)
    _need_cuda(dy.t, w, sigma)
    _need_cs8("conv2d_bwd_data", dy)
    w = w.detach().contiguous().float()
    c_out, c_in, kh, kw = w.shape
    n, h_in, w_in = x_shape
    d = _conv_desc(dy.dtype_id, n, h_in, w_in, c_in, c_out, kh, kw, stride, pad, dilation, PAD_ZERO, has_bias=False)
    if (d.h_out, d.w_out) != (dy.h, dy.w) or dy.c != c_out or dy.n != n:
        raise RuntimeError("conv2d_bwd_data: dy shape %s does not match the forward conv" % (tuple(dy.t.shape),))
    lib = _lib.load()
    nbytes = lib.cgan_conv2d_dgrad_packed_weight_bytes(C.byref(d))
    if nbytes == 0:
        _lib.check(-1, "cgan_conv2d_dgrad_packed_weight_bytes")
    if (prepacked is not None and prepacked.packed is not None and stride == 1 and prepacked.dtype == dy.t.dtype
            and prepacked.packed.numel() == nbytes and tuple(prepacked.w.shape) == tuple(w.shape)):
        packed = prepacked.packed
    else:
        packed = _empty(nbytes, dtype=torch.uint8, device=w.device)
        _lib.check(lib.cgan_conv2d_pack_weight_dgrad(_ptr(w), _ptr(sigma), _ptr(packed), C.byref(d), _stream()),
                   "cgan_conv2d_pack_weight_dgrad")
    dx = _empty((n, h_in, w_in, cs8(c_in)), dtype=dy.t.dtype, device=dy.t.device)
    _conv_ws()
    if relu_out is not None:
        if relu_out.t.shape != dx.shape or relu_out.t.dtype != dx.dtype or not relu_out.t.is_contiguous():
            raise RuntimeError("conv2d_bwd_data: ``relu_out`` %s does not match dx %s" % (tuple(relu_out.t.shape), tuple(dx.shape)))
        if add is not None:
            if add.t.shape != dx.shape or add.t.dtype != dx.dtype or not add.t.is_contiguous():
                raise RuntimeError("conv2d_bwd_data: ``add`` %s does not match dx %s" % (tuple(add.t.shape), tuple(dx.shape)))
            _lib.check(lib.cgan_conv2d_nhwc_bwd_data_add_relu(_ptr(dy.t), _ptr(packed), _ptr(add.t), _ptr(relu_out.t), _ptr(dx),
                                                              C.byref(d), _stream()), "cgan_conv2d_nhwc_bwd_data_add_relu")
            return NHWC(dx, c_in)
        _lib.check(lib.cgan_conv2d_nhwc_bwd_data_relu(_ptr(dy.t), _ptr(packed), _ptr(relu_out.t), _ptr(dx), C.byref(d), _stream()),
                   "cgan_conv2d_nhwc_bwd_data_relu")
        return NHWC(dx, c_in)
    if add is not None:
        if add.t.shape != dx.shape or add.t.dtype != dx.dtype or not add.t.is_contiguous():
            raise RuntimeError("conv2d_bwd_data: ``add`` %s does not match dx %s" % (tuple(add.t.shape), tuple(dx.shape)))
        _lib.check(lib.cgan_conv2d_nhwc_bwd_data_add(_ptr(dy.t), _ptr(packed), _ptr(add.t), _ptr(dx), C.byref(d), _stream()),
                   "cgan_conv2d_nhwc_bwd_data_add")
        return NHWC(dx, c_in)
    _lib.check(lib.cgan_conv2d_nhwc_bwd_data(_ptr(dy.t), _ptr(packed), _ptr(dx), C.byref(d), _stream()),
               "cgan_conv2d_nhwc_bwd_data")
    return NHWC(dx, c_in)


@_batch_chunked("x")
def sumpool2x2(x: NHWC) -> NHWC:
    _need_cuda(x.t)
    if x.h % 2 or x.w % 2 or x.cs != cs8(x.c):
        raise RuntimeError("sumpool2x2: even extent and round_up(c, 8) storage expected")
    y = _empty((x.n, x.h // 2, x.w // 2, x.cs), dtype=x.t.dtype, device=x.t.device)
    lib = _lib.load()
    _lib.check(lib.cgan_sumpool2x2_nhwc(_ptr(x.t), _ptr(y), x.dtype_id, x.n, x.c, x.h // 2, x.w // 2, _stream()),
               "cgan_sumpool2x2_nhwc")
    return NHWC(y, x.c)


class ZeroArena:

    def __init__(self, numel: int, device):
        self.buf = torch.zeros(int(numel), dtype=torch.float32, device=device)
        self.off = 0

    def take(self, n: int):
        n_al = (n + 63) // 64 * 64
        if self.off + n_al > self.buf.numel():
            return None
        t = self.buf[self.off:self.off + n]
        self.off += n_al
        return t


_ZERO_ARENA = None


# ... 782 lines not shown
```

include/climategan_hip.h:

```cpp
#ifndef CLIMATEGAN_HIP_H
#define CLIMATEGAN_HIP_H

#include <stddef.h>
#include <stdint.h>

#ifdef __cplusplus
extern "C" {
#endif

#define CGAN_ABI_VERSION 1

typedef enum {
  CGAN_OK = 0,
  CGAN_ERR_BAD_ARG = -1,
  CGAN_ERR_UNSUPPORTED = -2,
  CGAN_ERR_WORKSPACE = -3,
  CGAN_ERR_HIP = -4
} cgan_status_t;

typedef enum { CGAN_F16 = 0, CGAN_BF16 = 1, CGAN_F32 = 2  } cgan_dtype_t;
typedef enum { CGAN_ACT_NONE = 0, CGAN_ACT_RELU = 1, CGAN_ACT_LRELU = 2, CGAN_ACT_TANH = 3, CGAN_ACT_SIGMOID = 4 } cgan_act_t;
typedef enum { CGAN_PAD_ZERO = 0, CGAN_PAD_REFLECT = 1 } cgan_pad_t;

static inline int cgan_cs(int c) { return (c + 7) & ~7; }
// ... 2 lines not shown
const char* cgan_last_error(void);

typedef struct {
  int32_t dtype;
  int32_t n, h_in, w_in;
  int32_t c_in, c_out;
  int32_t kh, kw, stride, pad, dilation;
  int32_t pad_mode;
  int32_t h_out, w_out;
  int32_t in_upsample;
  int32_t act;
  float act_slope;
  int32_t has_bias;
  int32_t has_residual;
  int32_t residual_upsample;
} CganConvDesc;

size_t cgan_conv2d_packed_weight_bytes(const CganConvDesc* d);
int cgan_conv2d_pack_weight(const float* w_oihw, const float* bias, const float* sigma, void* packed,
                            float* bias_out, const CganConvDesc* d, void* stream);
int cgan_conv2d_nhwc_fwd(const void* x, const void* packed_w, const float* bias_padded, const void* residual,
                         void* y, const CganConvDesc* d, void* stream);
typedef struct {
  const float* w_oihw;
  const float* bias;
  const float* sigma;
  void* packed;
  float* bias_out;
  int32_t c_out, c_in, kh, kw;
  int32_t transposed;
} CganPackItem;
int cgan_conv2d_pack_weight_batched(const CganPackItem* items_device, int32_t count, int32_t dtype,
                                    int32_t max_fragments, void* stream);

int32_t cgan_conv2d_stats_chunk_pixels(const CganConvDesc* d);
int cgan_conv2d_nhwc_fwd_stats(const void* x, const void* packed_w, const float* bias_padded, void* y, float* partial,
                               size_t partial_bytes, const CganConvDesc* d, void* stream);

enum { CGAN_CONV_KERNEL_GENERAL = 0, CGAN_CONV_KERNEL_LDS3X3 = 1, CGAN_CONV_KERNEL_GEMM = 2 };
int cgan_conv2d_bind_workspace(void* stream, void* workspace, size_t bytes);
int cgan_conv2d_kernel_kind(const CganConvDesc* d, int32_t bwd_data);
int cgan_conv2d_kernel_kind_on(const CganConvDesc* d, int32_t bwd_data, void* stream);
size_t cgan_conv2d_dgrad_packed_weight_bytes(const CganConvDesc* fwd);
int cgan_conv2d_pack_weight_dgrad(const float* w_oihw, const float* sigma, void* packed, const CganConvDesc* fwd,
                                  void* stream);
int cgan_conv2d_nhwc_bwd_data(const void* dy, const void* packed_w_dgrad, void* dx, const CganConvDesc* fwd,
                              void* stream);
int cgan_conv2d_nhwc_bwd_data_add(const void* dy, const void* packed_w_dgrad, const void* dx_add, void* dx,
                                  const CganConvDesc* fwd, void* stream);
int cgan_conv2d_nhwc_bwd_data_relu(const void* dy, const void* packed_w_dgrad, const void* relu_out, void* dx,
                                   const CganConvDesc* fwd, void* stream);
int cgan_conv2d_nhwc_bwd_data_add_relu(const void* dy, const void* packed_w_dgrad, const void* dx_add, const void* relu_out,
                                       void* dx, const CganConvDesc* fwd, void* stream);
size_t cgan_conv2d_bwd_weight_workspace_bytes(const CganConvDesc* fwd);
int cgan_conv2d_nhwc_bwd_weight(const void* x, const void* dy, float* dw_oihw, float* dbias, const CganConvDesc* fwd,
                                void* workspace, size_t workspace_bytes,
                                void* stream);

typedef struct {
  int32_t dtype;
  int32_t n, hw, c;
  float eps;
} CganNormStatsDesc;
size_t cgan_instnorm_stats_workspace_bytes(const CganNormStatsDesc* d);
int cgan_instnorm_stats(const void* x, float* mean, float* rstd, const CganNormStatsDesc* d, void* workspace,
                        size_t workspace_bytes, void* stream);
int cgan_norm_act_apply(const void* x, const float* mean, const float* rstd, void* y, const CganNormStatsDesc* d,
                        int32_t act, float act_slope, void* stream);
int cgan_norm_add_act_apply(const void* x, const float* mean, const float* rstd, const void* residual, void* y,
                            const CganNormStatsDesc* d, int32_t act, float act_slope, void* stream);

typedef struct {
  int32_t dtype;
  int32_t n, h, w, c;
  int32_t x_upsample;
  int32_t cond_h, cond_w, cond_c;
  int32_t hidden;
  int32_t ksize;
  int32_t act;
  float act_slope;
} CganSpadeDesc;
static inline int cgan_cond_cs(int c) { return (c + 3) & ~3; }
size_t cgan_spade_packed_weight_bytes(const CganSpadeDesc* d);
int cgan_spade_pack_weights(const float* w_shared, const float* b_shared, const float* w_gamma, const float* b_gamma,
                            const float* w_beta, const float* b_beta, void* packed, const CganSpadeDesc* d,
                            void* stream);
int cgan_spade_fused_fwd(const void* x, const float* mean, const float* rstd, const void* cond, const void* packed,
                         void* y, const CganSpadeDesc* d, void* stream);
int cgan_spade_fused_fwd_train(const void* x, const float* mean, const float* rstd, const void* cond, const void* packed,
                               void* y, void* gamma_out, const CganSpadeDesc* d, void* stream);

size_t cgan_spectral_norm_workspace_bytes(int32_t rows, int32_t cols);
int cgan_spectral_norm_power_iter(const float* w_bar, float* u, float* v, float* sigma, int32_t rows, int32_t cols,
                                  void* workspace, size_t workspace_bytes, void* stream);
typedef struct {
  const float* w_bar;
  float* u;
  float* v;
  float* sigma;
  float* workspace;
  int32_t rows, cols;
} CganSnItem;
int cgan_spectral_norm_power_iter_batched(const CganSnItem* items_device, int32_t count, int32_t max_rows,
                                          int32_t max_cols, void* stream);

typedef struct {
// ... 34 lines not shown
int cgan_resize_nearest_nhwc(const void* x, void* y, int32_t dtype, int32_t n, int32_t c, int32_t h_in, int32_t w_in,
                             int32_t cs_in, int32_t h_out, int32_t w_out, int32_t cs_out, void* stream);
int cgan_avgpool3x3s2_nhwc(const void* x, void* y, int32_t dtype, int32_t n, int32_t c, int32_t h_in, int32_t w_in,
                           void* stream);

int cgan_maxpool3x3s2_nhwc(const void* x, void* y, int32_t dtype, int32_t n, int32_t c, int32_t h_in, int32_t w_in,
                           void* stream);
int cgan_resize_bilinear_nhwc(const void* x, void* y, int32_t dtype, int32_t n, int32_t c, int32_t h_in, int32_t w_in,
                              int32_t h_out, int32_t w_out, int32_t align_corners, void* stream);
int cgan_resize_bicubic_nhwc(const void* x, void* y, int32_t dtype, int32_t n, int32_t c, int32_t h_in, int32_t w_in,
                             int32_t h_out, int32_t w_out, void* stream);
int cgan_sumpool2x2_nhwc(const void* x, void* y, int32_t dtype, int32_t n, int32_t c, int32_t h_out, int32_t w_out,
                         void* stream);
int cgan_reflect_pad_bwd_nhwc(const void* dx_padded, void* dx, int32_t dtype, int32_t n, int32_t c, int32_t h, int32_t w,
                              int32_t pad, void* stream);
int cgan_copy_channels_nhwc(const void* src, void* dst, int64_t npix, int32_t c, int32_t cs_src, int32_t cs_dst,
                            int32_t c_off, void* stream);
int cgan_eltwise_nhwc(const void* a, const void* b, void* y, int32_t dtype, int32_t op, int64_t numel, void* stream);
int cgan_fold_bn(const float* w, const float* bias, const float* gamma, const float* beta, const float* mean,
                 const float* var, float eps, float* w_out, float* b_out, int32_t c_out, int64_t per_out, void* stream);

int cgan_act_bwd(const void* out, const void* dy, void* dx, int32_t dtype, int32_t act, float act_slope,
                 int64_t numel, void* stream);
size_t cgan_instnorm_act_bwd_workspace_bytes(const CganNormStatsDesc* d);
int cgan_instnorm_act_bwd(const void* out, const void* dy, const float* rstd, void* dx, const CganNormStatsDesc* d,
                          int32_t act, float act_slope, void* workspace, size_t workspace_bytes, void* stream);
int cgan_spade_bwd_prepare(const void* dy, const void* y, const void* x, const float* mean, const float* rstd,
                           const void* gamma, void* dgb, void* xhat, void* dxhat, const CganSpadeDesc* d, void* stream);
size_t cgan_spade_hidden_bwd_workspace_bytes(const CganSpadeDesc* d);
int cgan_spade_hidden_bwd(const void* dgb, const void* packed_dgrad_gb, const void* cond_hw, const void* packed_w_shared,
                          const float* bias_shared_padded, float* dw_shared, float* db_shared, void* workspace,
                          size_t workspace_bytes, const CganSpadeDesc* d, void* stream);
int cgan_bn_train_prepare(const float* batch_mean, const float* batch_rstd, const float* gamma, const float* beta,
                          float eps, float momentum, int64_t count, float* running_mean, float* running_var,
                          float* mean_out, float* rstd_out, int64_t* num_batches_tracked, int32_t c, void* stream);
int cgan_batchnorm_train_stats(const void* x, const float* gamma, const float* beta, float momentum, float* running_mean,
                               float* running_var, int64_t* num_batches_tracked, float* batch_mean, float* batch_rstd,
                               float* mean_out, float* rstd_out, const CganNormStatsDesc* d, void* workspace,
                               size_t workspace_bytes, void* stream);
int cgan_batchnorm_train_stats_from_partials(float* partial, int32_t chunk_pixels, const float* gamma,
                                             const float* beta, float momentum, float* running_mean, float* running_var,
                                             int64_t* num_batches_tracked, float* batch_mean, float* batch_rstd,
                                             float* mean_out, float* rstd_out, const CganNormStatsDesc* d, void* stream);
size_t cgan_batchnorm_act_bwd_workspace_bytes(int32_t c);
int cgan_batchnorm_act_bwd(const void* x, const void* out, const void* dy, const float* batch_mean,
                           const float* batch_rstd, const float* gamma, const float* fold_mean, const float* fold_rstd,
                           void* dx, float* dgamma, float* dbeta, void* dz_out, int32_t dtype, int64_t npix, int32_t c,
                           int32_t act, float act_slope, void* workspace, size_t workspace_bytes, void* stream);
int cgan_batchnorm_act_bwd_grouped(const void* x, const void* out, const void* dy, const float* batch_mean,
                                   const float* batch_rstd, const float* gamma, const float* fold_mean,
                                   const float* fold_rstd, void* dx, float* dgamma, float* dbeta, void* dz_out,
                                   int32_t dtype, int64_t npix_total, int32_t c, int32_t groups, int32_t act,
                                   float act_slope, void* workspace, size_t workspace_bytes, void* stream);
int cgan_bce_logits_nhwc(const void* x, int32_t dtype, int64_t npix, int32_t c, float target, float weight,
                         float* loss_accum, void* dx, void* stream);
int cgan_hinge_nhwc(const void* x, int32_t dtype, int64_t npix, int32_t c, int32_t target_is_real,
                    int32_t for_discriminator, float weight, float* loss_accum, void* dx, void* stream);
int cgan_mse_const_nhwc(const void* x, int32_t dtype, int64_t npix, int32_t c, float target, float weight, float* loss_accum,
                        void* dx, void* stream);
int cgan_painter_aux_losses(const void* fake_nhwc, const float* x_nchw, const float* m_nchw, int32_t dtype, int32_t n,
                            int32_t h, int32_t w, float w_tv_h, float w_tv_w, float w_context, float w_reconstruction,
                            float* loss3, void* d_fake, void* stream);
int cgan_resize_bicubic_bwd_nhwc(const void* dy, void* dx, int32_t dtype, int32_t n, int32_t c, int32_t h_in, int32_t w_in,
                                 int32_t h_out, int32_t w_out, void* stream);
int cgan_l1_nhwc(const void* a, const void* b, int32_t dtype, int64_t numel, float weight, float* loss_accum, void* da,
                 void* stream);
#define CGAN_SN_BWD_WORKSPACE_FLOATS 1024
int cgan_spectral_norm_bwd(float* grad_w, const float* w_bar, const float* u, const float* v, const float* sigma,
                           int32_t rows, int32_t cols, float* workspace, void* stream);

int cgan_painter_heads_fwd(const void* fake_nhwc, const float* x_nchw, const float* m_nchw, void* d_in, void* vgg_in,
                           int32_t dtype, int32_t n, int32_t h, int32_t w, void* stream);
int cgan_painter_heads_bwd(const void* d_d_in, const void* d_vgg_in, const float* m_nchw, void* d_fake, int32_t dtype,
                           int32_t n, int32_t h, int32_t w, void* stream);
#define CGAN_DA_BRIGHTNESS 1
#define CGAN_DA_CONTRAST 2
#define CGAN_DA_SATURATION 4
#define CGAN_DA_TRANSLATION 8
#define CGAN_DA_CUTOUT 16
#define CGAN_DA_ALL 31
#define CGAN_DIFFAUG_PARTS 256
int cgan_diffaug_fwd(const float* x, float* y, const float* color, const int64_t* geo, int32_t flags, int32_t cut_h,
                     int32_t cut_w, int32_t n, int32_t c, int32_t h, int32_t w, float* ws, void* stream);
int cgan_diffaug_bwd(const float* dy, float* dx, const float* color, const int64_t* geo, int32_t flags, int32_t cut_h,
                     int32_t cut_w, int32_t n, int32_t c, int32_t h, int32_t w, float* ws, void* stream);
int cgan_painter_heads_diffaug_fwd(const void* fake_nhwc, const float* x_nchw, const float* m_nchw, void* d_in, void* vgg_in,
                                   const float* color, const int64_t* geo, int32_t flags, int32_t cut_h, int32_t cut_w,
                                   int32_t dtype, int32_t n, int32_t h, int32_t w, float* ws, void* stream);
int cgan_painter_heads_diffaug_bwd(const void* d_d_in, const void* d_vgg_in, const float* m_nchw, void* d_fake,
                                   const float* color, const int64_t* geo, int32_t flags, int32_t cut_h, int32_t cut_w,
                                   int32_t dtype, int32_t n, int32_t h, int32_t w, float* ws, void* stream);
int cgan_avgpool3x3s2_bwd_nhwc(const void* dy, void* dx, int32_t dtype, int32_t n, int32_t c, int32_t h_in,
                               int32_t w_in, void* stream);
int cgan_maxpool2x2_nhwc(const void* x, void* y, int32_t dtype, int32_t n, int32_t c, int32_t h_in, int32_t w_in,
                         void* stream);
int cgan_maxpool2x2_bwd_nhwc(const void* x, const void* dy, void* dx, int32_t dtype, int32_t n, int32_t c, int32_t h_in,
                             int32_t w_in, void* stream);
int cgan_maxpool2x2_relu_bwd_nhwc(const void* x, const void* dy, void* dx, int32_t dtype, int32_t n, int32_t c, int32_t h_in,
                                  int32_t w_in, void* stream);

int cgan_softmax_nhwc(const void* x, void* y, int32_t dtype, int64_t npix, int32_t c, void* stream);
int cgan_softmax_bwd_nhwc(const void* y, const void* dy, void* dx, int32_t dtype, int64_t npix, int32_t c, void* stream);
int cgan_sigmoid_pair_nhwc(const void* x, void* y, int32_t dtype, int64_t npix, void* stream);
int cgan_sigmoid_pair_bwd_nhwc(const void* y, const void* dy, void* dx, int32_t dtype, int64_t npix, void* stream);
int cgan_softmax_ce_nhwc(const void* logits, const int64_t* target, int32_t dtype, int64_t npix, int32_t c, float weight,
                         float* loss_accum, void* dlogits, void* stream);
// ... 215 lines not shown
```

Baseline: 58.02.

## Fuse BatchNorm backward channel sums into conv data-gradient epilogue

When a conv is the sole consumer of a BatchNorm+ReLU output, the conv's data-gradient GEMM epilogue now applies the ReLU mask and accumulates the per-channel sums (dy and dy*(x-mean)) into per-chunk partials. The BatchNorm backward then consumes these partials instead of re-reading x and dy in a separate reduction pass. This removes one full read of two activation tensors per fused BN layer, mainly in the ResNet bottlenecks. In exchange the GEMM store path carries extra loads and registers, and a consistency check is added that raises if the gradient arrives from a different producer.

Result: no change. 57.92 (-0.2%).

```diff
diff --git a/climategan_amd/_lib.py b/climategan_amd/_lib.py
--- a/climategan_amd/_lib.py
+++ b/climategan_amd/_lib.py
@@ -78,6 +78,12 @@
 class DataMinmaxItem(C.Structure):
     _fields_ = [("src", C.c_void_p), ("out", C.c_void_p), ("pixels", C.c_int64), ("channels", C.c_int32),
                 ("far_plane", C.c_float)]
+
+
+class BnSumsReq(C.Structure):
+    _fields_ = [("x", C.c_void_p), ("mean", C.c_void_p), ("rstd", C.c_void_p), ("fold_mean", C.c_void_p),
+                ("fold_rstd", C.c_void_p), ("partial", C.c_void_p), ("partial_bytes", C.c_size_t), ("groups", C.c_int32),
+                ("mask_src", C.c_int32), ("gneg", C.c_float)]
 
 
 _P = C.c_void_p
@@ -191,6 +197,10 @@
                                          C.c_int32, C.c_float, _P, C.c_size_t, _P]),
     "cgan_batchnorm_act_bwd_grouped": (C.c_int, [_P, _P, _P, _P, _P, _P, _P, _P, _P, _P, _P, _P, C.c_int32, C.c_int64,
                                                  C.c_int32, C.c_int32, C.c_int32, C.c_float, _P, C.c_size_t, _P]),
+    "cgan_batchnorm_act_bwd_from_partials": (C.c_int, [_P, _P, _P, _P, _P, _P, C.c_int32, _P, _P, _P, C.c_int32, C.c_int64,
+                                                       C.c_int32, C.c_int32, _P, C.c_size_t, _P]),
+    "cgan_conv2d_bwd_data_bn_sums_chunk_pixels": (C.c_int32, [C.POINTER(ConvDesc), C.c_int32, _P]),
+    "cgan_conv2d_bwd_data_bn_sums_next": (C.c_int, [_P, C.POINTER(BnSumsReq)]),
     "cgan_bce_logits_nhwc": (C.c_int, [_P, C.c_int32, C.c_int64, C.c_int32, C.c_float, C.c_float, _P, _P, _P]),
     "cgan_hinge_nhwc": (C.c_int, [_P, C.c_int32, C.c_int64, C.c_int32, C.c_int32, C.c_int32, C.c_float, _P, _P, _P]),
     "cgan_l1_nhwc": (C.c_int, [_P, _P, C.c_int32, C.c_int64, C.c_float, _P, _P, _P]),
diff --git a/climategan_amd/autograd.py b/climategan_amd/autograd.py
--- a/climategan_amd/autograd.py
+++ b/climategan_amd/autograd.py
@@ -165,7 +165,8 @@
             relu_out = ops.NHWC(x_t, cfg["c_in"]) if cfg.get("mask_input") else None
             dx = ops.conv2d_bwd_data(dy, w_eff, (x_t.shape[0], h_in, w_in), stride=cfg["stride"], pad=cfg["pad"],
                                      dilation=cfg["dilation"], sigma=sigma, pad_mode=cfg.get("pad_mode", ops.PAD_ZERO),
-                                     prepacked=ctx.dgrad, relu_out=relu_out)
+                                     prepacked=ctx.dgrad, relu_out=relu_out,
+                                     bn_sums=None if (ups or pair) else cfg.get("bn_sums"))
             dx_t = (ops.sumpool2x2(dx) if ups else dx).t
         if ctx.has_res and ctx.needs_input_grad[3]:
             dres_t = (ops.sumpool2x2(dy) if cfg.get("residual_upsample", False) else dy).t
@@ -221,7 +222,7 @@
             dx_t = ops.conv2d_bwd_data(dy, weight, (x_t.shape[0], x_t.shape[1], x_t.shape[2]), stride=cfg["stride"],
                                        pad=cfg["pad"], dilation=cfg["dilation"],
                                        pad_mode=cfg.get("pad_mode", ops.PAD_ZERO), add=add, prepacked=ctx.dgrad,
-                                       relu_out=relu_out).t
+                                       relu_out=relu_out, bn_sums=cfg.get("bn_sums")).t
         dw = db = None
         if ctx.needs_input_grad[1] or (ctx.has_bias and ctx.needs_input_grad[2]):
             dw, db = ops.conv2d_bwd_weight(
@@ -449,6 +450,7 @@
         ctx.cfg = (c, act, slope, G)
         ctx.has_res = res_t is not None
         ctx.premasked = False
+        ctx.bn_sums = None
         keep_out = res_t is not None or _BN_BWD_READS_OUT
         ctx.save_for_backward(x_t, out if keep_out else None, mean, rstd, gamma,
                               None if keep_out else mean_f, None if keep_out else rstd_f)
@@ -468,6 +470,20 @@
         dx = torch.empty_like(x_t)
         want_res = ctx.has_res and ctx.needs_input_grad[11]
         dy_t = dy_t.contiguous()
+        sums = ctx.bn_sums
+        if sums is not None and sums.get("partial") is not None:
+            partial, chunks, claimed = sums.pop("partial"), sums.pop("chunks"), sums.pop("dx")
+            if dy_t.data_ptr() != claimed.data_ptr() or dy_t.shape != claimed.shape:
+                raise RuntimeError("BatchNormActFn: the channel sums were claimed by one data gradient (claim_bn_sums), but the "
+                                   "gradient arrives from elsewhere -- the output has a second reader")
+            dg = db = None
+            if gamma is not None:
+                dg, db = torch.empty((2, c), dtype=torch.float32, device=x_t.device).unbind(0)
+            _lib.check(lib.cgan_batchnorm_act_bwd_from_partials(
+                ops._ptr(x_t), ops._ptr(dy_t), ops._ptr(mean), ops._ptr(rstd), ops._ptr(gamma), ops._ptr(partial), chunks,
+                ops._ptr(dx), ops._ptr(dg), ops._ptr(db), ops._DT[x_t.dtype], n * h * w, c, G, ops._ptr(ws), nbytes,
+                ops._stream()), "cgan_batchnorm_act_bwd_from_partials")
+            return dx, dg, db, None, None, None, None, None, None, None, None, (dy_t if want_res else None), None
         if want_res and act == ops.ACT_NONE:
             dres = dy_t
         else:
@@ -497,6 +513,30 @@
         return False
     fn.premasked = True
     return True
+
+
+FUSE_BN_BWD_SUMS = os.environ.get("CGAN_FUSE_BN_BWD_SUMS", "1") != "0"
+
+
+def claim_bn_sums(out_t: torch.Tensor):
+    fn = out_t.grad_fn
+    if not FUSE_BN_BWD_SUMS or fn is None or not isinstance(fn, BatchNormActFn._backward_cls):
+        return None
+    if fn.bn_sums is not None:
+        fn.bn_sums["void"] = True
+        return None
+    c, act, slope, G = fn.cfg
+    x_t, out, mean, rstd, _gamma, mean_f, rstd_f = fn.saved_tensors
+    if fn.has_res:
+        return None
+    if act == ops.ACT_NONE:
+        mask, gneg = 0, 0.0
+    elif act in (ops.ACT_RELU, ops.ACT_LRELU) and out is None and mean_f is not None:
+        mask, gneg = 2, (0.0 if act == ops.ACT_RELU else float(slope))
+    else:
+        return None
+    fn.bn_sums = dict(x=x_t, mean=mean, rstd=rstd, mean_f=mean_f, rstd_f=rstd_f, mask=mask, gneg=gneg, groups=G, void=False)
+    return fn.bn_sums
 
 
 def _scaled(dx, c, g):
diff --git a/climategan_amd/csrc/conv_gemm.h b/climategan_amd/csrc/conv_gemm.h
--- a/climategan_amd/csrc/conv_gemm.h
+++ b/climategan_amd/csrc/conv_gemm.h
@@ -1,5 +1,18 @@
 #pragma once
 #include "cgan_common.h"
+
+struct ConvGemmBnSums {
+  const uint16_t* x;
+  const float* mean;
+  const float* rstd;
+  const float* fmean;
+  const float* frstd;
+  float* partial;
+  int gpix;
+  int chunks;
+  int mask;
+  float gneg;
+};
 
 struct ConvGemmArgs {
   const uint16_t* x;
@@ -39,13 +52,14 @@
 int conv_gemm_pair_launch(const ConvGemmArgs& a, int dtype, hipStream_t s);
 
 bool conv_gemm_applicable(const CganConvDesc* d);
-int conv_gemm_launch(const ConvGemmArgs& a, int dtype, hipStream_t s);
+int conv_gemm_launch(const ConvGemmArgs& a, int dtype, hipStream_t s, const ConvGemmBnSums* bns = nullptr);
 bool conv_gemm_res2_ok(const ConvGemmArgs& a, int dtype);
 int conv_gemm_stats_chunk_pixels(const ConvGemmArgs& a, int dtype);
+int conv_gemm_bn_sums_chunk_pixels(const ConvGemmArgs& a, int dtype);
 bool conv_gemm_big_ok(const ConvGemmArgs& a);
 bool conv1x1_allc_ok(const ConvGemmArgs& a);
 int conv1x1_allc_launch(const ConvGemmArgs& a, int dtype, hipStream_t s);
-int conv_gemm_big_launch(const ConvGemmArgs& a, int dtype, hipStream_t s);
+int conv_gemm_big_launch(const ConvGemmArgs& a, int dtype, hipStream_t s, const ConvGemmBnSums* bns = nullptr);
 bool conv_gemm_big_pair_ok(const ConvGemmArgs& a, int dtype);
 int conv_gemm_big_pair_launch(const ConvGemmArgs& a, int dtype, hipStream_t s);
 bool conv1x1_xres_ok(const ConvGemmArgs& a);
@@ -127,10 +141,10 @@
   }
 }
 
-template <typename T, int WC, int WP, int PP, bool RES2 = false>
+template <typename T, int WC, int WP, int PP, bool RES2 = false, bool BNS = false>
 __device__ __forceinline__ void conv_gemm_staged_store(const f32x4 (&acc)[WC][WP], const ConvGemmArgs& p,
                                                        unsigned char* stg, int pix0, int cout_base, const float* bias_ep,
-                                                       int lane, int j, int g) {
+                                                       int lane, int j, int g, const ConvGemmBnSums* bnp = nullptr) {
   constexpr int ROWB = WC * 64 + 16;
   constexpr int CH = WC * 2;
   constexpr int NIT = PP * 16 * CH / 64;
@@ -140,6 +154,7 @@
   const int qc = lane % CH, pl0 = lane / CH;
   const int ch = cout_base + qc * 8;
   const bool ch_ok = ch < p.cout_s;
+  constexpr bool BNS_WIDE = BNS && WC * WP >= 32;
   const bool plain = !bias_ep && !p.has_res && p.act == CGAN_ACT_NONE && p.cout == p.cout_s;
   f32x4 bb0 = (f32x4){0.f, 0.f, 0.f, 0.f}, bb1 = bb0;
   if (bias_ep && ch_ok) {
@@ -147,6 +162,19 @@
     bb1 = *reinterpret_cast<const f32x4*>(bias_ep + ch + 4);
   }
   u32x4 rv[NPASS][NIT];
+  u32x4 bx[BNS ? NPASS : 1][BNS ? NIT : 1];
+  float bsum[BNS ? 16 : 1], bmu[BNS ? 8 : 1], bfm[BNS ? 8 : 1], bfr[BNS ? 8 : 1];
+  auto load_bx = [&](int pass) {
+#pragma unroll
+    for (int it = 0; it < (BNS ? NIT : 0); ++it) {
+      const int pix = pix0 + pass * PP * 16 + it * PSTEP + pl0;
+      bx[pass][it] = (u32x4){0u, 0u, 0u, 0u};
+      if (pix < p.npix && ch_ok) bx[pass][it] = CGAN_LD_STREAM(reinterpret_cast<const u32x4*>(bnp->x + (size_t)pix * p.cout_s + ch));
+    }
+  };
+  const float bgn = (BNS && bnp->mask == 2) ? bnp->gneg : 1.f;
+  const int bgrp = BNS ? min(pix0, p.npix - 1) / bnp->gpix : 0;
+  static_assert(!BNS || PP * 16 * ROWB >= 64 * 64, "the lanes' sums are exchanged through the wave's staging rows");
   u32x4 rm[RES2 ? (NPASS > 1 ? 2 : 1) : 1][RES2 ? NIT : 1];
   auto load_rm = [&](int pass, u32x4 (&dst)[RES2 ? NIT : 1]) {
 #pragma unroll
@@ -156,7 +184,7 @@
       if (pix < p.npix && ch_ok) dst[it] = CGAN_LD_STREAM(reinterpret_cast<const u32x4*>(p.res2 + (size_t)pix * p.cout_s + ch));
     }
   };
-  if (p.has_res) {
+  if (!BNS_WIDE && p.has_res) {
 #pragma unroll
     for (int pass = 0; pass < NPASS; ++pass)
 #pragma unroll
@@ -193,6 +221,21 @@
       load_rm(pass + 1, rm[(pass + 1) & 1]);
       __builtin_amdgcn_sched_barrier(0);
     }
+    if (BNS && pass == 0) {
+      __builtin_amdgcn_sched_barrier(0);
+#pragma unroll
+      for (int ps = 0; ps < NPASS; ++ps) load_bx(ps);
+      const size_t row = (size_t)bgrp * p.cout_s + ch;
+#pragma unroll
+      for (int r = 0; r < (BNS ? 8 : 0); ++r) {
+        bmu[r] = ch_ok ? bnp->mean[row + r] : 0.f;
+        bfm[r] = (ch_ok && bnp->mask == 2) ? bnp->fmean[row + r] : 0.f;
+        bfr[r] = (ch_ok && bnp->mask == 2) ? bnp->frstd[row + r] : 0.f;
+      }
+#pragma unroll
+      for (int r = 0; r < (BNS ? 16 : 0); ++r) bsum[r] = 0.f;
+      __builtin_amdgcn_sched_barrier(0);
+    }
     if (pass == 0 || (RES2 && p.has_res == 3 && pass >= 2)) __builtin_amdgcn_s_waitcnt(0x0F70);
 #pragma unroll
     for (int it = 0; it < NIT; ++it) {
@@ -218,7 +261,7 @@
             v[2 * e] = cgan_res_apply3(v[2 * e], r0, m0);
             v[2 * e + 1] = cgan_res_apply3(v[2 * e + 1], r1, m1);
           }
-        } else if (p.has_res) {
+        } else if (!BNS_WIDE && p.has_res) {
 #pragma unroll
           for (int e = 0; e < 4; ++e) {
             float r0, r1;
@@ -237,9 +280,51 @@
       u32x4 o;
 #pragma unroll
       for (int e = 0; e < 4; ++e) o[e] = pack2<T>(v[2 * e], v[2 * e + 1]);
+      if constexpr (BNS) {
+#pragma unroll
+        for (int e = 0; e < 4; ++e) {
+          float d0, d1, x0, x1;
+          unpack2<T>(o[e], d0, d1);
+          unpack2<T>(bx[pass][it][e], x0, x1);
+          d0 = (x0 - bfm[2 * e]) * bfr[2 * e] > 0.f ? d0 : d0 * bgn;
+          d1 = (x1 - bfm[2 * e + 1]) * bfr[2 * e + 1] > 0.f ? d1 : d1 * bgn;
+          o[e] = pack2<T>(d0, d1);
+          unpack2<T>(o[e], d0, d1);
+          bsum[4 * e] += d0;
+          bsum[4 * e + 1] += d0 * (x0 - bmu[2 * e]);
+          bsum[4 * e + 2] += d1;
+          bsum[4 * e + 3] += d1 * (x1 - bmu[2 * e + 1]);
+        }
+      }
       if (pix < p.npix && ch_ok) CGAN_ST_STREAM(o, reinterpret_cast<u32x4*>(p.y + (size_t)pix * p.cout_s + ch));
     }
     asm volatile("s_waitcnt lgkmcnt(0)" ::: "memory");
+  }
+  if constexpr (BNS) {
+    if (pix0 >= p.npix) return;
+    float* red = reinterpret_cast<float*>(stg);
+#pragma unroll
+    for (int q = 0; q < 4; ++q)
+      *reinterpret_cast<f32x4*>(red + lane * 16 + 4 * q) = (f32x4){bsum[4 * q], bsum[4 * q + 1], bsum[4 * q + 2], bsum[4 * q + 3]};
+    asm volatile("s_waitcnt lgkmcnt(0)" ::: "memory");
+    if (pl0 == 0 && ch_ok) {
+      f32x4 t[4];
+#pragma unroll
+      for (int q = 0; q < 4; ++q) t[q] = *reinterpret_cast<const f32x4*>(red + qc * 16 + 4 * q);
+#pragma unroll
+      for (int l = 1; l < 64 / CH; ++l)
+#pragma unroll
+        for (int q = 0; q < 4; ++q) t[q] += *reinterpret_cast<const f32x4*>(red + (l * CH + qc) * 16 + 4 * q);
+      const float* rs = bnp->rstd + (size_t)bgrp * p.cout_s + ch;
+      const int chunk = (pix0 - bgrp * bnp->gpix) / (WP * 16);
+      float* dst = bnp->partial + (((size_t)bgrp * bnp->chunks + chunk) * p.cout_s + ch) * 2;
+#pragma unroll
+      for (int q = 0; q < 4; ++q) {
+        t[q][1] *= rs[2 * q];
+        t[q][3] *= rs[2 * q + 1];
+        *reinterpret_cast<f32x4*>(dst + 4 * q) = t[q];
+      }
+    }
   }
 }
 #endif
diff --git a/climategan_amd/csrc/conv_gemm.hip b/climategan_amd/csrc/conv_gemm.hip
--- a/climategan_amd/csrc/conv_gemm.hip
+++ b/climategan_amd/csrc/conv_gemm.hip
@@ -14,8 +14,8 @@
   return i;
 }
 
-template <typename T, int WAVES_C, int WC, int WP, bool REFLECT, int NS = NSTAGE, bool RES2 = false>
-__global__ __launch_bounds__(256, 2) void conv_gemm_kernel(ConvGemmArgs p, int npb, int ncb) {
+template <typename T, int WAVES_C, int WC, int WP, bool REFLECT, int NS = NSTAGE, bool RES2 = false, bool BNS = false>
+__global__ __launch_bounds__(256, 2) void conv_gemm_kernel(ConvGemmArgs p, int npb, int ncb, ConvGemmBnSums bn) {
   constexpr int WAVES_P = 4 / WAVES_C;
   constexpr int CT_BLK = WAVES_C * WC;
   constexpr int PT_BLK = WAVES_P * WP;
@@ -147,7 +147,7 @@
     conv_gemm_stats_epilogue<T, WC, WP>(acc, p, cout_base, pblk * WAVES_P + wp, j, g);
     if (p.bias) bias_ep = nullptr;
   }
-  conv_gemm_staged_store<T, WC, WP, PP, RES2>(acc, p, stg, (pblk * PT_BLK + wp * WP) * 16, cout_base, bias_ep, lane, j, g);
+  conv_gemm_staged_store<T, WC, WP, PP, RES2, BNS>(acc, p, stg, (pblk * PT_BLK + wp * WP) * 16, cout_base, bias_ep, lane, j, g, &bn);
 }
 
 template <typename T, int WC, int WP>
@@ -410,14 +410,14 @@
 }
 
 
-template <typename T, int WAVES_C, int WC, int WP, bool REFLECT, int NS = NSTAGE, bool RES2 = false>
-int launch_cfg2(const ConvGemmArgs& a, hipStream_t s) {
+template <typename T, int WAVES_C, int WC, int WP, bool REFLECT, int NS = NSTAGE, bool RES2 = false, bool BNS = false>
+int launch_cfg2(const ConvGemmArgs& a, hipStream_t s, const ConvGemmBnSums* bns = nullptr) {
   constexpr int WAVES_P = 4 / WAVES_C;
   constexpr int CT_BLK = WAVES_C * WC, PT_BLK = WAVES_P * WP;
   constexpr size_t smem = (size_t)NS * (CT_BLK + PT_BLK) * 1024;
   static bool attr_set = false;
   if (!attr_set) {
-    hipError_t e = hipFuncSetAttribute(reinterpret_cast<const void*>(&conv_gemm_kernel<T, WAVES_C, WC, WP, REFLECT, NS, RES2>),
+    hipError_t e = hipFuncSetAttribute(reinterpret_cast<const void*>(&conv_gemm_kernel<T, WAVES_C, WC, WP, REFLECT, NS, RES2, BNS>),
                                        hipFuncAttributeMaxDynamicSharedMemorySize, 160 * 1024);
     if (e != hipSuccess) {
       cgan_set_error("conv_gemm: hipFuncSetAttribute failed: %s", hipGetErrorString(e));
@@ -428,7 +428,8 @@
   const int npb = ceil_div(ceil_div(a.npix, 16), PT_BLK);
   const int ncb = ceil_div(a.ctiles, CT_BLK);
   const int grid = ceil_div(npb, 8) * 8 * ncb;
-  hipLaunchKernelGGL((conv_gemm_kernel<T, WAVES_C, WC, WP, REFLECT, NS, RES2>), dim3(grid), dim3(256), smem, s, a, npb, ncb);
+  hipLaunchKernelGGL((conv_gemm_kernel<T, WAVES_C, WC, WP, REFLECT, NS, RES2, BNS>), dim3(grid), dim3(256), smem, s, a, npb, ncb,
+                     bns ? *bns : ConvGemmBnSums{});
   return CGAN_OK;
 }
 
@@ -486,15 +487,25 @@
 }
 
 template <typename T>
-int launch(const ConvGemmArgs& a, hipStream_t s) {
+int launch(const ConvGemmArgs& a, hipStream_t s, const ConvGemmBnSums* bns) {
   const Choice ch = choose(a, std::is_same<T, BF16>::value);
   switch (ch.kind) {
     case KIND_K64_256x128: return launch_k64<T, 8, 4>(a, s);
     case KIND_K64_128x256: return launch_k64<T, 4, 8>(a, s);
-    case KIND_BIG: return conv_gemm_big_launch(a, T::id, s);
+    case KIND_BIG: return conv_gemm_big_launch(a, T::id, s, bns);
     case KIND_DIRECT: return conv1x1_allc_launch(a, T::id, s);
     case KIND_XRES: return conv1x1_xres_launch(a, T::id, s);
     default: break;
+  }
+  if (bns) {
+    switch (ch.cfg) {
+      case 2: return launch_cfg2<T, 2, 8, 4, false, NSTAGE, false, true>(a, s, bns);
+      case 3: return launch_cfg2<T, 2, 4, 8, false, NSTAGE, false, true>(a, s, bns);
+      case 4: return launch_cfg2<T, 2, 4, 4, false, NSTAGE, false, true>(a, s, bns);
+      default: break;
+    }
+    cgan_set_error("conv_gemm: no BatchNorm-sums store path for this launch");
+    return CGAN_ERR_UNSUPPORTED;
   }
   switch (ch.cfg) {
     case 1: return launch_cfg<T, 1, 4, 4>(a, s);
@@ -520,13 +531,28 @@
 CGAN_DEV_ONLY(extern "C" void cgan_debug_set_gemm_cfg(int v) { g_gemm_cfg = v; })
 CGAN_DEV_ONLY(extern "C" void cgan_debug_set_gemm_ws(int v) { g_gemm_ws = v; })
 
-int conv_gemm_launch(const ConvGemmArgs& a, int dtype, hipStream_t s) {
-  return dtype == CGAN_F16 ? launch<F16>(a, s) : launch<BF16>(a, s);
+int conv_gemm_launch(const ConvGemmArgs& a, int dtype, hipStream_t s, const ConvGemmBnSums* bns) {
+  if (bns && !bns->partial) bns = nullptr;
+  return dtype == CGAN_F16 ? launch<F16>(a, s, bns) : launch<BF16>(a, s, bns);
 }
 
 bool conv_gemm_res2_ok(const ConvGemmArgs& a, int dtype) {
   const Choice ch = choose(a, dtype == CGAN_BF16);
   return (ch.kind == KIND_PLAIN && ch.cfg == 5 && a.pad_mode != CGAN_PAD_REFLECT) || ch.kind == KIND_BIG;
+}
+
+int conv_gemm_bn_sums_chunk_pixels(const ConvGemmArgs& a, int dtype) {
+  if (a.bias || a.act != CGAN_ACT_NONE || a.stats || a.res_ups || a.pad_mode == CGAN_PAD_REFLECT) return 0;
+  if (a.cout != a.cout_s || (a.cout_s & 63) != 0) return 0;
+  const Choice ch = choose(a, dtype == CGAN_BF16);
+  if (ch.kind == KIND_BIG) return a.has_res == 0 ? 64 : 0;
+  if (ch.kind != KIND_PLAIN) return 0;
+  switch (ch.cfg) {
+    case 2: return a.has_res == 0 ? 64 : 0;
+    case 3: return a.has_res == 0 ? 128 : 0;
+    case 4: return 64;
+    default: return 0;
+  }
 }
 
 int conv_gemm_stats_chunk_pixels(const ConvGemmArgs& a, int dtype) {
diff --git a/climategan_amd/csrc/conv_gemm_big.hip b/climategan_amd/csrc/conv_gemm_big.hip
--- a/climategan_amd/csrc/conv_gemm_big.hip
+++ b/climategan_amd/csrc/conv_gemm_big.hip
@@ -5,8 +5,8 @@
 
 __device__ __attribute__((aligned(16))) unsigned int g_big_zeros[4];
 
-template <typename T, int NW, bool PAIR = false, bool RES2 = false>
-__global__ __launch_bounds__(NW * 64, NW / 4) void conv_gemm_big_kernel(ConvGemmArgs p, int npb, int ncb) {
+template <typename T, int NW, bool PAIR = false, bool RES2 = false, bool BNS = false>
+__global__ __launch_bounds__(NW * 64, NW / 4) void conv_gemm_big_kernel(ConvGemmArgs p, int npb, int ncb, ConvGemmBnSums bn) {
   constexpr int WC = NW == 16 ? 4 : 8;
   constexpr int WP = NW == 4 ? 8 : 4;
   constexpr bool DOUBLE = NW == 4;
@@ -219,7 +219,7 @@
     if (p.bias) bias_ep = nullptr;
   }
   if constexpr (!PAIR) {
-    conv_gemm_staged_store<T, WC, WP, PP, RES2>(acc, p, stg, (pblk * PT_BLK + wp * WP) * 16, cout_base, bias_ep, lane, j16, g);
+    conv_gemm_staged_store<T, WC, WP, PP, RES2, BNS>(acc, p, stg, (pblk * PT_BLK + wp * WP) * 16, cout_base, bias_ep, lane, j16, g, &bn);
     return;
   }
   constexpr int NIT = PP * 16 * CH / 64;
@@ -322,12 +322,12 @@
   epilogue_pass(std::integral_constant<int, 1>{});
 }
 
-template <typename T, int NW, bool PAIR = false, bool RES2 = false>
-int launch_big(const ConvGemmArgs& a, hipStream_t s) {
+template <typename T, int NW, bool PAIR = false, bool RES2 = false, bool BNS = false>
+int launch_big(const ConvGemmArgs& a, hipStream_t s, const ConvGemmBnSums* bns = nullptr) {
   constexpr size_t smem = 160 * 1024;
   static bool attr_set = false;
   if (!attr_set) {
-    hipError_t e = hipFuncSetAttribute(reinterpret_cast<const void*>(&conv_gemm_big_kernel<T, NW, PAIR, RES2>),
+    hipError_t e = hipFuncSetAttribute(reinterpret_cast<const void*>(&conv_gemm_big_kernel<T, NW, PAIR, RES2, BNS>),
                                        hipFuncAttributeMaxDynamicSharedMemorySize, 160 * 1024);
     if (e != hipSuccess) {
       cgan_set_error("conv_gemm_big: hipFuncSetAttribute failed: %s", hipGetErrorString(e));
@@ -338,7 +338,8 @@
   const int npb = ceil_div(ceil_div(a.npix, 16), 16);
   const int ncb = ceil_div(a.ctiles, 16);
   const int grid = ceil_div(npb, 8) * 8 * ncb;
-  hipLaunchKernelGGL((conv_gemm_big_kernel<T, NW, PAIR, RES2>), dim3(grid), dim3(NW * 64), smem, s, a, npb, ncb);
+  hipLaunchKernelGGL((conv_gemm_big_kernel<T, NW, PAIR, RES2, BNS>), dim3(grid), dim3(NW * 64), smem, s, a, npb, ncb,
+                     bns ? *bns : ConvGemmBnSums{});
   return CGAN_OK;
 }
 
@@ -352,7 +353,14 @@
 CGAN_KNOB(int, g_big_waves, 8);
 CGAN_DEV_ONLY(extern "C" void cgan_debug_set_big_waves(int v) { g_big_waves = v; })
 
-int conv_gemm_big_launch(const ConvGemmArgs& a, int dtype, hipStream_t s) {
+int conv_gemm_big_launch(const ConvGemmArgs& a, int dtype, hipStream_t s, const ConvGemmBnSums* bns) {
+  if (bns && bns->partial) {
+    if (a.has_res == 3) {
+      cgan_set_error("conv_gemm_big: no BatchNorm-sums store path with has_res == 3");
+      return CGAN_ERR_UNSUPPORTED;
+    }
+    return dtype == CGAN_F16 ? launch_big<F16, 8, false, false, true>(a, s, bns) : launch_big<BF16, 8, false, false, true>(a, s, bns);
+  }
   if (g_big_waves == 16 && a.has_res != 3)
     return dtype == CGAN_F16 ? launch_big<F16, 16>(a, s) : launch_big<BF16, 16>(a, s);
   if (a.has_res == 3)
diff --git a/climategan_amd/csrc/conv_mfma.hip b/climategan_amd/csrc/conv_mfma.hip
--- a/climategan_amd/csrc/conv_mfma.hip
+++ b/climategan_amd/csrc/conv_mfma.hip
@@ -672,6 +672,21 @@
     if (g_ws[i].stream == stream && g_ws[i].device == dev) return g_ws[i];
   return WsSlot{dev, stream, nullptr, 0};
 }
+struct BnsSlot { int device; void* stream; CganBnSumsReq req; };
+BnsSlot g_bns[WS_SLOTS];
+int g_bns_n = 0;
+bool bns_take(void* stream, CganBnSumsReq* out) {
+  const int dev = ws_device();
+  std::lock_guard<std::mutex> lk(g_ws_mu);
+  for (int i = 0; i < g_bns_n; ++i)
+    if (g_bns[i].stream == stream && g_bns[i].device == dev) {
+      if (out) *out = g_bns[i].req;
+      g_bns[i] = g_bns[g_bns_n - 1];
+      --g_bns_n;
+      return true;
+    }
+  return false;
+}
 size_t ws_max_bytes() {
   const int dev = ws_device();
   std::lock_guard<std::mutex> lk(g_ws_mu);
@@ -779,6 +794,7 @@
 enum { RES_NONE = 0, RES_ADD = 1, RES_RELU = 2, RES_ADD_RELU = 3 };
 
 struct ConvPlan {
+  ConvGemmBnSums bns;
   ConvRoute route;
   ConvParams p;
   CganConvDesc d;
@@ -857,7 +873,7 @@
   ConvParams& p = pl.p;
   int rc = fill_params(p, d);
   if (rc != CGAN_OK) return rc;
-  pl.d = *d; pl.ksplit = 1; pl.ws = nullptr;
+  pl.d = *d; pl.ksplit = 1; pl.ws = nullptr; pl.bns = ConvGemmBnSums{};
   if (mode != FWD_PAIR) {
     pl.route = route_stride1(pl, mode == FWD_STATS, ws);
     return CGAN_OK;
@@ -889,7 +905,7 @@
   }
   rc = fill_params(p, &t);
   if (rc != CGAN_OK) return rc;
-  pl.ksplit = 1; pl.ws = nullptr;
+  pl.ksplit = 1; pl.ws = nullptr; pl.bns = ConvGemmBnSums{};
   t.pad = p.pad = pad_t;
   t.h_out = p.h_out = f->h_in; t.w_out = p.w_out = f->w_in;
   p.npix = f->n * f->h_in * f->w_in;
@@ -943,7 +959,7 @@
   const int dt = pl.d.dtype;
   int rc = CGAN_OK;
   switch (pl.route) {
-    case ROUTE_GEMM: rc = conv_gemm_launch(gemm_args(p), dt, s); break;
+    case ROUTE_GEMM: rc = conv_gemm_launch(gemm_args(p), dt, s, &pl.bns); break;
     case ROUTE_SPLITK: rc = conv_gemm_splitk_launch(gemm_args(p), pl.ksplit, pl.ws, dt, s); break;
     case ROUTE_LDS3X3: case ROUTE_SUBPIXEL: rc = conv3x3_lds_launch(lds_args(pl), dt, s); break;
     case ROUTE_SMALLCIN: rc = conv_smallcin_launch(lds_args(pl), dt, s); break;
@@ -1097,14 +1113,64 @@
   return kernel_kind_impl(d, bwd_data, WsSlot{0, nullptr, nullptr, ws_max_bytes()});
 }
 
+static int bn_sums_chunk_pixels(const ConvPlan& pl, int res_mode) {
+  const ConvParams& p = pl.p;
+  if (pl.route != ROUTE_GEMM || (res_mode == RES_ADD_RELU && p.has_res != 3)) return 0;
+  if ((double)p.npix * p.cout_s * 2.0 >= 2147483648.0) return 0;
+  return conv_gemm_bn_sums_chunk_pixels(gemm_args(p), pl.d.dtype);
+}
+
+extern "C" int32_t cgan_conv2d_bwd_data_bn_sums_chunk_pixels(const CganConvDesc* fwd, int32_t res_mode, void* stream) {
+  if (res_mode < RES_NONE || res_mode > RES_ADD_RELU) return 0;
+  ConvPlan pl;
+  if (plan_dgrad(pl, fwd, res_mode, ws_lookup(stream)) != CGAN_OK) return 0;
+  return bn_sums_chunk_pixels(pl, res_mode);
+}
+
+extern "C" int cgan_conv2d_bwd_data_bn_sums_next(void* stream, const CganBnSumsReq* req) {
+  bns_take(stream, nullptr);
+  if (!req) return CGAN_OK;
+  CGAN_REQUIRE(req->x && req->mean && req->rstd && req->partial, "conv2d_bwd_data_bn_sums_next: null pointer");
+  CGAN_REQUIRE(req->groups >= 1 && req->groups <= 16, "conv2d_bwd_data_bn_sums_next: bad group count %d", req->groups);
+  CGAN_REQUIRE(req->mask_src >= 0 && req->mask_src <= 2, "conv2d_bwd_data_bn_sums_next: bad mask source %d", req->mask_src);
+  CGAN_REQUIRE(req->mask_src != 2 || (req->fold_mean && req->fold_rstd),
+               "conv2d_bwd_data_bn_sums_next: mask source 2 needs fold_mean / fold_rstd");
+  const int dev = ws_device();
+  std::lock_guard<std::mutex> lk(g_ws_mu);
+  CGAN_REQUIRE(g_bns_n < WS_SLOTS, "conv2d_bwd_data_bn_sums_next: too many pending requests");
+  g_bns[g_bns_n++] = BnsSlot{dev, stream, *req};
+  return CGAN_OK;
+}
+
 static int bwd_data_impl(const void* dy, const void* packed_w_dgrad, const void* res, const void* relu_out, void* dx,
                          const CganConvDesc* fwd, void* stream, int res_mode) {
+  CganBnSumsReq req;
+  const bool want_bns = bns_take(stream, &req);
   CGAN_REQUIRE(dy && packed_w_dgrad && dx, "conv2d_nhwc_bwd_data: null pointer");
   ConvPlan pl;
   int rc = plan_dgrad(pl, fwd, res_mode, ws_lookup(stream));
   if (rc != CGAN_OK) return rc;
   bind(pl.p, dy, packed_w_dgrad, nullptr, res, dx);
   if (pl.p.has_res == 3) pl.p.res2 = (const uint16_t*)relu_out;
+  if (want_bns) {
+    const int ppb = bn_sums_chunk_pixels(pl, res_mode);
+    CGAN_REQUIRE(ppb > 0, "conv2d_nhwc_bwd_data: this launch's kernel takes no BatchNorm sums "
+                          "(cgan_conv2d_bwd_data_bn_sums_chunk_pixels returned 0)");
+    const int gpix = pl.p.npix / req.groups;
+    CGAN_REQUIRE(pl.p.npix % req.groups == 0 && gpix % ppb == 0,
+                 "conv2d_nhwc_bwd_data: a group's %d pixels are no whole number of %d-pixel sums rows", gpix, ppb);
+    CGAN_REQUIRE(req.mask_src != 1 || res_mode == RES_RELU || res_mode == RES_ADD_RELU,
+                 "conv2d_nhwc_bwd_data: mask source 1 is the _relu / _add_relu epilogue's");
+    CGAN_REQUIRE(req.mask_src == 1 || (res_mode != RES_RELU && res_mode != RES_ADD_RELU),
+                 "conv2d_nhwc_bwd_data: two activation masks on one gradient");
+    const size_t need = (size_t)req.groups * (gpix / ppb) * pl.p.cout_s * 2 * sizeof(float);
+    if (req.partial_bytes < need) {
+      cgan_set_error("conv2d_nhwc_bwd_data: BatchNorm-sums partial buffer %zu B < required %zu B", req.partial_bytes, need);
+      return CGAN_ERR_WORKSPACE;
+    }
+    pl.bns = ConvGemmBnSums{(const uint16_t*)req.x, req.mean, req.rstd, req.fold_mean, req.fold_rstd, req.partial,
+                            gpix, gpix / ppb, req.mask_src == 2 ? 2 : 0, req.gneg};
+  }
   rc = launch_plan(pl, (hipStream_t)stream, "conv2d_nhwc_bwd_data");
   if (rc != CGAN_OK || res_mode != RES_ADD_RELU || pl.p.has_res == 3) return rc;
   return cgan_act_bwd(relu_out, dx, dx, fwd->dtype, CGAN_ACT_RELU, 0.f,
diff --git a/climategan_amd/csrc/train_ops.hip b/climategan_amd/csrc/train_ops.hip
--- a/climategan_amd/csrc/train_ops.hip
+++ b/climategan_amd/csrc/train_ops.hip
@@ -449,6 +449,23 @@
     if (dgamma) dgamma[ch] = dg_sum;
     if (dbeta) dbeta[ch] = db_sum;
   }
+}
+
+__global__ __launch_bounds__(256) void bn_bwd_premerge_kernel(const float* __restrict__ partial, float* __restrict__ out,
+                                                              int chunks, int len, int out_rows, int cs) {
+  const int ncol = cs / 2;
+  const long idx = (long)blockIdx.x * 256 + threadIdx.x;
+  if (idx >= (long)out_rows * ncol) return;
+  const int k = (int)(idx / ncol), c = (int)(idx - (long)k * ncol);
+  const float4* src = reinterpret_cast<const float4*>(partial + (size_t)blockIdx.y * chunks * cs * 2) + c;
+  const int r0 = k * len, r1 = min(chunks, r0 + len);
+  float4 a = make_float4(0.f, 0.f, 0.f, 0.f);
+#pragma unroll 4
+  for (int r = r0; r < r1; ++r) {
+    const float4 v = src[(size_t)r * ncol];
+    a.x += v.x; a.y += v.y; a.z += v.z; a.w += v.w;
+  }
+  reinterpret_cast<float4*>(out + ((size_t)blockIdx.y * out_rows + k) * cs * 2)[c] = a;
 }
 
 template <typename T, int MASK>
@@ -732,6 +749,46 @@
   return CGAN_OK;
 }
 
+extern "C" int cgan_batchnorm_act_bwd_from_partials(const void* x, const void* dz, const float* batch_mean,
+                                                    const float* batch_rstd, const float* gamma, const float* partial,
+                                                    int32_t chunks, void* dx, float* dgamma, float* dbeta, int32_t dtype,
+                                                    int64_t npix_total, int32_t c, int32_t groups, void* workspace,
+                                                    size_t workspace_bytes, void* stream) {
+  CGAN_REQUIRE(x && dz && batch_mean && batch_rstd && partial && dx && workspace, "batchnorm_act_bwd_from_partials: null pointer");
+  CGAN_REQUIRE(dtype == CGAN_F16 || dtype == CGAN_BF16, "batchnorm_act_bwd_from_partials: bad dtype %d", dtype);
+  CGAN_REQUIRE(groups >= 1 && groups <= 16 && npix_total > 0 && c > 0 && npix_total % groups == 0 && chunks >= 1,
+               "batchnorm_act_bwd_from_partials: bad shape (the pixel count must divide into the groups)");
+  CGAN_REQUIRE(workspace_bytes >= (size_t)groups * cgan_batchnorm_act_bwd_workspace_bytes(c),
+               "batchnorm_act_bwd_from_partials: workspace too small");
+  const long npix = npix_total / groups;
+  const int cs = cgan_cs(c);
+  hipStream_t s = (hipStream_t)stream;
+  float* coef = (float*)workspace;
+  float* merged = coef + (size_t)groups * 3 * cs;
+  const float* rows = partial;
+  int nrows = chunks;
+  if (chunks > BN_BWD_MAX_CHUNKS) {
+    const int len = ceil_div(chunks, BN_BWD_MAX_CHUNKS);
+    nrows = ceil_div(chunks, len);
+    const long items = (long)nrows * (cs / 2);
+    hipLaunchKernelGGL(bn_bwd_premerge_kernel, dim3((unsigned)((items + 255) / 256), groups), dim3(256), 0, s, partial, merged,
+                       (int)chunks, len, nrows, cs);
+    rows = merged;
+  }
+  hipLaunchKernelGGL(bn_bwd_finalize_kernel, dim3(cs / 8), dim3(256), 0, s, rows, nrows, batch_mean, batch_rstd, gamma,
+                     1.f / (float)npix, coef, dgamma, dbeta, (int)c, cs, (int)groups);
+  const int cg_total = cs / 8;
+  const int tpp = cg_total < 256 ? cg_total : 256;
+  const int prows = 256 / tpp;
+  long blocks = (npix + (long)prows * 4 - 1) / ((long)prows * 4);
+  blocks = blocks < 1 ? 1 : (blocks > 4096 / groups ? 4096 / groups : blocks);
+  DISPATCH_T2(dtype, bn_bwd_apply_kernel, 0, dim3((unsigned)blocks, groups), dim3(256), 0, s, (const uint16_t*)x,
+              (const uint16_t*)nullptr, (const uint16_t*)dz, (const float*)coef, (const float*)nullptr, (const float*)nullptr,
+              (uint16_t*)dx, (uint16_t*)nullptr, (long)npix, cs, 0.f);
+  CGAN_CHECK_LAUNCH("batchnorm_act_bwd_from_partials");
+  return CGAN_OK;
+}
+
 extern "C" int cgan_spectral_norm_bwd(float* grad_w, const float* w_bar, const float* u, const float* v,
                                       const float* sigma, int32_t rows, int32_t cols, float* workspace,
                                       void* stream) {
diff --git a/climategan_amd/deeplab/resnet101_v3.py b/climategan_amd/deeplab/resnet101_v3.py
--- a/climategan_amd/deeplab/resnet101_v3.py
+++ b/climategan_amd/deeplab/resnet101_v3.py
@@ -34,10 +34,10 @@
             x = residual
         else:
             out = conv_bn_forward(self.conv1, self.bn1, self._c[0], x, act=ops.ACT_RELU)
-        out = conv_bn_forward(self.conv2, self.bn2, self._c[1], out, act=ops.ACT_RELU)
+        out = conv_bn_forward(self.conv2, self.bn2, self._c[1], out, act=ops.ACT_RELU, sole_consumer=True)
         if self.downsample is not None:
             residual = conv_bn_forward(self.downsample[0], self.downsample[1], self._c[3], x)
-        return conv_bn_forward(self.conv3, self.bn3, self._c[2], out, act=ops.ACT_RELU, residual=residual)
+        return conv_bn_forward(self.conv3, self.bn3, self._c[2], out, act=ops.ACT_RELU, residual=residual, sole_consumer=True)
 
 
 class ResNet(nn.Module):
diff --git a/climategan_amd/norms.py b/climategan_amd/norms.py
--- a/climategan_amd/norms.py
+++ b/climategan_amd/norms.py
@@ -31,6 +31,9 @@
                residual_upsample=bool(kw.get("residual_upsample", False)), pad_mode=pad_mode,
                sn_owned=bool(kw.get("sn_owned", False)), pair_in=bool(kw.get("pair_in", False)),
                want_stats=bool(kw.get("want_stats", False)))
+    if kw.get("sole_consumer"):
+        from .autograd import claim_bn_sums
+        cfg["bn_sums"] = claim_bn_sums(x.t)
     y_t = ConvFn.apply(x.t, weight, bias, res.t if res is not None else None, packed, cfg, sn)
     if kw.get("want_stats"):
         return ops.NHWC(y_t, weight.shape[0]), cfg.get("stats_out")
@@ -229,6 +232,7 @@
 
 
 def conv_bn_forward(conv: nn.Conv2d, bn, cache: _PackCache, x: ops.NHWC, pad_mode=ops.PAD_ZERO, pad=None, **kw) -> ops.NHWC:
+    sole_consumer = kw.pop("sole_consumer", False)
     train_bn = bn is not None and bn.training
     grad = needs_grad(conv, x.t) or (bn is not None and needs_grad(bn))
     p = conv.padding[0] if pad is None else pad
@@ -258,7 +262,6 @@
     from .autograd import BatchNormActFn
 
     act, slope, residual = kw.pop("act", ops.ACT_NONE), kw.pop("slope", 0.2), kw.pop("residual", None)
-    sole_consumer = kw.pop("sole_consumer", False)
     if kw.get("in_upsample") or kw.get("residual_upsample"):
         raise NotImplementedError("conv_bn_forward: folded upsamples are not used on the training path")
     pw = cache.get_plain(conv.weight, conv.bias, x.t.dtype)
@@ -271,6 +274,9 @@
         if sole_consumer and FUSE_RELU_MASK:
             from .autograd import claim_relu_mask
             pcfg["mask_input"] = claim_relu_mask(x.t)
+        if sole_consumer:
+            from .autograd import claim_bn_sums
+            pcfg["bn_sums"] = claim_bn_sums(x.t)
         y_t, pass_t = ConvPassFn.apply(x.t, conv.weight, conv.bias, pw, pcfg)
         y, passthrough = ops.NHWC(y_t, conv.weight.shape[0]), ops.NHWC(pass_t, x.c)
         conv_stats = pcfg.get("stats_out")
@@ -281,9 +287,10 @@
         conv_stats = None
         if FUSE_BN_STATS:
             y, conv_stats = _conv_train(x, conv.weight, conv.bias, pw, None, conv.stride[0], p, conv.dilation[0],
-                                        dict(pad_mode=pad_mode, want_stats=True))
+                                        dict(pad_mode=pad_mode, want_stats=True, sole_consumer=sole_consumer))
         else:
-            y = _conv_train(x, conv.weight, conv.bias, pw, None, conv.stride[0], p, conv.dilation[0], dict(pad_mode=pad_mode))
+            y = _conv_train(x, conv.weight, conv.bias, pw, None, conv.stride[0], p, conv.dilation[0],
+                            dict(pad_mode=pad_mode, sole_consumer=sole_consumer))
     if residual is not None and not FUSE_BN_RESIDUAL:
         from . import functional as Fn
         out_t = BatchNormActFn.apply(y.t, bn.weight if bn.affine else None, bn.bias if bn.affine else None,
diff --git a/climategan_amd/ops.py b/climategan_amd/ops.py
--- a/climategan_amd/ops.py
+++ b/climategan_amd/ops.py
@@ -1057,9 +1057,27 @@
     return NHWC(dx, dxp.c)
 
 
+def _bn_sums_request(h: dict, d, res_mode: int, dx: torch.Tensor) -> None:
+    x = h["x"]
+    if x.shape != dx.shape or x.dtype != dx.dtype or not x.is_contiguous() or (h["mask"] == 1) != (res_mode >= 2):
+        return
+    lib = _lib.load()
+    ppb = lib.cgan_conv2d_bwd_data_bn_sums_chunk_pixels(C.byref(d), res_mode, _stream())
+    groups, npix = h["groups"], dx.shape[0] * dx.shape[1] * dx.shape[2]
+    if ppb <= 0 or npix % groups or (npix // groups) % ppb:
+        return
+    chunks = npix // groups // ppb
+    partial = _empty((groups, chunks, dx.shape[3], 2), dtype=torch.float32, device=dx.device)
+    req = _lib.BnSumsReq(_ptr(x), _ptr(h["mean"]), _ptr(h["rstd"]), _ptr(h["mean_f"]), _ptr(h["rstd_f"]), _ptr(partial),
+                         partial.nbytes, groups, h["mask"], h["gneg"])
+    _lib.check(lib.cgan_conv2d_bwd_data_bn_sums_next(_stream(), C.byref(req)), "cgan_conv2d_bwd_data_bn_sums_next")
+    h["partial"], h["chunks"], h["dx"] = partial, chunks, dx
+
+
 def conv2d_bwd_data(dy: NHWC, w: torch.Tensor, x_shape, stride=1, pad=0, dilation=1,
                     sigma: Optional[torch.Tensor] = None, pad_mode=PAD_ZERO, add: Optional[NHWC] = None,
-                    prepacked: Optional[DgradPack] = None, relu_out: Optional[NHWC] = None) -> NHWC:
+                    prepacked: Optional[DgradPack] = None, relu_out: Optional[NHWC] = None,
+                    bn_sums: Optional[dict] = None) -> NHWC:
     same = stride == 1 and pad_mode == PAD_ZERO and 2 * pad == dilation * (w.shape[2] - 1) and w.shape[2] == w.shape[3]
     if relu_out is not None:
         if not same:
@@ -1103,6 +1121,8 @@
                    "cgan_conv2d_pack_weight_dgrad")
     dx = _empty((n, h_in, w_in, cs8(c_in)), dtype=dy.t.dtype, device=dy.t.device)
     _conv_ws()
+    if bn_sums is not None and not bn_sums.get("void"):
+        _bn_sums_request(bn_sums, d, (2 if relu_out is not None else 0) + (1 if add is not None else 0), dx)
     if relu_out is not None:
         if relu_out.t.shape != dx.shape or relu_out.t.dtype != dx.dtype or not relu_out.t.is_contiguous():
             raise RuntimeError("conv2d_bwd_data: ``relu_out`` %s does not match dx %s" % (tuple(relu_out.t.shape), tuple(dx.shape)))
diff --git a/include/climategan_hip.h b/include/climategan_hip.h
--- a/include/climategan_hip.h
+++ b/include/climategan_hip.h
@@ -78,6 +78,20 @@
                                    const CganConvDesc* fwd, void* stream);
 int cgan_conv2d_nhwc_bwd_data_add_relu(const void* dy, const void* packed_w_dgrad, const void* dx_add, const void* relu_out,
                                        void* dx, const CganConvDesc* fwd, void* stream);
+typedef struct {
+  const void* x;
+  const float* mean;
+  const float* rstd;
+  const float* fold_mean;
+  const float* fold_rstd;
+  float* partial;
+  size_t partial_bytes;
+  int32_t groups;
+  int32_t mask_src;
+  float gneg;
+} CganBnSumsReq;
+int32_t cgan_conv2d_bwd_data_bn_sums_chunk_pixels(const CganConvDesc* fwd, int32_t res_mode, void* stream);
+int cgan_conv2d_bwd_data_bn_sums_next(void* stream, const CganBnSumsReq* req);
 size_t cgan_conv2d_bwd_weight_workspace_bytes(const CganConvDesc* fwd);
 int cgan_conv2d_nhwc_bwd_weight(const void* x, const void* dy, float* dw_oihw, float* dbias, const CganConvDesc* fwd,
                                 void* workspace, size_t workspace_bytes,
@@ -218,6 +232,10 @@
                                    const float* fold_rstd, void* dx, float* dgamma, float* dbeta, void* dz_out,
                                    int32_t dtype, int64_t npix_total, int32_t c, int32_t groups, int32_t act,
                                    float act_slope, void* workspace, size_t workspace_bytes, void* stream);
+int cgan_batchnorm_act_bwd_from_partials(const void* x, const void* dz, const float* batch_mean, const float* batch_rstd,
+                                         const float* gamma, const float* partial, int32_t chunks, void* dx, float* dgamma,
+                                         float* dbeta, int32_t dtype, int64_t npix_total, int32_t c, int32_t groups,
+                                         void* workspace, size_t workspace_bytes, void* stream);
 int cgan_bce_logits_nhwc(const void* x, int32_t dtype, int64_t npix, int32_t c, float target, float weight,
                          float* loss_accum, void* dx, void* stream);
 int cgan_hinge_nhwc(const void* x, int32_t dtype, int64_t npix, int32_t c, int32_t target_is_real,
```
